# arkworks-rs/algebra

Hardware: AMD Instinct MI355X
Metric: G1 scalar-muls/sec (MSM, 2^24) (higher is better)
Workload: dtype u32

## Files before the change

### algebra_amd/_lib.py

```python
import ctypes as C
import os

_HERE = os.path.dirname(os.path.abspath(__file__))
LIB_PATH = os.environ.get("ARK_HIP_LIB") or os.path.join(_HERE, "libark_hip.so")

u64p = C.POINTER(C.c_uint64)


class ArkHipError(RuntimeError):
    def __init__(self, code, what):
        super().__init__("%s failed with code %d" % (what, code))
        self.code = code


class Radix2DomainStruct(C.Structure):
    _fields_ = [
        ("size", C.c_uint64),
        ("log_size_of_group", C.c_uint32),
        ("_pad", C.c_uint32),
        ("size_as_field_element", C.c_uint64 * 4),
        ("size_inv", C.c_uint64 * 4),
        ("group_gen", C.c_uint64 * 4),
        ("group_gen_inv", C.c_uint64 * 4),
        ("offset", C.c_uint64 * 4),
        ("offset_inv", C.c_uint64 * 4),
        ("offset_pow_size", C.c_uint64 * 4),
    ]


SYMBOLS = {
    "ark_hip_device_count": (C.c_int, []),
    "ark_hip_init": (C.c_int, [C.c_int]),
    "ark_hip_set_device": (C.c_int, [C.c_int]),
    "ark_hip_get_device": (C.c_int, []),
    "ark_hip_host_alloc": (C.c_int, [C.c_size_t, C.POINTER(C.c_void_p)]),
    "ark_hip_host_free": (C.c_int, [C.c_void_p]),
    "ark_hip_msm_sw_device_async": (C.c_int, [C.c_int, C.c_void_p, C.c_void_p, C.c_size_t, C.c_int, C.POINTER(C.c_void_p)]),
    "ark_hip_msm_wait": (C.c_int, [C.c_void_p, C.c_void_p]),
    "ark_hip_msm_bases_prepare": (C.c_int, [C.c_int, C.c_void_p, C.c_size_t, C.POINTER(C.c_void_p)]),
    "ark_hip_msm_bases_prepare_device": (C.c_int, [C.c_int, C.c_void_p, C.c_size_t, C.POINTER(C.c_void_p)]),
    "ark_hip_msm_bases_free": (C.c_int, [C.c_void_p]),
    "ark_hip_msm_bases_info": (C.c_int, [C.c_void_p, C.POINTER(C.c_size_t), C.POINTER(C.c_int), C.POINTER(C.c_int),
                                         C.POINTER(C.c_size_t)]),
    "ark_hip_msm_prepared": (C.c_int, [C.c_void_p, C.c_void_p, C.c_size_t, C.c_int, C.c_void_p]),
    "ark_hip_msm_prepared_device": (C.c_int, [C.c_void_p, C.c_void_p, C.c_size_t, C.c_int, C.c_void_p]),
    "ark_hip_msm_prepared_async": (C.c_int, [C.c_void_p, C.c_void_p, C.c_size_t, C.c_int, C.POINTER(C.c_void_p)]),
    "ark_hip_msm_prepared_device_async": (C.c_int, [C.c_void_p, C.c_void_p, C.c_size_t, C.c_int, C.POINTER(C.c_void_p)]),
    "ark_hip_msm_sw_chunks": (C.c_int, [C.c_int, C.c_void_p, C.c_size_t, C.c_void_p, C.c_size_t, C.c_size_t, C.c_void_p]),
    "ark_hip_msm_sw_multi": (C.c_int, [C.c_int, C.c_int, C.c_void_p, C.c_void_p, C.c_size_t, C.c_int, C.c_void_p]),
    "ark_hip_msm_sw_multi_device": (C.c_int, [C.c_int, C.c_int, C.POINTER(C.c_void_p), C.POINTER(C.c_void_p),
                                              C.POINTER(C.c_size_t), C.c_int, C.c_void_p]),
    "ark_hip_batch_mul_table_new": (C.c_int, [C.c_int, C.c_void_p, C.c_size_t, C.POINTER(C.c_void_p)]),
    "ark_hip_batch_mul_table_free": (C.c_int, [C.c_void_p]),
    "ark_hip_batch_mul": (C.c_int, [C.c_void_p, C.c_void_p, C.c_size_t, C.c_int, C.c_void_p]),
    "ark_hip_batch_mul_device": (C.c_int, [C.c_void_p, C.c_void_p, C.c_size_t, C.c_int, C.c_void_p]),
    "ark_hip_fft_in_place_degree_aware": (C.c_int, [C.c_int, C.POINTER(Radix2DomainStruct), C.c_void_p, C.c_size_t]),
    "ark_hip_fft_in_place_degree_aware_device": (C.c_int, [C.c_int, C.POINTER(Radix2DomainStruct), C.c_void_p, C.c_size_t]),
    "ark_hip_fft_batch_in_place_device": (C.c_int, [C.c_int, C.POINTER(Radix2DomainStruct), C.POINTER(C.c_void_p), C.c_size_t,
                                                    C.c_int]),
    "ark_hip_shutdown": (None, []),
    "ark_hip_synchronize": (C.c_int, []),
    "ark_hip_version": (C.c_char_p, []),
    "ark_hip_host_threads": (C.c_int, [C.POINTER(C.c_int)]),
    "ark_hip_curve_info": (C.c_int, [C.c_int] + [C.POINTER(C.c_int)] * 4),
    "ark_hip_malloc": (C.c_int, [C.c_size_t, C.POINTER(C.c_void_p)]),
    "ark_hip_free": (C.c_int, [C.c_void_p]),
    "ark_hip_memcpy_h2d": (C.c_int, [C.c_void_p, C.c_void_p, C.c_size_t]),
    "ark_hip_memcpy_d2h": (C.c_int, [C.c_void_p, C.c_void_p, C.c_size_t]),
    "ark_hip_curve_generator": (C.c_int, [C.c_int, C.c_void_p]),
    "ark_hip_msm_sw": (C.c_int, [C.c_int, C.c_void_p, C.c_void_p, C.c_size_t, C.c_int, C.c_void_p]),
    "ark_hip_msm_sw_small": (C.c_int, [C.c_int, C.c_void_p, C.c_void_p, C.c_size_t, C.c_int, C.c_int, C.c_void_p]),
    "ark_hip_msm_sw_small_device": (C.c_int, [C.c_int, C.c_void_p, C.c_void_p, C.c_size_t, C.c_int, C.c_int, C.c_void_p]),
    "ark_hip_msm_prepared_small_device": (C.c_int, [C.c_void_p, C.c_void_p, C.c_size_t, C.c_int, C.c_int, C.c_void_p]),
    "ark_hip_msm_bases_pin": (C.c_int, [C.c_int, C.c_void_p, C.c_size_t]),
    "ark_hip_msm_bases_unpin": (C.c_int, [C.c_int, C.c_void_p, C.c_size_t]),
    "ark_hip_msm_cache_config": (C.c_int, [C.c_longlong, C.c_int]),
    "ark_hip_msm_cache_clear": (C.c_int, []),
    "ark_hip_msm_cache_stats": (C.c_int, [C.POINTER(C.c_uint64)]),
    "ark_hip_msm_cache_hash_stats": (C.c_int, [C.POINTER(C.c_uint64)]),
    "ark_hip_msm_sw_device": (C.c_int, [C.c_int, C.c_void_p, C.c_void_p, C.c_size_t, C.c_int, C.c_void_p]),
    "ark_hip_msm_plan": (C.c_int, [C.c_int, C.c_size_t, C.c_int, C.POINTER(C.c_int), C.POINTER(C.c_int)]),
    "ark_hip_msm_plan_widths": (C.c_int, [C.c_int, C.c_size_t, C.c_uint32, C.POINTER(C.c_uint32), C.POINTER(C.c_int),
                                          C.POINTER(C.c_int)]),
    "ark_hip_msm_set_timing": (C.c_int, [C.c_int]),
    "ark_hip_msm_last_timing": (C.c_int, [C.POINTER(C.c_double)]),
    "ark_hip_sw_sum": (C.c_int, [C.c_int, C.c_void_p, C.c_size_t, C.c_void_p]),
    "ark_hip_sw_into_affine": (C.c_int, [C.c_int, C.c_void_p, C.c_size_t, C.c_void_p]),
    "ark_hip_sw_add_affine_device": (C.c_int, [C.c_int, C.c_void_p, C.c_void_p, C.c_size_t, C.c_void_p]),
    "ark_hip_sw_normalize_batch_device": (C.c_int, [C.c_int, C.c_void_p, C.c_void_p, C.c_size_t]),
    "ark_hip_radix2_domain_new": (C.c_int, [C.c_int, C.c_size_t, C.POINTER(Radix2DomainStruct)]),
    "ark_hip_radix2_domain_get_coset": (C.c_int, [C.c_int, C.POINTER(Radix2DomainStruct), C.c_void_p,
                                                  C.POINTER(Radix2DomainStruct)]),
    "ark_hip_fft_in_place": (C.c_int, [C.c_int, C.POINTER(Radix2DomainStruct), C.c_void_p]),
    "ark_hip_ifft_in_place": (C.c_int, [C.c_int, C.POINTER(Radix2DomainStruct), C.c_void_p]),
    "ark_hip_fft_in_place_device": (C.c_int, [C.c_int, C.POINTER(Radix2DomainStruct), C.c_void_p]),
    "ark_hip_ifft_in_place_device": (C.c_int, [C.c_int, C.POINTER(Radix2DomainStruct), C.c_void_p]),
    "ark_hip_fr_mul_device": (C.c_int, [C.c_int, C.c_void_p, C.c_void_p, C.c_void_p, C.c_size_t]),
    "ark_hip_poly_mul": (C.c_int, [C.c_int, C.c_void_p, C.c_size_t, C.c_void_p, C.c_size_t, C.c_void_p, C.POINTER(C.c_size_t)]),
    "ark_hip_sw_normalize_batch": (C.c_int, [C.c_int, C.c_void_p, C.c_size_t, C.c_void_p]),
    "ark_hip_fr_pow": (C.c_int, [C.c_int, C.c_void_p, C.c_uint64, C.c_void_p]),
    "ark_hip_fft_axis_device": (C.c_int, [C.c_int, C.c_void_p, C.c_uint, C.c_size_t, C.c_void_p]),
    "ark_hip_comm_unique_id": (C.c_int, [C.c_void_p]),
    "ark_hip_comm_init": (C.c_int, [C.c_void_p, C.c_int, C.c_int]),
    "ark_hip_comm_info": (C.c_int, [C.POINTER(C.c_int), C.POINTER(C.c_int)]),
    "ark_hip_comm_destroy": (C.c_int, []),
    "ark_hip_msm_sw_device_sharded": (C.c_int, [C.c_int, C.c_void_p, C.c_void_p, C.c_size_t, C.c_int, C.c_void_p]),
    "ark_hip_msm_prepared_device_sharded": (C.c_int, [C.c_void_p, C.c_void_p, C.c_size_t, C.c_int, C.c_void_p]),
    "ark_hip_msm_prepared_multi": (C.c_int, [C.c_int, C.POINTER(C.c_void_p), C.c_void_p, C.c_size_t, C.c_int, C.c_void_p]),
    "ark_hip_fft_sharded_device": (C.c_int, [C.c_int, C.POINTER(Radix2DomainStruct), C.c_void_p, C.c_int]),
    "ark_hip_fft_shard_local_device": (C.c_int, [C.c_int, C.POINTER(Radix2DomainStruct), C.c_int, C.c_int, C.c_void_p, C.c_int]),
    "ark_hip_fft_shard_cross_device": (C.c_int, [C.c_int, C.POINTER(Radix2DomainStruct), C.c_int, C.c_void_p, C.c_void_p, C.c_int]),
    "ark_hip_fr_add_device": (C.c_int, [C.c_int, C.c_void_p, C.c_void_p, C.c_void_p, C.c_size_t]),
    "ark_hip_fr_sub_device": (C.c_int, [C.c_int, C.c_void_p, C.c_void_p, C.c_void_p, C.c_size_t]),
    "ark_hip_fr_neg_device": (C.c_int, [C.c_int, C.c_void_p, C.c_void_p, C.c_size_t]),
    "ark_hip_fft_group_in_place": (C.c_int, [C.c_int, C.c_void_p, C.c_void_p, C.c_int]),
    "ark_hip_fft_group_in_place_device": (C.c_int, [C.c_int, C.c_void_p, C.c_void_p, C.c_int]),
    "ark_hip_fr_div_device": (C.c_int, [C.c_int, C.c_void_p, C.c_void_p, C.c_void_p, C.c_size_t]),
    "ark_hip_fr_inverse_device": (C.c_int, [C.c_int, C.c_void_p, C.c_void_p, C.c_size_t]),
    "ark_hip_fr_scale_device": (C.c_int, [C.c_int, C.c_void_p, C.c_void_p, C.c_void_p, C.c_size_t]),
    "ark_hip_memcpy_d2d": (C.c_int, [C.c_void_p, C.c_void_p, C.c_size_t]),
    "ark_hip_memset_device": (C.c_int, [C.c_void_p, C.c_int, C.c_size_t]),
    "ark_hip_poly_evaluate_device": (C.c_int, [C.c_int, C.c_void_p, C.c_size_t, C.c_void_p, C.c_void_p]),
    "ark_hip_poly_divide_linear_device": (C.c_int, [C.c_int, C.c_void_p, C.c_size_t, C.c_void_p, C.c_void_p, C.c_void_p]),
    "ark_hip_poly_divide_by_vanishing_device": (C.c_int, [C.c_int, C.c_size_t, C.c_void_p, C.c_size_t, C.c_void_p, C.c_void_p]),
    "ark_hip_domain_lagrange_coefficients_device": (C.c_int, [C.c_int, C.POINTER(Radix2DomainStruct), C.c_void_p, C.c_void_p]),
    "ark_hip_fr_inner_product_device": (C.c_int, [C.c_int, C.c_void_p, C.c_void_p, C.c_size_t, C.c_void_p]),
    "ark_hip_poly_scan_plan": (C.c_int, [C.c_size_t, C.POINTER(C.c_int), C.POINTER(C.c_int)]),
    "ark_hip_fft_set_kernel": (C.c_int, [C.c_int]),
    "ark_hip_fft_set_timing": (C.c_int, [C.c_int]),
    "ark_hip_fft_last_timing": (C.c_int, [C.POINTER(C.c_double)]),
}

TEST_SYMBOLS = {
    "ark_hip_test_field_op": (C.c_int, [C.c_int, C.c_int, C.c_void_p, C.c_void_p, C.c_void_p, C.c_size_t]),
    "ark_hip_test_basefield_op": (C.c_int, [C.c_int, C.c_int, C.c_void_p, C.c_void_p, C.c_void_p, C.c_size_t]),
    "ark_hip_test_host_basefield_op": (C.c_int, [C.c_int, C.c_int, C.c_void_p, C.c_void_p, C.c_void_p, C.c_size_t]),
    "ark_hip_test_point_op": (C.c_int, [C.c_int, C.c_int, C.c_void_p, C.c_void_p, C.c_void_p, C.c_size_t]),
    "ark_hip_test_msm_sharded_emulated": (C.c_int, [C.c_int, C.c_int, C.POINTER(C.c_void_p), C.POINTER(C.c_void_p),
                                                    C.POINTER(C.c_size_t), C.c_int, C.c_void_p, C.POINTER(C.c_int)]),
    "ark_hip_test_base_hash": (C.c_int, [C.c_void_p, C.c_size_t, C.POINTER(C.c_uint64)]),
    "ark_hip_test_lazy_raw_op": (C.c_int, [C.c_int, C.c_int, C.c_int, C.c_int, C.c_void_p, C.c_void_p, C.c_size_t]),
    "ark_hip_test_lazy_acc_op": (C.c_int, [C.c_int, C.c_int, C.c_void_p, C.c_void_p, C.c_void_p, C.c_size_t]),
    "ark_hip_test_msm_host_fold": (C.c_int, [C.c_int, C.c_void_p, C.c_int, C.c_int, C.c_int, C.c_void_p, C.c_void_p]),
    "ark_hip_test_msm_host_fold_l0": (C.c_int, [C.c_int, C.c_void_p, C.c_int, C.c_int, C.c_int, C.c_void_p, C.c_void_p]),
}
TEST_LIB_PATH = os.path.join(_HERE, "libark_hip_test.so")

_lib = None
_test_lib = None


def lib():
    global _lib
    if _lib is None:
        if not os.path.exists(LIB_PATH):
            raise ImportError(
                "algebra_amd: %s not found -- the HIP extension is not built and there is no CPU fallback "
                "(run `make -C algebra_amd/csrc -j8` or __graft_entry__.build())" % LIB_PATH)
        try:
            import torch
        except ImportError:
            pass
        l = C.CDLL(LIB_PATH)
        _bind(l, SYMBOLS, not os.environ.get("ARK_HIP_LIB"))
        _lib = l
    return _lib


def _bind(l, table, strict):
    for name, (res, args) in table.items():
        try:
            fn = getattr(l, name)
        except AttributeError:
            if not strict:
                continue
            raise
        fn.restype = res
        fn.argtypes = args


def test_lib():
    global _test_lib
    if _test_lib is None:
        if not os.path.exists(TEST_LIB_PATH):
            raise ImportError("algebra_amd: %s not found (run `make -C algebra_amd/csrc -j8`)" % TEST_LIB_PATH)
        try:
            import torch
        except ImportError:
            pass
        l = C.CDLL(TEST_LIB_PATH)
        _bind(l, SYMBOLS, True)
        _bind(l, TEST_SYMBOLS, True)
        _test_lib = l
    return _test_lib


def check(code, what):
    if code != 0:
        raise ArkHipError(code, what)
```

### algebra_amd/csrc/msm.cuh

```cuda
#pragma once
#include <hip/hip_runtime.h>
#include <stdio.h>
#include <stdlib.h>
#include <vector>
#include <mutex>
#include <atomic>
#include "hostpool.hpp"
#include <math.h>
#include "curves.cuh"
#include "ec28.cuh"
#include "lazyk.cuh"
#include "msm_sort.cuh"

namespace arkhip {

#define ARK_HIP_TRY(expr)                                                                          \
  do {                                                                                             \
    hipError_t _e = (expr);                                                                        \
    if (_e != hipSuccess) {                                                                        \
      fprintf(stderr, "ark_hip: %s failed: %s (%s:%d)\n", #expr, hipGetErrorString(_e), __FILE__, __LINE__); \
      return -(int)_e - 1000;                                                                      \
    }                                                                                              \
  } while (0)

static constexpr u32 KEY_NONE = 0xffffffffu;

__host__ __device__ __forceinline__ int msm_window_width(int w, int c, int W, int narrow) {
  return w >= W - narrow ? c - 1 : c;
}

template <class SP>
__host__ __device__ __forceinline__ u32 msm_scalar_magnitude(const u32* __restrict__ scalars, u32 i, int mont, u32* v ,
                                                             u32* __restrict__ err) {
  typedef Fp<SP> S;
  S s = S::load(scalars + (size_t)i * S::N);
  if (mont) s = S::from_mont(s);
  if constexpr (SP::BITS < 32 * S::N) {
    if ((s.l[S::N - 1] >> (SP::BITS - 32 * (S::N - 1))) != 0) {
#if defined(__HIP_DEVICE_COMPILE__)
      if (err) atomicOr(err, 1u);
#else
      (void)err;
#endif
      s = S::zero();
    }
  }
  {
    u32 u[S::N];
    u32 borrow = 0;
#pragma unroll
    for (int k = 0; k < S::N; k++) {
      u32 bo;
      u[k] = __builtin_subc(s.l[k], (u32)SP::P[k], borrow, &bo);
      borrow = bo;
    }
    if (!borrow) {
#pragma unroll
      for (int k = 0; k < S::N; k++) s.l[k] = u[k];
    }
  }
  u32 t[S::N];
  {
    u32 borrow = 0;
#pragma unroll
    for (int k = 0; k < S::N; k++) {
      u64 x = (u64)SP::P[k] - s.l[k] - borrow;
      t[k] = (u32)x;
      borrow = (u32)(x >> 63);
    }
  }
  bool lt = false;
#pragma unroll
  for (int k = 0; k < S::N; k++) {
    if (t[k] != s.l[k]) lt = t[k] < s.l[k];
  }
#pragma unroll
  for (int k = 0; k < S::N; k++) v[k] = lt ? t[k] : s.l[k];
  v[S::N] = 0;
  return lt ? 0x80000000u : 0u;
}

static constexpr int MSM_WIDTH_CLASSES = 9;
static constexpr int MSM_WIDTH_TOP[MSM_WIDTH_CLASSES] = {0, 1, 8, 16, 32, 64, 128, 192, 256};
struct MsmWidths {
  u32 max_bits;
  u32 count[MSM_WIDTH_CLASSES];
};
template <class SP>
__global__ void __launch_bounds__(1024) msm_scalar_bits_kernel(const u32* __restrict__ scalars, u32 n, u32 stride, int mont,
                                                               u32* __restrict__ out ,
                                                               u32 chunk = 0, u32* __restrict__ nz_counts = nullptr) {
  typedef Fp<SP> S;
  __shared__ u32 blk[1 + MSM_WIDTH_CLASSES];
  if (threadIdx.x <= MSM_WIDTH_CLASSES) blk[threadIdx.x] = 0;
  __syncthreads();
  u32 bits = 0;
  u32 mine[MSM_WIDTH_CLASSES] = {0, 0, 0, 0, 0, 0, 0, 0, 0};
  const u64 step = chunk ? (u64)blockDim.x : (u64)gridDim.x * blockDim.x;
  const u64 first = chunk ? (u64)blockIdx.x * chunk + threadIdx.x : (u64)blockIdx.x * blockDim.x + threadIdx.x;
  const u64 rounds = chunk ? (u64)chunk / blockDim.x
                           : (((u64)n + stride - 1) / stride + step - 1) / step;
  for (u64 it = 0; it < rounds; it++) {
    const u64 t = it * step + first;
    int cls = -1;
    if (t * stride < n) {
      u32 v[S::N + 1];
      (void)msm_scalar_magnitude<SP>(scalars, (u32)(t * stride), mont, v, nullptr);
      u32 b = 0;
#pragma unroll
      for (int k = 0; k < S::N; k++)
        if (v[k]) b = 32u * (u32)k + 32u - (u32)__builtin_clz(v[k]);
      bits = b > bits ? b : bits;
      cls = 0;
#pragma unroll
      for (int k = 1; k < MSM_WIDTH_CLASSES; k++) cls += b > (u32)MSM_WIDTH_TOP[k - 1] ? 1 : 0;
    }
#pragma unroll
    for (int k = 0; k < MSM_WIDTH_CLASSES; k++) mine[k] += (u32)__popcll(__ballot(cls == k));
  }
#pragma unroll
  for (int o = 32; o > 0; o >>= 1) {
    const u32 other = (u32)__shfl_xor((int)bits, o);
    bits = other > bits ? other : bits;
  }
  if ((threadIdx.x & 63) == 0) {
    atomicMax(&blk[0], bits);
#pragma unroll
    for (int k = 0; k < MSM_WIDTH_CLASSES; k++)
      if (mine[k]) atomicAdd(&blk[1 + k], mine[k]);
  }
  __syncthreads();
  if (nz_counts && threadIdx.x == 0) {
    u32 seen = 0;
#pragma unroll
    for (int k = 0; k < MSM_WIDTH_CLASSES; k++) seen += blk[1 + k];
    nz_counts[blockIdx.x] = seen - blk[1];
  }
  if (gridDim.x == 1) {
    if (threadIdx.x <= MSM_WIDTH_CLASSES) out[threadIdx.x] = blk[threadIdx.x];
  } else if (threadIdx.x == 0) {
    if (blk[0] > __atomic_load_n(out, __ATOMIC_RELAXED)) atomicMax(out, blk[0]);
  } else if (threadIdx.x <= MSM_WIDTH_CLASSES && blk[threadIdx.x]) {
    atomicAdd(out + threadIdx.x, blk[threadIdx.x]);
  }
}

template <class SP>
__global__ void __launch_bounds__(1024) msm_compact_scalars_kernel(const u32* __restrict__ scalars, u32 n, int mont, u32 chunk,
                                                                   const u32* __restrict__ chunk_off, u32* __restrict__ err,
                                                                   u32* __restrict__ out_scalars, u32* __restrict__ out_idx, u32 cap) {
  typedef Fp<SP> S;
  __shared__ u32 wave_cnt[16];
  __shared__ u32 run_s;
  if (threadIdx.x == 0) run_s = chunk_off[blockIdx.x];
  __syncthreads();
  const u32 lane = threadIdx.x & 63u, wave = threadIdx.x >> 6;
  const u32 rounds = chunk / blockDim.x;
  for (u32 it = 0; it < rounds; it++) {
    const u64 i = (u64)blockIdx.x * chunk + (u64)it * blockDim.x + threadIdx.x;
    bool keep = false;
    if (i < n) {
      u32 v[S::N + 1];
      (void)msm_scalar_magnitude<SP>(scalars, (u32)i, mont, v, err);
      u32 any = 0;
#pragma unroll
      for (int k = 0; k < S::N; k++) any |= v[k];
      keep = any != 0;
    }
    const unsigned long long m = __ballot(keep);
    if (lane == 0) wave_cnt[wave] = (u32)__popcll(m);
    __syncthreads();
    u32 before = run_s;
    for (u32 w = 0; w < wave; w++) before += wave_cnt[w];
    if (keep) {
      const u32 pos = before + (u32)__popcll(m & ((1ull << lane) - 1ull));
      if (pos < cap) {
        const uint4* src = (const uint4*)(scalars + (size_t)i * S::N);
        uint4* dst = (uint4*)(out_scalars + (size_t)pos * S::N);
        dst[0] = src[0];
        dst[1] = src[1];
        out_idx[pos] = (u32)i;
      } else {
        atomicOr(err, 2u);
      }
    }
    __syncthreads();
    if (threadIdx.x == 0) {
      u32 tot = 0;
      for (u32 w = 0; w < (blockDim.x >> 6); w++) tot += wave_cnt[w];
      run_s += tot;
    }
    __syncthreads();
  }
}
template <class SP>
void msm_sample_widths_host(const void* h_scalars, size_t n, int mont, MsmWidths* out) {
  typedef Fp<SP> S;
  *out = MsmWidths{};
  out->max_bits = (u32)SP::BITS;
  if (n == 0) return;
  const size_t stride = n > 1024 ? n / 1024 : 1;
  size_t seen = 0;
  u32 cnt[MSM_WIDTH_CLASSES] = {0};
  for (size_t i = 0; i < n; i += stride) {
    u32 v[S::N + 1];
    (void)msm_scalar_magnitude<SP>((const u32*)h_scalars, (u32)i, mont, v, nullptr);
    u32 b = 0;
    for (int k = 0; k < S::N; k++)
      if (v[k]) b = 32u * (u32)k + 32u - (u32)__builtin_clz(v[k]);
    int cls = 0;
    for (int k = 1; k < MSM_WIDTH_CLASSES; k++) cls += b > (u32)MSM_WIDTH_TOP[k - 1] ? 1 : 0;
    cnt[cls]++;
    seen++;
  }
  for (int k = 0; k < MSM_WIDTH_CLASSES; k++) out->count[k] = (u32)((double)cnt[k] * (double)n / (double)seen);
}
static inline struct MsmPlan msm_plan_for_widths(size_t n, int field_bits, double mul_cost, bool lazy28, const MsmWidths& w);
static inline bool msm_widths_skewed(const MsmWidths& w) {
  u64 seen = 0, wide = 0;
  for (int k = 0; k < MSM_WIDTH_CLASSES; k++) {
    seen += w.count[k];
    if (MSM_WIDTH_TOP[k] > 128) wide += w.count[k];
  }
  return 2 * wide < seen;
}

template <class SP>
__global__ void __launch_bounds__(256) msm_digits_kernel(const u32* __restrict__ scalars, u32 n, int mont, int c,
                                                         int W, int narrow, u32* __restrict__ keys,
                                                         u32* __restrict__ err) {
  u32 i = blockIdx.x * blockDim.x + threadIdx.x;
  if (i >= n) return;
  typedef Fp<SP> S;
  u32 v[S::N + 1];
  const u32 flip = msm_scalar_magnitude<SP>(scalars, i, mont, v, err);
  u32 carry = 0;
  for (int w = 0; w < W; w++) {
    const int cw = msm_window_width(w, c, W, narrow);
    const u32 mask = (1u << cw) - 1u;
    const u32 half = 1u << (cw - 1);
    u32 raw = (v[0] & mask) + carry;
#pragma unroll
    for (int k = 0; k < S::N; k++) v[k] = (v[k] >> cw) | (v[k + 1] << (32 - cw));
    u32 key = KEY_NONE;
    if (w < W - 1) {
      carry = raw >= half ? 1u : 0u;
    } else {
      carry = 0;
    }
    int d = (int)raw - (int)(carry << cw);
    if (d != 0) {
      u32 mag = d < 0 ? (u32)(-d) : (u32)d;
      if (mag > half) {
        atomicOr(err, 1u);
        mag = half;
      }
      u32 sign = (d < 0 ? 0x80000000u : 0u) ^ flip;
      key = sign | (mag - 1);
    }
    keys[(size_t)w * n + i] = key;
  }
}

template <int BYTES>
__global__ void __launch_bounds__(256) msm_digits_small_kernel(const unsigned char* __restrict__ scalars, u32 n, int c, int W,
                                                               int narrow, u64 vmask, u32* __restrict__ keys) {
  u32 i = blockIdx.x * blockDim.x + threadIdx.x;
  if (i >= n) return;
  u64 v;
  if constexpr (BYTES == 1) v = scalars[i];
  else if constexpr (BYTES == 2) v = ((const unsigned short*)scalars)[i];
  else if constexpr (BYTES == 4) v = ((const u32*)scalars)[i];
  else v = ((const u64*)scalars)[i];
  v &= vmask;
  u32 carry = 0;
  for (int w = 0; w < W; w++) {
    const int cw = msm_window_width(w, c, W, narrow);
    const u32 mask = (1u << cw) - 1u;
    const u32 half = 1u << (cw - 1);
    const u32 raw = ((u32)v & mask) + carry;
    v >>= cw;
    carry = (w < W - 1 && raw >= half) ? 1u : 0u;
    const int d = (int)raw - (int)(carry << cw);
    u32 key = KEY_NONE;
    if (d != 0) {
      u32 mag = d < 0 ? (u32)(-d) : (u32)d;
      if (mag > half) mag = half;
      key = (d < 0 ? 0x80000000u : 0u) | (mag - 1);
    }
    keys[(size_t)w * n + i] = key;
  }
}

static constexpr int SCAN_TILE = 2048;

static __global__ void __launch_bounds__(256) scan_block_sums(const u32* __restrict__ in, size_t m, u32* __restrict__ sums) {
  __shared__ u32 sh[256];
  size_t base = (size_t)blockIdx.x * SCAN_TILE;
  u32 s = 0;
  for (int k = 0; k < 8; k++) {
    size_t j = base + threadIdx.x + (size_t)k * 256;
    if (j < m) s += in[j];
  }
  sh[threadIdx.x] = s;
  __syncthreads();
  for (int o = 128; o > 0; o >>= 1) {
    if ((int)threadIdx.x < o) sh[threadIdx.x] += sh[threadIdx.x + o];
    __syncthreads();
  }
  if (threadIdx.x == 0) sums[blockIdx.x] = sh[0];
}
static __global__ void __launch_bounds__(1024) scan_sums_inplace(u32* sums, u32 nb) {
  __shared__ u32 sh[1024];
  __shared__ u32 carry_s;
  if (threadIdx.x == 0) carry_s = 0;
  __syncthreads();
  for (u32 base = 0; base < nb; base += 1024) {
    u32 j = base + threadIdx.x;
    u32 x = j < nb ? sums[j] : 0;
    sh[threadIdx.x] = x;
    __syncthreads();
    for (int o = 1; o < 1024; o <<= 1) {
      u32 y = (int)threadIdx.x >= o ? sh[threadIdx.x - o] : 0;
      __syncthreads();
      sh[threadIdx.x] += y;
      __syncthreads();
    }
    u32 incl = sh[threadIdx.x];
    u32 cbase = carry_s;
    if (j < nb) sums[j] = cbase + incl - x;
    __syncthreads();
    if (threadIdx.x == 1023) carry_s = cbase + incl;
    __syncthreads();
  }
}
static constexpr u32 SCAN_SMALL_MAX = 16384;
static __global__ void __launch_bounds__(1024) scan_small_kernel(const u32* __restrict__ in, u32 m, u32* __restrict__ offsets) {
  __shared__ u32 sh[1024];
  const u32 per = (m + 1023u) / 1024u;
  const u32 lo = threadIdx.x * per;
  u32 s = 0;
  for (u32 k = 0; k < per; k++)
    if (lo + k < m) s += in[lo + k];
  sh[threadIdx.x] = s;
  __syncthreads();
  for (u32 o = 1; o < 1024; o <<= 1) {
    u32 y = threadIdx.x >= o ? sh[threadIdx.x - o] : 0;
    __syncthreads();
    sh[threadIdx.x] += y;
    __syncthreads();
  }
  u32 run = sh[threadIdx.x] - s;
  for (u32 k = 0; k < per; k++)
    if (lo + k < m) {
      offsets[lo + k] = run;
      run += in[lo + k];
    }
  if (threadIdx.x == 1023) offsets[m] = sh[1023];
}
static inline void scan_exclusive(const u32* in, size_t m, u32* sums, u32* offsets, hipStream_t stream);
static __global__ void __launch_bounds__(256) scan_apply(const u32* __restrict__ in, size_t m, const u32* __restrict__ sums,
                                                  u32* __restrict__ offsets) {
  __shared__ u32 sh[256];
  size_t base = (size_t)blockIdx.x * SCAN_TILE + (size_t)threadIdx.x * 8;
  u32 x[8];
  u32 s = 0;
#pragma unroll
  for (int k = 0; k < 8; k++) {
    size_t j = base + k;
    x[k] = j < m ? in[j] : 0;
    s += x[k];
  }
  sh[threadIdx.x] = s;
  __syncthreads();
  for (int o = 1; o < 256; o <<= 1) {
    u32 y = (int)threadIdx.x >= o ? sh[threadIdx.x - o] : 0;
    __syncthreads();
    sh[threadIdx.x] += y;
    __syncthreads();
  }
  u32 run = sums[blockIdx.x] + sh[threadIdx.x] - s;
#pragma unroll
  for (int k = 0; k < 8; k++) {
    size_t j = base + k;
    if (j < m) offsets[j] = run;
    run += x[k];
    if (j == m - 1) offsets[m] = run;
  }
}

static inline void scan_exclusive(const u32* in, size_t m, u32* sums, u32* offsets, hipStream_t stream) {
  if (m <= SCAN_SMALL_MAX) {
    hipLaunchKernelGGL(scan_small_kernel, dim3(1), dim3(1024), 0, stream, in, (u32)m, offsets);
    return;
  }
  const u32 nblk = (u32)((m + SCAN_TILE - 1) / SCAN_TILE);
  hipLaunchKernelGGL(scan_block_sums, dim3(nblk), dim3(256), 0, stream, in, m, sums);
  hipLaunchKernelGGL(scan_sums_inplace, dim3(1), dim3(1024), 0, stream, sums, nblk);
  hipLaunchKernelGGL(scan_apply, dim3(nblk), dim3(256), 0, stream, in, m, sums, offsets);
}

static constexpr int ORDER_TILE = 2048;
static constexpr int ORDER_BINS = 256;
__device__ __forceinline__ u32 msm_lane_load(const u32* __restrict__ offsets, size_t g, int wsum, size_t wstride) {
  u32 cnt = 0;
  for (int w = 0; w < wsum; w++) cnt += offsets[g + w * wstride + 1] - offsets[g + w * wstride];
  return cnt;
}
static __global__ void __launch_bounds__(256) msm_order_hist_kernel(const u32* __restrict__ offsets, size_t nb, int shift,
                                                                    u32 nblocks, int wsum, size_t wstride,
                                                                    u32* __restrict__ block_hist) {
  __shared__ u32 sh[ORDER_BINS];
  sh[threadIdx.x] = 0;
  __syncthreads();
  size_t base = (size_t)blockIdx.x * ORDER_TILE;
  for (int k = 0; k < ORDER_TILE / 256; k++) {
    size_t g = base + threadIdx.x + (size_t)k * 256;
    if (g < nb) {
      u32 cls = msm_lane_load(offsets, g, wsum, wstride) >> shift;
      if (cls > ORDER_BINS - 1) cls = ORDER_BINS - 1;
      atomicAdd(&sh[ORDER_BINS - 1 - cls], 1u);
    }
  }
  __syncthreads();
  block_hist[(size_t)threadIdx.x * nblocks + blockIdx.x] = sh[threadIdx.x];
}
static __global__ void __launch_bounds__(256) msm_order_scatter_kernel(const u32* __restrict__ offsets, size_t nb, int shift,
                                                                       u32 nblocks, int wsum, size_t wstride,
                                                                       const u32* __restrict__ block_off,
                                                                       u32* __restrict__ order) {
  __shared__ u32 sh[ORDER_BINS];
  sh[threadIdx.x] = block_off[(size_t)threadIdx.x * nblocks + blockIdx.x];
  __syncthreads();
  size_t base = (size_t)blockIdx.x * ORDER_TILE;
  for (int k = 0; k < ORDER_TILE / 256; k++) {
    size_t g = base + threadIdx.x + (size_t)k * 256;
    if (g < nb) {
      u32 cls = msm_lane_load(offsets, g, wsum, wstride) >> shift;
      if (cls > ORDER_BINS - 1) cls = ORDER_BINS - 1;
      u32 pos = atomicAdd(&sh[ORDER_BINS - 1 - cls], 1u);
      order[pos] = (u32)g;
    }
  }
}

template <class C>
__global__ void __launch_bounds__(256, C::ACC_MIN_WAVES) msm_accumulate_kernel(const char* __restrict__ bases,
                                                             const u32* __restrict__ sorted,
                                                             const u32* __restrict__ offsets,
                                                             const u32* __restrict__ order, u32 nbuckets,
                                                             const u32* __restrict__ d_thresh, int HB, int LB,
                                                             int accum, char* __restrict__ buckets) {
  typedef typename C::FA F;
  u32 t = (blockIdx.x * blockDim.x + threadIdx.x) / F::LANES;
  if (t >= nbuckets) return;
  u32 g = order ? order[t] : t;
  u32 j = offsets[g], end = offsets[g + 1];
  if (end - j > *d_thresh) return;
  if (accum && j == end) return;
  char* cell = buckets + (size_t)msm_slot_to_bucket(g, HB, LB) * XYZZ<F>::BYTES;
  XYZZ<F> acc = accum ? XYZZ<F>::load(cell) : XYZZ<F>::zero();
  if (j < end) {
    u32 e = sorted[j];
    u32 e1 = j + 1 < end ? sorted[j + 1] : 0;
    Affine<F> p = Affine<F>::load(bases + (size_t)(e & 0x7fffffffu) * Affine<F>::BYTES);
    for (;;) {
      u32 e2 = 0;
      Affine<F> p_next = p;
      const bool more = j + 1 < end;
      if (more) {
        p_next = Affine<F>::load(bases + (size_t)(e1 & 0x7fffffffu) * Affine<F>::BYTES);
        if (j + 2 < end) e2 = sorted[j + 2];
      }
      if (!p.is_zero()) {
        F y = p.y;
        if constexpr (C::RELAXED_A) y = (e >> 31) != 0 ? F::neg_r(p.y) : p.y;
        else y = F::cond_neg(p.y, (e >> 31) != 0);
        if constexpr (C::RELAXED_A) xyzz_madd_relaxed<F>(acc, p.x, y);
        else xyzz_madd<F>(acc, p.x, y);
      }
      if (!more) break;
      e = e1;
      e1 = e2;
      p = p_next;
      j++;
    }
  }
  if constexpr (C::RELAXED_A) acc = xyzz_canonical<F>(acc);
  acc.store(cell);
}

#ifndef ARK_LAZY_MIN_WAVES
#define ARK_LAZY_MIN_WAVES 2
#endif
template <class C>
__global__ void __launch_bounds__(256, ARK_LAZY_MIN_WAVES) msm_accumulate_lazy_kernel(const char* __restrict__ bases,
                                                                  const u32* __restrict__ sorted,
                                                                  const u32* __restrict__ offsets,
                                                                  const u32* __restrict__ order, u32 nbuckets,
                                                                  const u32* __restrict__ d_thresh, int HB, int LB,
                                                                  int accum, char* __restrict__ buckets) {
  typedef LazyK<C> K;
  typedef typename K::FM F;
  u32 t = (blockIdx.x * blockDim.x + threadIdx.x) / K::LANES;
  if (t >= nbuckets) return;
  u32 g = order ? order[t] : t;
  u32 j = offsets[g], end = offsets[g + 1];
  if (end - j > *d_thresh) return;
  if (accum && j == end) return;
  char* cell = buckets + (size_t)msm_slot_to_bucket(g, HB, LB) * XYZZ<F>::BYTES;
  typename K::Acc acc = K::inf();
  if (accum) acc = K::from_bucket(XYZZ<F>::load(cell));
  if (j < end) {
    u32 e = sorted[j];
    u32 e1 = j + 1 < end ? sorted[j + 1] : 0;
    Affine<F> p = Affine<F>::load(bases + (size_t)(e & 0x7fffffffu) * Affine<F>::BYTES);
    for (;;) {
      u32 e2 = 0;
      Affine<F> p_next = p;
      const bool more = j + 1 < end;
      if (more) {
        p_next = Affine<F>::load(bases + (size_t)(e1 & 0x7fffffffu) * Affine<F>::BYTES);
        if (j + 2 < end) e2 = sorted[j + 2];
      }
      if (!p.is_zero()) {
        if (K::madd(acc, p, (e >> 31) != 0))
          K::mdbl(acc, bases + (size_t)(e & 0x7fffffffu) * Affine<F>::BYTES, (e >> 31) != 0);
      }
      if (!more) break;
      e = e1;
      e1 = e2;
      p = p_next;
      j++;
    }
  }
  K::to_bucket(acc).store(cell);
}
template <class C>
__global__ void __launch_bounds__(256, ARK_LAZY_MIN_WAVES) msm_accumulate_parts_kernel(const char* __restrict__ bases,
                                                                  const u32* __restrict__ sorted,
                                                                  const u32* __restrict__ offsets,
                                                                  const u32* __restrict__ order, u32 nbuckets,
                                                                  const u32* __restrict__ d_thresh, int HB, int LB,
                                                                  u32 nparts, char* __restrict__ parts) {
  typedef LazyK<C> K;
  typedef typename K::FM F;
  const u32 gid = (blockIdx.x * blockDim.x + threadIdx.x) / K::LANES;
  const u32 part = gid / nbuckets, t = gid - part * nbuckets;
  if (part >= nparts) return;
  const u32 g = order ? order[t] : t;
  const u32 start = offsets[g], stop = offsets[g + 1];
  const u32 len = stop - start;
  if (len > *d_thresh) return;
  const u32 per = (len + nparts - 1) / nparts;
  const u32 a = part * per, b = a + per;
  u32 j = start + (a < len ? a : len);
  const u32 end = start + (b < len ? b : len);
  char* cell = parts + ((size_t)part * nbuckets + msm_slot_to_bucket(g, HB, LB)) * XYZZ<F>::BYTES;
  typename K::Acc acc = K::inf();
  if (j < end) {
    u32 e = sorted[j];
    u32 e1 = j + 1 < end ? sorted[j + 1] : 0;
    Affine<F> p = Affine<F>::load(bases + (size_t)(e & 0x7fffffffu) * Affine<F>::BYTES);
    for (;;) {
      u32 e2 = 0;
      Affine<F> p_next = p;
      const bool more = j + 1 < end;
      if (more) {
        p_next = Affine<F>::load(bases + (size_t)(e1 & 0x7fffffffu) * Affine<F>::BYTES);
        if (j + 2 < end) e2 = sorted[j + 2];
      }
      if (!p.is_zero()) {
        if (K::madd(acc, p, (e >> 31) != 0))
          K::mdbl(acc, bases + (size_t)(e & 0x7fffffffu) * Affine<F>::BYTES, (e >> 31) != 0);
      }
      if (!more) break;
      e = e1;
      e1 = e2;
      p = p_next;
      j++;
    }
  }
  K::to_bucket(acc).store(cell);
}
template <class C>
__global__ void __launch_bounds__(256) msm_sum_parts_kernel(const u32* __restrict__ offsets, u32 nbuckets,
                                                            const u32* __restrict__ d_thresh, int HB, int LB, u32 nparts,
                                                            const char* __restrict__ parts, int accum,
                                                            char* __restrict__ buckets) {
  typedef LazyK<C> K;
  typedef typename K::FM F;
  const u32 g = (blockIdx.x * blockDim.x + threadIdx.x) / K::LANES;
  if (g >= nbuckets) return;
  const u32 len = offsets[g + 1] - offsets[g];
  if (len > *d_thresh) return;
  if (accum && len == 0) return;
  const size_t bkt = msm_slot_to_bucket(g, HB, LB);
  char* cell = buckets + bkt * XYZZ<F>::BYTES;
  typename K::Acc acc = K::inf();
  if (accum) acc = K::from_bucket(XYZZ<F>::load(cell));
  for (u32 q = 0; q < nparts; q++) K::add(acc, XYZZ<F>::load(parts + ((size_t)q * nbuckets + bkt) * XYZZ<F>::BYTES));
  K::to_bucket(acc).store(cell);
}


template <class C>
__global__ void __launch_bounds__(256, ARK_LAZY_MIN_WAVES) msm_accumulate_shared_lazy_kernel(
    const char* __restrict__ table, size_t wstride, const u32* __restrict__ sorted, const u32* __restrict__ offsets,
    const u32* __restrict__ order, u32 nbuckets, int W, int B, const u32* __restrict__ d_thresh, int HB, int LB,
    char* __restrict__ buckets) {
  typedef LazyK<C> K;
  typedef typename K::FM F;
  u32 t = (blockIdx.x * blockDim.x + threadIdx.x) / K::LANES;
  if (t >= nbuckets) return;
  const u32 s = order ? order[t] : t;
  const u32 heavy_thresh = *d_thresh;
  typename K::Acc acc = K::inf();
  int w = 0;
  u32 na = offsets[s], nb2 = offsets[s + 1];
  u32 j = 0, end = 0;
  const char* wbase = table;
  auto open_next = [&]() -> bool {
    while (w < W) {
      const u32 a = na, b = nb2;
      const char* wb = table + (size_t)w * wstride * Affine<F>::BYTES;
      w++;
      if (w < W) {
        const u32 g = ((u32)w << B) | s;
        na = offsets[g];
        nb2 = offsets[g + 1];
      }
      if (b - a > heavy_thresh) continue;
      if (b > a) {
        j = a;
        end = b;
        wbase = wb;
        return true;
      }
    }
    return false;
  };
  auto next_entry = [&](u32& eo, const char*& wbo) -> bool {
    if (j >= end && !open_next()) return false;
    eo = sorted[j];
    wbo = wbase;
    j++;
    return true;
  };
  u32 e = 0, e1 = 0;
  const char *wb = table, *wb1 = table;
  if (next_entry(e, wb)) {
    Affine<F> p = Affine<F>::load(wb + (size_t)(e & 0x7fffffffu) * Affine<F>::BYTES);
    bool have1 = next_entry(e1, wb1);
    for (;;) {
      u32 e2 = 0;
      const char* wb2 = table;
      bool have2 = false;
      Affine<F> p_next = p;
      if (have1) {
        p_next = Affine<F>::load(wb1 + (size_t)(e1 & 0x7fffffffu) * Affine<F>::BYTES);
        have2 = next_entry(e2, wb2);
      }
      if (!p.is_zero()) {
        if (K::madd(acc, p, (e >> 31) != 0))
          K::mdbl(acc, wb + (size_t)(e & 0x7fffffffu) * Affine<F>::BYTES, (e >> 31) != 0);
      }
      if (!have1) break;
      e = e1;
      p = p_next;
      e1 = e2;
      wb1 = wb2;
      have1 = have2;
    }
  }
  K::to_bucket(acc).store(buckets + (size_t)msm_slot_to_bucket(s, HB, LB) * XYZZ<F>::BYTES);
}

template <class C>
__global__ void __launch_bounds__(256, C::ACC_MIN_WAVES) msm_accumulate_shared_kernel(
    const char* __restrict__ table, size_t wstride, const u32* __restrict__ sorted, const u32* __restrict__ offsets,
    const u32* __restrict__ order, u32 nbuckets, int W, int B, const u32* __restrict__ d_thresh, int HB, int LB,
    char* __restrict__ buckets) {
  typedef typename C::FA F;
  typedef XYZZ<F> Pt;
  u32 t = (blockIdx.x * blockDim.x + threadIdx.x) / F::LANES;
  if (t >= nbuckets) return;
  const u32 s = order ? order[t] : t;
  const u32 heavy_thresh = *d_thresh;
  Pt acc = Pt::zero();
  int w = 0;
  u32 na = offsets[s], nb2 = offsets[s + 1];
  u32 j = 0, end = 0;
  const char* wbase = table;
  auto open_next = [&]() -> bool {
    while (w < W) {
      const u32 a = na, b = nb2;
      const char* wb = table + (size_t)w * wstride * Affine<F>::BYTES;
      w++;
      if (w < W) {
        const u32 g = ((u32)w << B) | s;
        na = offsets[g];
        nb2 = offsets[g + 1];
      }
      if (b - a > heavy_thresh) continue;
      if (b > a) {
        j = a;
        end = b;
        wbase = wb;
        return true;
      }
    }
    return false;
  };
  auto next_entry = [&](u32& eo, const char*& wbo) -> bool {
    if (j >= end && !open_next()) return false;
    eo = sorted[j];
    wbo = wbase;
    j++;
    return true;
  };
  u32 e = 0, e1 = 0;
  const char *wb = table, *wb1 = table;
  if (next_entry(e, wb)) {
    Affine<F> p = Affine<F>::load(wb + (size_t)(e & 0x7fffffffu) * Affine<F>::BYTES);
    bool have1 = next_entry(e1, wb1);
    for (;;) {
      u32 e2 = 0;
      const char* wb2 = table;
      bool have2 = false;
      Affine<F> p_next = p;
      if (have1) {
        p_next = Affine<F>::load(wb1 + (size_t)(e1 & 0x7fffffffu) * Affine<F>::BYTES);
        have2 = next_entry(e2, wb2);
      }
      if (!p.is_zero()) {
        F y = p.y;
        if constexpr (C::RELAXED_A) y = (e >> 31) != 0 ? F::neg_r(p.y) : p.y;
        else y = F::cond_neg(p.y, (e >> 31) != 0);
        if constexpr (C::RELAXED_A) xyzz_madd_relaxed<F>(acc, p.x, y);
        else xyzz_madd<F>(acc, p.x, y);
      }
      if (!have1) break;
      e = e1;
      p = p_next;
      e1 = e2;
      wb1 = wb2;
      have1 = have2;
    }
  }
  if constexpr (C::RELAXED_A) acc = xyzz_canonical<F>(acc);
  acc.store(buckets + (size_t)msm_slot_to_bucket(s, HB, LB) * Pt::BYTES);
}

template <class C>
__global__ void __launch_bounds__(128) msm_table_step_kernel(const char* __restrict__ in, char* __restrict__ out, size_t n,
                                                             int width) {
  typedef typename C::F F;
  size_t i = (size_t)blockIdx.x * blockDim.x + threadIdx.x;
  if (i >= n) return;
  Affine<F> p = Affine<F>::load(in + i * Affine<F>::BYTES);
  XYZZ<F> acc = XYZZ<F>::zero();
  if (!p.is_zero()) {
    acc = xyzz_mdbl<F>(p.x, p.y);
    for (int k = 1; k < width; k++) acc = xyzz_dbl<F>(acc);
  }
  acc.store(out + i * XYZZ<F>::BYTES);
}

#ifndef ARK_HEAVY_CHUNK
#define ARK_HEAVY_CHUNK 1024
#endif
#ifndef ARK_HEAVY_COMBINE_THREADS
#define ARK_HEAVY_COMBINE_THREADS 128
#endif
static constexpr u32 HEAVY_CHUNK = ARK_HEAVY_CHUNK;
struct HeavyEntry { u32 bucket, first_item, items; };
__host__ __device__ __forceinline__ u32 msm_heavy_chunk(u32 total) {
  return total >= (1u << 23) ? 4u * HEAVY_CHUNK : total >= (1u << 22) ? 2u * HEAVY_CHUNK : HEAVY_CHUNK;
}

__device__ __forceinline__ u32 msm_heavy_threshold(const u32* __restrict__ offsets, u32 nslots, u32 forced) {
  const u32 total = offsets[nslots];
  u32 t = total / 154000u;
  if (t < 64u) t = 64u;
  const u32 mr = 4u * (total / nslots);
  if (t < mr && nslots >= 32768u) t = mr;
  return forced ? forced : t;
}

static __global__ void __launch_bounds__(256) msm_find_heavy_kernel(const u32* __restrict__ offsets, u32 nbuckets,
                                                                    u32 forced, u32* __restrict__ ctr ,
                                                                    HeavyEntry* __restrict__ list,
                                                                    uint2* __restrict__ items) {
  u32 g = blockIdx.x * blockDim.x + threadIdx.x;
  const u32 thresh = msm_heavy_threshold(offsets, nbuckets, forced);
  if (g == 0) ctr[2] = thresh;
  const u32 chunk = msm_heavy_chunk(offsets[nbuckets]);
  u32 k = 0, first = 0;
  if (g < nbuckets) {
    const u32 cnt = offsets[g + 1] - offsets[g];
    if (cnt > thresh) {
      k = (cnt + chunk - 1) / chunk;
      first = atomicAdd(&ctr[0], k);
      const u32 slot = atomicAdd(&ctr[1], 1u);
      list[slot] = HeavyEntry{g, first, k};
    }
  }
  if (k && k <= 16)
    for (u32 q = 0; q < k; q++) items[first + q] = make_uint2(g, q);
  unsigned long long big = __ballot(k > 16);
  while (big) {
    const int src = __ffsll((long long)big) - 1;
    big &= big - 1;
    const u32 kk = (u32)__shfl((int)k, src), ff = (u32)__shfl((int)first, src), gg = (u32)__shfl((int)g, src);
    for (u32 q = threadIdx.x & 63u; q < kk; q += 64u) items[ff + q] = make_uint2(gg, q);
  }
}

#ifndef ARK_REDUCE_LAZY
#define ARK_REDUCE_LAZY 1
#endif
template <class C, bool LAZY = (C::LAZY_A && ARK_REDUCE_LAZY != 0)>
struct AccOps;

template <class C>
struct AccOps<C, false> {
  typedef typename C::FA F;
  typedef XYZZ<F> Pt;
  typedef Pt Acc;
  static constexpr u32 LANES = F::LANES;
  static constexpr size_t ACC_BYTES = Pt::BYTES;
  ARK_DEV static Acc zero() { return Pt::zero(); }
  ARK_DEV static Acc from_pt(const Pt& p) { return p; }
  ARK_DEV static void madd(Acc& acc, const Affine<F>& p, bool neg, const char*) {
    if constexpr (C::RELAXED_A) xyzz_madd_relaxed<F>(acc, p.x, neg ? F::neg_r(p.y) : p.y);
    else xyzz_madd<F>(acc, p.x, F::cond_neg(p.y, neg));
  }
  ARK_DEV static void add(Acc& acc, const Pt& b) {
    if constexpr (C::RELAXED_A) xyzz_add_relaxed<F>(acc, b);
    else xyzz_add<F>(acc, b);
  }
  ARK_DEV static void add_acc(Acc& acc, const Acc& b) { add(acc, b); }
  ARK_DEV static Pt fin(const Acc& a) {
    if constexpr (C::RELAXED_A) return xyzz_canonical<F>(a);
    else return a;
  }
  ARK_DEV static void park(const Acc& a, char* slot) { a.store(slot); }
  ARK_DEV static Acc unpark(const char* slot) { return Pt::load(slot); }
  ARK_DEV static void tree(Acc& acc, char* sh, u32 slot, u32 width) {
    park(acc, sh + (size_t)slot * ACC_BYTES);
    __syncthreads();
    for (u32 o = width / 2; o > 0; o >>= 1) {
      if (slot < o) {
        add_acc(acc, unpark(sh + (size_t)(slot + o) * ACC_BYTES));
        park(acc, sh + (size_t)slot * ACC_BYTES);
      }
      __syncthreads();
    }
  }
};

template <class C>
struct AccOps<C, true> {
  typedef LazyK<C> K;
  typedef typename K::FM F;
  typedef XYZZ<F> Pt;
  typedef typename K::Acc Acc;
  static constexpr u32 LANES = K::LANES;
  static constexpr size_t ACC_BYTES = ((size_t)K::WORDS * 4 + 15) / 16 * 16;
  ARK_DEV static Acc zero() { return K::inf(); }
  ARK_DEV static Acc from_pt(const Pt& p) { return K::from_bucket(p); }
  ARK_DEV static void madd(Acc& acc, const Affine<F>& p, bool neg, const char* src) {
    if (K::madd(acc, p, neg)) K::mdbl(acc, src, neg);
  }
  ARK_DEV static void add(Acc& acc, const Pt& b) { K::add(acc, b); }
  ARK_DEV static void add_acc(Acc& acc, const Acc& b) { K::add_acc(acc, b); }
  ARK_DEV static Pt fin(const Acc& a) { return K::to_bucket(a); }
  ARK_DEV static void park(const Acc& a, char* slot) { K::park(a, slot); }
  ARK_DEV static Acc unpark(const char* slot) { return K::unpark(slot); }
  ARK_DEV static void tree(Acc& acc, char* sh, u32 slot, u32 width) {
    park(acc, sh + (size_t)slot * ACC_BYTES);
    __syncthreads();
    for (u32 o = width / 2; o > 0; o >>= 1) {
      if (slot < o) {
        add_acc(acc, unpark(sh + (size_t)(slot + o) * ACC_BYTES));
        park(acc, sh + (size_t)slot * ACC_BYTES);
      }
      __syncthreads();
    }
  }
};

template <class C>
__global__ void __launch_bounds__(256, (C::LAZY_A && C::FA::LANES == 2) ? 1 : 2) msm_heavy_partial_kernel(const char* __restrict__ bases,
                                                                const u32* __restrict__ sorted,
                                                                const u32* __restrict__ offsets,
                                                                const u32* __restrict__ ctr,
                                                                const uint2* __restrict__ items, size_t wstride, int B,
                                                                u32 nslots, char* __restrict__ partials) {
  typedef AccOps<C> Ops;
  typedef typename Ops::F F;
  typedef typename Ops::Pt Pt;
  constexpr u32 NS = 64 / Ops::LANES;
  extern __shared__ uint4 heavy_lds[];
  const u32 wave = __builtin_amdgcn_readfirstlane(threadIdx.x >> 6), slot = (threadIdx.x & 63) / Ops::LANES, wpb = blockDim.x >> 6;
  char* sh = (char*)heavy_lds + (size_t)wave * NS * Ops::ACC_BYTES;
  const u32 nitems = ctr[0];
  const u32 chunk = msm_heavy_chunk(offsets[nslots]);
  for (u32 first = blockIdx.x * wpb; first < nitems; first += gridDim.x * wpb) {
    const u32 item = first + wave;
    const bool live = item < nitems;
    typename Ops::Acc acc = Ops::zero();
    if (live) {
      uint2 it = items[item];
      u32 lo = offsets[it.x] + it.y * chunk;
      u32 hi = offsets[it.x + 1];
      if (hi > lo + chunk) hi = lo + chunk;
      const char* wb = bases + (size_t)(it.x >> B) * wstride * Affine<F>::BYTES;
      for (u32 j = lo + slot; j < hi; j += NS) {
        u32 e = sorted[j];
        const char* src = wb + (size_t)(e & 0x7fffffffu) * Affine<F>::BYTES;
        Affine<F> p = Affine<F>::load(src);
        if (!p.is_zero()) Ops::madd(acc, p, (e >> 31) != 0, src);
      }
    }
    Ops::tree(acc, sh, slot, NS);
    if (live && slot == 0) Ops::fin(acc).store(partials + (size_t)item * Pt::BYTES);
    __syncthreads();
  }
}

template <class C, bool SHARED>
__global__ void __launch_bounds__(ARK_HEAVY_COMBINE_THREADS) msm_heavy_combine_kernel(const u32* __restrict__ ctr,
                                                               const HeavyEntry* __restrict__ list,
                                                               const char* __restrict__ partials, int HB, int LB,
                                                               const u32* __restrict__ offsets, u32* __restrict__ sorted,
                                                               int accum, char* __restrict__ buckets) {
  typedef AccOps<C> Ops;
  typedef typename Ops::Pt Pt;
  constexpr u32 NS = ARK_HEAVY_COMBINE_THREADS / Ops::LANES;
  extern __shared__ uint4 heavy_lds[];
  char* sh = (char*)heavy_lds;
  const u32 slot = threadIdx.x / Ops::LANES;
  const u32 nheavy = ctr[1];
  for (u32 hslot = blockIdx.x; hslot < nheavy; hslot += gridDim.x) {
    HeavyEntry h = list[hslot];
    typename Ops::Acc acc = Ops::zero();
    for (u32 q = slot; q < h.items; q += NS) {
      Pt x = Pt::load(partials + (size_t)(h.first_item + q) * Pt::BYTES);
      Ops::add(acc, x);
    }
    Ops::tree(acc, sh, slot, NS);
    if (slot == 0) {
      if constexpr (SHARED) {
        Ops::fin(acc).store(buckets + (size_t)hslot * Pt::BYTES);
        if (threadIdx.x == 0) sorted[offsets[h.bucket]] = hslot;
      } else {
        char* cell = buckets + (size_t)msm_slot_to_bucket(h.bucket, HB, LB) * Pt::BYTES;
        if (accum) {
          Pt prev = Pt::load(cell);
          Ops::add(acc, prev);
        }
        Ops::fin(acc).store(cell);
      }
    }
    __syncthreads();
  }
}

template <class C>
__global__ void __launch_bounds__(64) msm_apply_heavy_kernel(const u32* __restrict__ ctr, const HeavyEntry* __restrict__ list,
                                                             const u32* __restrict__ offsets,
                                                             const u32* __restrict__ sorted,
                                                             const char* __restrict__ hfinal, int W, int B,
                                                             int HB, int LB, char* __restrict__ buckets) {
  typedef AccOps<C> Ops;
  typedef typename Ops::Pt Pt;
  const u32 nheavy = ctr[1], heavy_thresh = ctr[2];
  const u32 stride = gridDim.x * blockDim.x / Ops::LANES;
  for (u32 h = (blockIdx.x * blockDim.x + threadIdx.x) / Ops::LANES; h < nheavy; h += stride) {
    const u32 g = list[h].bucket;
    const u32 w0 = g >> B, s = g & ((1u << B) - 1u);
    bool owner = true;
    for (u32 w = 0; w < w0; w++) {
      const u32 gg = (w << B) | s;
      if (offsets[gg + 1] - offsets[gg] > heavy_thresh) owner = false;
    }
    if (!owner) continue;
    char* cell = buckets + (size_t)msm_slot_to_bucket(s, HB, LB) * Pt::BYTES;
    typename Ops::Acc acc = Ops::from_pt(Pt::load(cell));
    for (u32 w = w0; w < (u32)W; w++) {
      const u32 gg = (w << B) | s;
      const u32 a2 = offsets[gg];
      if (offsets[gg + 1] - a2 > heavy_thresh) {
        Pt x = Pt::load(hfinal + (size_t)sorted[a2] * Pt::BYTES);
        Ops::add(acc, x);
      }
    }
    Ops::fin(acc).store(cell);
  }
}

struct MsmLevelGeom {
  u32 L;
  u32 mwin;
  u32 m;
  u32 mn;
  u32 nfull;
  u32 total;
};
ARK_DEV void msm_level_chunk(const MsmLevelGeom& g, u32 t, u32& w, u32& tt, u32& len) {
  const u32 nf = g.nfull * g.m;
  u32 nbw;
  if (t < nf) {
    w = t / g.m;
    tt = t - w * g.m;
    nbw = g.mwin;
  } else {
    const u32 u = t - nf, wn = u / g.mn;
    w = g.nfull + wn;
    tt = u - wn * g.mn;
    nbw = g.mwin >> 1;
  }
  const u32 first = tt * g.L;
  len = nbw - first < g.L ? nbw - first : g.L;
}
template <class C>
__global__ void __launch_bounds__(128, (C::LAZY_A && C::FA::LANES == 2) ? 1 : 2) msm_reduce_level_kernel(const char* __restrict__ in, MsmLevelGeom g,
                                                               char* __restrict__ outS, char* __restrict__ outA) {
  typedef AccOps<C> Ops;
  typedef typename Ops::Pt Pt;
  const u32 t = (blockIdx.x * blockDim.x + threadIdx.x) / Ops::LANES;
  if (t >= g.total) return;
  u32 w, tt, len;
  msm_level_chunk(g, t, w, tt, len);
  const size_t base = (size_t)w * g.mwin + (size_t)tt * g.L;
  const size_t o = (size_t)w * g.m + tt;
  __shared__ uint4 park_lds[(128 / Ops::LANES) * Ops::ACC_BYTES / 16];
  char* slot = (char*)park_lds + (size_t)(threadIdx.x / Ops::LANES) * Ops::ACC_BYTES;
  typename Ops::Acc running = Ops::zero();
  Ops::park(running, slot);
  for (u32 r = len; r-- > 0;) {
    Pt x = Pt::load(in + (base + r) * Pt::BYTES);
    Ops::add(running, x);
    typename Ops::Acc acc = Ops::unpark(slot);
    Ops::add_acc(acc, running);
    Ops::park(acc, slot);
  }
  Ops::fin(running).store(outS + o * Pt::BYTES);
  Ops::fin(Ops::unpark(slot)).store(outA + o * Pt::BYTES);
}

template <class C>
__global__ void __launch_bounds__(128, (C::LAZY_A && C::FA::LANES == 2) ? 1 : 2) msm_reduce_level_split_kernel(
    const char* __restrict__ in, MsmLevelGeom g, char* __restrict__ outS, char* __restrict__ outA) {
  typedef AccOps<C> Ops;
  typedef typename Ops::Pt Pt;
  constexpr u32 PTS = 64 / Ops::LANES;
  __shared__ uint4 hand_lds[2 * PTS * Ops::ACC_BYTES / 16];
  const u32 role = threadIdx.x >> 6;
  const u32 pslot = (threadIdx.x & 63u) / Ops::LANES;
  const u32 t = blockIdx.x * PTS + pslot;
  const bool live = t < g.total;
  u32 w = 0, tt = 0, len = 0;
  if (live) msm_level_chunk(g, t, w, tt, len);
  const size_t base = (size_t)w * g.mwin + (size_t)tt * g.L;
  char* slot0 = (char*)hand_lds + (size_t)pslot * Ops::ACC_BYTES;
  char* slot1 = slot0 + (size_t)PTS * Ops::ACC_BYTES;
  typename Ops::Acc a = Ops::zero();
  for (u32 step = 0; step <= g.L; step++) {
    if (role == 0) {
      if (step < len) {
        Pt x = Pt::load(in + (base + (len - 1 - step)) * Pt::BYTES);
        Ops::add(a, x);
        Ops::park(a, (step & 1u) ? slot1 : slot0);
      }
    } else if (step > 0 && step <= len) {
      Ops::add_acc(a, Ops::unpark(((step - 1) & 1u) ? slot1 : slot0));
    }
    __syncthreads();
  }
  if (live) Ops::fin(a).store((role == 0 ? outS : outA) + ((size_t)w * g.m + tt) * Pt::BYTES);
}

template <class C>
__global__ void __launch_bounds__(256) msm_reduce_bits_kernel(const char* __restrict__ S, const char* __restrict__ A,
                                                              u32 m, u32 mn, u32 nfull, int nbits, u32 chunk,
                                                              char* __restrict__ partial) {
  typedef AccOps<C> Ops;
  typedef typename Ops::Pt Pt;
  extern __shared__ uint4 reduce_lds[];
  char* sh = (char*)reduce_lds;
  const u32 q = blockIdx.y, w = blockIdx.z, ch = blockIdx.x;
  const u32 slot = threadIdx.x / Ops::LANES, nslots = blockDim.x / Ops::LANES;
  const u32 mw = w < nfull ? m : mn;
  const bool plain = (int)q == nbits;
  const char* src = plain ? A : S;
  typename Ops::Acc acc = Ops::zero();
  for (u32 e = slot; e < chunk; e += nslots) {
    u32 j = ch * chunk + e;
    if (j < mw && (plain || ((j >> q) & 1u))) {
      Pt x = Pt::load(src + ((size_t)w * m + j) * Pt::BYTES);
      Ops::add(acc, x);
    }
  }
  Ops::tree(acc, sh, slot, nslots);
  if (slot == 0) Ops::fin(acc).store(partial + (((size_t)w * gridDim.y + q) * gridDim.x + ch) * Pt::BYTES);
}

template <class C>
__global__ void __launch_bounds__(64) msm_reduce_rowcol_kernel(const char* __restrict__ S, const char* __restrict__ A, u32 m,
                                                               u32 mn, u32 nfull, u32 d, u32 rows, u32 lps,
                                                               char* __restrict__ out) {
  typedef AccOps<C> Ops;
  typedef typename Ops::Pt Pt;
  constexpr u32 NS = 64 / Ops::LANES;
  __shared__ uint4 rowcol_lds[NS * Ops::ACC_BYTES / 16];
  const u32 w = blockIdx.y, slot = threadIdx.x / Ops::LANES;
  const u32 mw = w < nfull ? m : mn;
  const u32 D = 1u << d, nsum = 2 * rows + D;
  const u32 grp = slot / lps, k0 = slot - grp * lps;
  const u32 s = blockIdx.x * (NS / lps) + grp;
  typename Ops::Acc acc = Ops::zero();
  if (s < nsum) {
    const char* src = S;
    u32 first, step, len;
    if (s < 2 * rows) {
      const u32 h = s < rows ? s : s - rows;
      if (s >= rows) src = A;
      first = h * D;
      step = 1;
      len = first >= mw ? 0 : (mw - first < D ? mw - first : D);
    } else {
      first = s - 2 * rows;
      step = D;
      len = first >= mw ? 0 : (mw - first + D - 1) >> d;
    }
    src += (size_t)w * m * Pt::BYTES;
    for (u32 k = k0; k < len; k += lps) {
      Pt x = Pt::load(src + (size_t)(first + k * step) * Pt::BYTES);
      Ops::add(acc, x);
    }
  }
  Ops::tree(acc, (char*)rowcol_lds + (size_t)grp * lps * Ops::ACC_BYTES, k0, lps);
  if (s < nsum && k0 == 0) Ops::fin(acc).store(out + ((size_t)w * nsum + s) * Pt::BYTES);
}
template <class C>
__global__ void __launch_bounds__(256) msm_reduce_bits2_kernel(const char* __restrict__ rc, u32 d, u32 rows, int nbits,
                                                               char* __restrict__ out) {
  typedef AccOps<C> Ops;
  typedef typename Ops::Pt Pt;
  extern __shared__ uint4 reduce_lds[];
  char* sh = (char*)reduce_lds;
  const u32 q = blockIdx.x, w = blockIdx.y;
  const u32 slot = threadIdx.x / Ops::LANES, nslots = blockDim.x / Ops::LANES;
  const u32 D = 1u << d, nsum = 2 * rows + D;
  const bool plain = (int)q == nbits;
  const u32 first = plain ? rows : (q < d ? 2 * rows : 0);
  const u32 len = q < d ? D : rows;
  const u32 bit = q < d ? q : q - d;
  const char* src = rc + ((size_t)w * nsum + first) * Pt::BYTES;
  typename Ops::Acc acc = Ops::zero();
  for (u32 e = slot; e < len; e += nslots)
    if (plain || ((e >> bit) & 1u)) {
      Pt x = Pt::load(src + (size_t)e * Pt::BYTES);
      Ops::add(acc, x);
    }
  u32 width = 1;
  while (width < len && width < nslots) width <<= 1;
  Ops::tree(acc, sh, slot, width);
  if (slot == 0) Ops::fin(acc).store(out + ((size_t)w * gridDim.x + q) * Pt::BYTES);
}

template <class C>
__global__ void __launch_bounds__(64) msm_sum_chunks_kernel(const char* __restrict__ partial, u32 npairs, u32 nchunks,
                                                            char* __restrict__ out) {
  typedef AccOps<C> Ops;
  typedef typename Ops::Pt Pt;
  constexpr u32 NS = 64 / Ops::LANES;
  extern __shared__ uint4 chunk_lds[];
  char* sh = (char*)chunk_lds;
  const u32 t = blockIdx.x, slot = threadIdx.x / Ops::LANES;
  if (t >= npairs) return;
  typename Ops::Acc acc = Ops::zero();
  for (u32 k = slot; k < nchunks; k += NS) {
    Pt x = Pt::load(partial + ((size_t)t * nchunks + k) * Pt::BYTES);
    Ops::add(acc, x);
  }
  u32 width = 1;
  while (width < nchunks && width < NS) width <<= 1;
  Ops::tree(acc, sh, slot, width);
  if (slot == 0) Ops::fin(acc).store(out + (size_t)t * Pt::BYTES);
}

struct MsmPlan {
  int c;
  int W;
  int narrow;
  size_t nb;
  bool shared;
  unsigned parts = 0;
  size_t nbuckets() const { return shared ? ((size_t)1 << (c - 1)) : nb; }
  int red_windows() const { return shared ? 1 : W; }
};

static inline double msm_mul_cost(int curve_id) { return curve_id == 0 ? 0.5 : (curve_id >= 3 ? 2.7 : 1.0); }
static inline bool msm_lazy28(int curve_id) { return curve_id <= 2; }
static inline bool msm_lazy_enabled() {
  static const bool on = [] {
    const char* e = getenv("ARK_HIP_MSM_LAZY");
    return !(e && e[0] == '0');
  }();
  return on;
}
static inline int msm_scalar_bits(int curve_id) {
  switch (curve_id) {
    case 0: return BN254_FR::BITS;
    case 1: case 4: return BLS12_381_FR::BITS;
    default: return BLS12_377_FR::BITS;
  }
}

static inline void msm_window_layout(int c, int bits, int* W, int* narrow) {
  int w = (bits + c - 1) / c;
  int deficit = w * c - bits;
  if (deficit > w || c < 3) {
    *W = (bits + 1 + c - 1) / c;
    *narrow = 0;
    return;
  }
  *W = w;
  *narrow = deficit;
}
static inline int msm_window_offset(int w, int c, int W, int narrow) {
  int off = 0;
  for (int k = 0; k < w; k++) off += msm_window_width(k, c, W, narrow);
  return off;
}

static inline MsmPlan msm_make_plan(size_t n, int bits, double mul_cost, bool shared, bool lazy28 = false,
                                    const MsmWidths* widths = nullptr, bool split_runs = false) {
  const double plain_k = lazy28 ? 0.79 : 1.0;
  int best_c = 3;
  double best = 1e300;
  const char* env = getenv(shared ? "ARK_HIP_MSM_C_PREPARED" : "ARK_HIP_MSM_C");
  if (env && atoi(env) >= 3 && atoi(env) <= 26) {
    best_c = atoi(env);
  } else {
    const int c_max = shared ? 25 : 23;
    for (int c = 3; c <= (bits < c_max ? (bits < 3 ? 3 : bits) : c_max); c++) {
      int W, narrow;
      msm_window_layout(c, bits, &W, &narrow);
      double nbk = (double)(W - narrow) * (double)(1u << (c - 1)) + (double)narrow * (double)(1u << (c - 2));
      if (shared) nbk = (double)(1u << (c - 1));
      double entries = (double)n * W;
      if (widths) {
        entries = 0.0;
        for (int k = 1; k < MSM_WIDTH_CLASSES; k++) {
          int need = (MSM_WIDTH_TOP[k] + 1 + c - 1) / c;
          if (need > W) need = W;
          entries += (double)widths->count[k] * need;
        }
        if (entries < 1.0) entries = 1.0;
      }
      const double madd = 1.0 / 5.5e9 * mul_cost, fadd = 1.4 / 5.5e9 * mul_cost;
      const bool fp2 = mul_cost > 2.0;
      double acc = entries * madd;
      if (shared) {
        const double lanes = 131072.0 / (fp2 ? 2.0 : 1.0);
        const double load = entries / nbk, lmax = load + 3.0 * sqrt(load) + 2.0;
        const double per_add = fp2 ? 30e-6 : (nbk <= lanes / 2 ? 14e-6 : 24e-6) * mul_cost;
        const double walk = lmax * per_add + W * 5e-6;
        if (nbk <= lanes || walk > acc) acc = walk;
      } else if (fp2) {
        acc = entries * 0.40e-9 * (1.0 + ldexp(1.0, 13 - c));
        const double load = entries / nbk;
        const double chain = (load + 3.0 * sqrt(load) + 2.0) * 38e-6;
        if (chain > acc) acc = chain;
      } else {
        const double load = entries / nbk;
        const double rounds = nbk / 131072.0;
        const double credit = nbk <= 1e6 ? 1.0 : (nbk >= 4e6 ? 0.0 : (4e6 - nbk) / 3e6);
        acc = (entries - credit * nbk * (1.0 - exp(-load))) * madd * plain_k * (rounds >= 1.0 ? 1.0 + 0.3 / (rounds * rounds) : 1.0);
        const double lmax = load + 3.0 * sqrt(load) + 2.0;
        const double chain = lmax * (lazy28 ? (mul_cost < 1.0 ? 13.5e-6 : 19e-6) : 32e-6 * mul_cost);
        if (chain > acc) acc = chain;
        if (!widths && (narrow > 0 || W * c == bits)) {
          const double frac = bits == 253 ? 0.583 : (bits == 254 ? 0.756 : (bits == 255 ? 0.906 : 1.0));
          const int wt = narrow > 0 ? c - 1 : c;
          const double load_top = (double)n / (frac * ldexp(1.0, wt - 1));
          const double chain_top = (load_top + 3.0 * sqrt(load_top) + 2.0) * 11e-6 * (mul_cost < 1.0 ? 0.7 : 1.0);
          if (chain_top > acc) acc = chain_top;
        }
      }
      double red0 = nbk * 2.0 * fadd * (fp2 && shared ? 2.5 : 1.0);
      const double red0_lat = (fp2 && shared) ? 0.6e-3 : 2.0 * 8.0 * 21e-6 * mul_cost;
      if (red0_lat > red0) red0 = red0_lat;
      double bits_stage = 0.5e-3 * mul_cost;
      if (!shared && fp2) {
        red0 = 0.45e-3 + (nbk < 1.2e6 ? nbk : 1.2e6) * 2.6e-9 + (nbk > 1.2e6 ? nbk - 1.2e6 : 0.0) * 1.7e-9;
        bits_stage = 0.0;
      }
      if (!shared && !fp2) {
        const double nred = 0.5 * (nbk + (double)W * ldexp(1.0, c - 1));
        red0 = (nred * 0.47e-9 + (nred < 1e6 ? nred : 1e6) * 0.10e-9) * mul_cost;
        bits_stage = 0.40e-3 * mul_cost;
      }
      const double per_bucket = (shared && n >= ((size_t)1 << 23) && c <= 22) ? 1.5e-11 : 1.0e-10;
      const double sort = (double)n * W * 2.0e-11 + (double)W * (double)(1u << (c - 1)) * per_bucket;
      double cost = acc + red0 + bits_stage + sort;
      if (narrow == W) continue;
      if (narrow == 0) {
        const int tb = (bits - 1) - (W - 1) * c;
        if (tb >= (shared ? 0 : 1) && tb <= 5) cost *= shared ? 2.0 : 1.4;
        else if (!shared && !fp2 && bits <= 129 && tb > 5 && tb < c - 3) cost *= 1.4;
      }
      if ((size_t)n * (size_t)W >= (1ull << 32)) continue;
      static const bool dbg = getenv("ARK_HIP_PLAN_DEBUG") != nullptr;
      if (dbg)
        fprintf(stderr, "plan n=%zu c=%d W=%d narrow=%d: accumulate %.3f reduce %.3f + %.3f sort %.3f -> %.3f ms\n", n, c, W, narrow,
                acc * 1e3, red0 * 1e3, bits_stage * 1e3, sort * 1e3, cost * 1e3);
      if (cost < best) { best = cost; best_c = c; }
    }
  }
  unsigned parts = 0;
  if (split_runs && !shared && !widths && bits > 128 && !(env && atoi(env) >= 3 && atoi(env) <= 26)) {
    static const bool on = [] { const char* e = getenv("ARK_HIP_MSM_SMALL_SPLIT"); return !(e && e[0] == '0'); }();
    const bool fp2 = mul_cost > 2.0;
    int logn = 0;
    while (((size_t)1 << logn) < n) logn++;
    if (on && n >= 256 && n <= (fp2 ? (size_t)24576 : bits == 253 ? (size_t)20480 : (size_t)73728)) {
      const int cap = fp2 ? 11 : 12;
      best_c = logn - 2 < cap ? logn - 2 : cap;
      parts = (!fp2 && (n >> (best_c - 1)) >= 32) ? 8u : 4u;
    }
  }
  MsmPlan p;
  p.c = best_c;
  p.shared = shared;
  p.parts = parts;
  msm_window_layout(best_c, bits, &p.W, &p.narrow);
  if (!shared && getenv("ARK_HIP_MSM_UNIFORM")) {
    p.W = (bits + 1 + best_c - 1) / best_c;
    p.narrow = 0;
  }
  p.nb = (size_t)p.W << (best_c - 1);
  return p;
}

static inline MsmPlan msm_plan_for_widths(size_t n, int field_bits, double mul_cost, bool lazy28, const MsmWidths& w) {
  const int slack = 8;
  int bits = field_bits;
  if ((int)w.max_bits + 1 + slack <= field_bits) bits = (w.max_bits ? (int)w.max_bits : 1) + 1;
  return msm_make_plan(n, bits, mul_cost, false, lazy28, &w);
}

struct DevBuf {
  void* p = nullptr;
  size_t cap = 0;
  int ensure(size_t bytes) {
    if (bytes <= cap) return 0;
    if (p) (void)hipFree(p);
    p = nullptr;
    cap = 0;
    size_t want = bytes + bytes / 8 + 256;
    hipError_t e = hipMalloc(&p, want);
    if (e != hipSuccess) {
      fprintf(stderr, "ark_hip: hipMalloc(%zu) failed: %s\n", want, hipGetErrorString(e));
      (void)hipGetLastError();
      return -1;
    }
    cap = want;
    return 0;
  }
  void release() {
    if (p) (void)hipFree(p);
    p = nullptr;
    cap = 0;
  }
};

struct MsmTimings {
  float digits = 0, scan = 0, scatter = 0, accumulate = 0, reduce = 0, total = 0;
  int c = 0, W = 0;
};

struct MsmJob {
  void* pinned = nullptr;
  size_t pinned_cap = 0;
  hipEvent_t done = nullptr;
  hipEvent_t acc_done = nullptr;
  bool busy = false;
  bool empty = false;
  bool no_result = false;
  MsmPlan pl{};
  int nbits = 0;
  u32 L0 = 1;
  u32 Q = 0;
  size_t npairs = 0;
  const char* d_sums = nullptr;
  bool short_job = false;
  bool timing = false;
  hipEvent_t ev[6] = {nullptr, nullptr, nullptr, nullptr, nullptr, nullptr};
};
static constexpr int MSM_JOBS = 4;

struct MsmWorkspace {
  DevBuf hctr, hlist, hitems, hpart, hfinal, keys, part, thist, toff, sorted, offsets, sums, buckets, lvlS[2], lvlA[2],
      order, ohist, ooff, probe, big, parts;
  MsmJob jobs[MSM_JOBS];
  std::mutex mu;
  bool attr_set = false;
  hipStream_t side = nullptr;
  hipEvent_t grp_ev[2] = {nullptr, nullptr};
  u32* probe_host = nullptr;
  DevBuf nzcnt, cscal, cidx;
  bool probe_allowed = true;
  void release() {
    if (probe_host) (void)hipHostFree(probe_host);
    probe_host = nullptr;
    hctr.release(); hlist.release(); hitems.release(); hpart.release(); hfinal.release();
    nzcnt.release(); cscal.release(); cidx.release();
    keys.release(); part.release(); thist.release(); toff.release(); sorted.release();
    offsets.release(); sums.release();
    order.release(); ohist.release(); ooff.release(); probe.release(); big.release(); parts.release();
    buckets.release();
    if (side) { (void)hipStreamSynchronize(side); (void)hipStreamDestroy(side); side = nullptr; }
    for (auto& e : grp_ev) { if (e) (void)hipEventDestroy(e); e = nullptr; }
    for (int i = 0; i < 2; i++) { lvlS[i].release(); lvlA[i].release(); }
    for (auto& j : jobs) {
      if (j.pinned) (void)hipHostFree(j.pinned);
      j.pinned = nullptr;
      j.pinned_cap = 0;
      if (j.done) (void)hipEventDestroy(j.done);
      if (j.acc_done) (void)hipEventDestroy(j.acc_done);
      j.done = nullptr;
      for (auto& e : j.ev) { if (e) (void)hipEventDestroy(e); e = nullptr; }
      j.busy = false;
    }
  }
};

static inline int msm_job_pinned(MsmJob& j, size_t bytes) {
  if (j.pinned_cap >= bytes) return 0;
  if (j.pinned) (void)hipHostFree(j.pinned);
  j.pinned = nullptr;
  j.pinned_cap = 0;
  ARK_HIP_TRY(hipHostMalloc(&j.pinned, bytes + 256));
  j.pinned_cap = bytes + 256;
  return 0;
}

struct MsmPiece {
  const MsmPlan* plan;
  void* buckets;
  bool first, last;
  hipEvent_t after_prev;
  hipEvent_t after_this;
};

template <class C>
int msm_enqueue(MsmWorkspace& ws, const void* d_points, size_t wstride, const MsmPlan* prepared, const void* d_scalars,
                size_t n, int scalars_mont, hipStream_t stream, bool timing, int sbytes = 0, int sbits = 0,
                const MsmPiece* piece = nullptr) {
  typedef typename C::F F;
  typedef XYZZ<F> Pt;
  std::lock_guard<std::mutex> lock(ws.mu);
  int slot = -1;
  for (int i = 0; i < MSM_JOBS; i++)
    if (!ws.jobs[i].busy) { slot = i; break; }
  if (slot < 0) return -6;
  MsmJob& job = ws.jobs[slot];
  job.empty = (n == 0);
  job.timing = false;
  job.no_result = false;
  if (piece && (prepared || n == 0)) return -1;
  if (n == 0) {
    job.busy = true;
    return slot;
  }
  if (n >= (1ull << 31)) return -2;
  if (sbytes && (prepared || (sbytes != 1 && sbytes != 2 && sbytes != 4 && sbytes != 8) || sbits < 1 || sbits > 8 * sbytes))
    return -1;
  int plan_bits = sbytes ? sbits + 1 : C::S::BITS;
  MsmWidths widths{};
  bool have_widths = false;
  u32 nz_chunk = 0, nz_blocks = 0;
  bool measured_exact = false;
  if (!sbytes && !piece && n >= ((size_t)1 << 19)) {
    static const bool probe_on = [] {
      const char* e = getenv("ARK_HIP_MSM_PROBE");
      return !(e && atoi(e) == 0);
    }();
    bool idle = true;
    for (int i = 0; i < MSM_JOBS; i++) idle = idle && !ws.jobs[i].busy;
    if (probe_on && idle && ws.probe_allowed) {
      constexpr size_t PW = (1 + MSM_WIDTH_CLASSES) * 4;
      if (ws.probe.ensure(PW)) return -3;
      if (!ws.probe_host) ARK_HIP_TRY(hipHostMalloc((void**)&ws.probe_host, 64, hipHostMallocDefault));
      auto measure = [&](u32 stride, MsmWidths* w) -> int {
        const u32 cnt = (u32)((n + stride - 1) / stride);
        u32 blocks = cnt <= 8192 ? 1u : (cnt + 1023) / 1024;
        if (blocks > 1024) blocks = 1024;
        if (blocks > 1) ARK_HIP_TRY(hipMemsetAsync(ws.probe.p, 0, PW, stream));
        if (stride == 1 && blocks > 1) {
          nz_chunk = (u32)(((n + blocks - 1) / blocks + 1023) / 1024 * 1024);
          nz_blocks = (u32)((n + nz_chunk - 1) / nz_chunk);
          if (ws.nzcnt.ensure((size_t)(2 * nz_blocks + 2) * 4)) return -3;
          hipLaunchKernelGGL((msm_scalar_bits_kernel<typename C::S>), dim3(nz_blocks), dim3(1024), 0, stream,
                             (const u32*)d_scalars, (u32)n, stride, scalars_mont, (u32*)ws.probe.p, nz_chunk, (u32*)ws.nzcnt.p);
        } else
        hipLaunchKernelGGL((msm_scalar_bits_kernel<typename C::S>), dim3(blocks), dim3(1024), 0, stream,
                           (const u32*)d_scalars, (u32)n, stride, scalars_mont, (u32*)ws.probe.p);
        ARK_HIP_TRY(hipMemcpyAsync(ws.probe_host, ws.probe.p, PW, hipMemcpyDeviceToHost, stream));
        ARK_HIP_TRY(hipStreamSynchronize(stream));
        w->max_bits = ws.probe_host[0];
        for (int k = 0; k < MSM_WIDTH_CLASSES; k++) w->count[k] = ws.probe_host[1 + k];
        return 0;
      };
      MsmWidths sample{};
      if (int rc = measure((u32)(n / 4096), &sample)) return rc;
      if (msm_widths_skewed(sample)) {
        if (int rc = measure(1u, &widths)) return rc;
        measured_exact = nz_blocks > 1;
        if (!prepared) {
          have_widths = true;
        } else if (widths.max_bits <= 48) {
          prepared = nullptr;
          wstride = 0;
          have_widths = true;
        }
      }
    }
  }
  const MsmPlan pl = prepared ? *prepared
                     : piece  ? *piece->plan
                     : have_widths ? msm_plan_for_widths(n, C::S::BITS, msm_mul_cost(C::ID), C::LAZY_A, widths)
                                   : msm_make_plan(n, plan_bits, msm_mul_cost(C::ID), false, C::LAZY_A, nullptr,
                                                   C::LAZY_A && msm_lazy_enabled());
  const size_t n_all = n;
  const void* const d_scalars_all = d_scalars;
  bool compacted = false;
  if (measured_exact && !sbytes && !piece) {
    static const bool compact_env = [] { const char* e = getenv("ARK_HIP_MSM_COMPACT"); return !(e && e[0] == '0'); }();
    const size_t zeros = widths.count[0];
    if (compact_env && zeros * 4 >= n && zeros < n && zeros * (size_t)pl.W >= 3 * n) {
      const size_t nz = n - zeros;
      if (ws.cscal.ensure(nz * 32) || ws.cidx.ensure(nz * 4)) return -3;
      compacted = true;
      n = nz;
      d_scalars = ws.cscal.p;
    }
  }
  const int c = pl.c, W = pl.W;
  const size_t nb = pl.nb;
  const size_t nbk = pl.nbuckets();
  const int Wr = pl.red_windows();
  if ((size_t)n * (size_t)W >= (1ull << 32)) return -2;
  if (prepared && (wstride < n || (size_t)W * wstride >= (1ull << 31))) return -2;
  const size_t mwin = (size_t)1 << (c - 1);

  const int Bbits = c - 1;
  int HB, LB;
  msm_part_split(n, Bbits, &HB, &LB);
  const u32 nsuper = (u32)W << HB;
  const u32 ptile = msm_part_tile(HB);
  const u32 ntiles = (u32)((n + ptile - 1) / ptile);
  const size_t nthist = (size_t)nsuper * ntiles;
  if (ws.keys.ensure((size_t)W * n * 4)) return -3;
  if (ws.sorted.ensure((size_t)W * n * 4)) return -3;
  if (ws.part.ensure((size_t)W * n * 8)) return -3;
  if (ws.thist.ensure(nthist * 4) || ws.toff.ensure((nthist + 2) * 4)) return -3;
  if (ws.offsets.ensure((nb + 2) * 4)) return -3;
  const u32 ntscan = (u32)((nthist + SCAN_TILE - 1) / SCAN_TILE);
  const u32 noblk = (u32)((nbk + ORDER_TILE - 1) / ORDER_TILE);
  const size_t nohist = (size_t)noblk * ORDER_BINS;
  const u32 noscan = (u32)((nohist + SCAN_TILE - 1) / SCAN_TILE);
  const size_t nsums = (size_t)(ntscan > noscan ? ntscan : noscan) + 2;
  if (ws.sums.ensure(2 * nsums * 4)) return -3;
  if (ws.order.ensure(nbk * 4) || ws.ohist.ensure((nohist + ORDER_BINS) * 4) || ws.ooff.ensure((nohist + ORDER_BINS + 2) * 4)) return -3;
  if (!piece && ws.buckets.ensure(nbk * Pt::BYTES)) return -3;
  char* const d_buckets = piece ? (char*)piece->buckets : (char*)ws.buckets.p;
  const int accum = (piece && !piece->first) ? 1 : 0;

  const u32 red_narrow = (!pl.shared && mwin >= 2) ? (u32)pl.narrow : 0u;
  const u32 red_full = (u32)Wr - red_narrow;
  u32 L0 = 32;
  {
    size_t want = (mwin * (size_t)Wr) >> 17;
    u32 p2 = 1;
    while (p2 < want) p2 <<= 1;
    const size_t nbr = mwin * (size_t)Wr;
    const u32 l0_min = nbr <= ((size_t)1 << 15) ? 2 : (nbr <= ((size_t)1 << 17) ? 4 : 8);
    if (p2 < l0_min) p2 = l0_min;
    if (p2 < L0) L0 = p2;
    if (Wr == 1 && nbr > ((size_t)1 << 18)) L0 = nbr <= ((size_t)1 << 21) ? 16 : 32;
    if (Wr > 1 && C::FA::LANES == 1 && nbr > ((size_t)1 << 19) && nbr <= ((size_t)1 << 20)) L0 = 16;
    if (Wr > 1 && C::FA::LANES == 2 && nbr > ((size_t)1 << 18)) {
      const u32 cap = C::S::BITS == 253 ? 64u : 32u;
      u32 g = 8;
      while (g < cap && (size_t)g * 32768 < nbr) g <<= 1;
      L0 = g;
    }
    static const bool fill_env = [] { const char* e = getenv("ARK_HIP_MSM_L0_FILL"); return !(e && e[0] == '0'); }();
    if (fill_env && Wr > 1 && C::FA::LANES == 1 && L0 == 32 && nbr > ((size_t)1 << 21)) {
      static const size_t resident = [] {
        int dev = 0, cus = 0, blocks = 0;
        if (hipGetDevice(&dev) != hipSuccess || hipDeviceGetAttribute(&cus, hipDeviceAttributeMultiprocessorCount, dev) != hipSuccess ||
            hipOccupancyMaxActiveBlocksPerMultiprocessor(&blocks, msm_reduce_level_kernel<C>, 128, 0) != hipSuccess) {
          (void)hipGetLastError();
          return (size_t)0;
        }
        return (size_t)blocks * (size_t)cus * 128;
      }();
      auto chunks = [&](u32 L) { return red_full * ((mwin + L - 1) / L) + red_narrow * ((mwin / 2 + L - 1) / L); };
      if (resident) {
        const size_t rounds = (chunks(32) + resident - 1) / resident;
        while (L0 > 8 && chunks(L0 - 1) <= rounds * resident) L0--;
      }
    }
    if (const char* e0 = getenv("ARK_HIP_MSM_L0")) {
      int v = atoi(e0);
      if (v >= 1 && v <= 128) L0 = (u32)v;
    }
    if (L0 > mwin) L0 = (u32)mwin;
  }
  const size_t m = (mwin + L0 - 1) / L0;
  const size_t mn = red_narrow ? (mwin / 2 + L0 - 1) / L0 : m;
  int nbits = 0;
  while (((size_t)1 << nbits) < m) nbits++;
  const u32 Q = (u32)nbits + 1;
  bool two_digit = m >= (C::FA::LANES == 2 ? 1024u : 2048u);
  if (const char* e2 = getenv("ARK_HIP_MSM_STAGE2")) {
    if (e2[0] == '0') two_digit = false;
    if (e2[0] == '1') two_digit = true;
  }
  const u32 d2 = (u32)nbits / 2;
  const u32 rows2 = (u32)((m + ((size_t)1 << d2) - 1) >> d2);
  const size_t nsum2 = 2 * (size_t)rows2 + ((size_t)1 << d2);
  u32 chunk = (size_t)Wr * Q * ((m + 4095) / 4096) < 512 ? 1024 : 4096;
  if (Wr == 1) chunk = m <= 16384 ? 1024 : (m <= 65536 ? 2048 : 4096);
  if (const char* ec = getenv("ARK_HIP_MSM_CHUNK")) {
    int v = atoi(ec);
    if (v == 256 || v == 512 || v == 1024 || v == 2048 || v == 4096 || v == 8192 || v == 16384) chunk = (u32)v;
  }
  if (chunk > m || two_digit) chunk = (u32)m;
  const u32 nchunks = (u32)((m + chunk - 1) / chunk);
  const size_t npart = (size_t)Wr * Q * nchunks;
  const size_t npairs = (size_t)Wr * Q;
  if (ws.lvlS[0].ensure(m * Wr * Pt::BYTES) || ws.lvlA[0].ensure(m * Wr * Pt::BYTES)) return -3;
  if (ws.lvlS[1].ensure(npart * Pt::BYTES)) return -3;
  if (nchunks > 1 && ws.lvlA[1].ensure(npairs * Pt::BYTES)) return -3;
  if (two_digit && ws.lvlA[1].ensure((size_t)Wr * nsum2 * Pt::BYTES)) return -3;
  {
    int rc = msm_job_pinned(job, npairs * Pt::BYTES + 64);
    if (rc) return rc;
  }
  if (!job.done) ARK_HIP_TRY(hipEventCreateWithFlags(&job.done, hipEventDisableTiming));
  if (!job.acc_done) ARK_HIP_TRY(hipEventCreateWithFlags(&job.acc_done, hipEventDisableTiming));
  if (timing) {
    for (auto& e : job.ev)
      if (!e) ARK_HIP_TRY(hipEventCreate(&e));
    ARK_HIP_TRY(hipEventRecord(job.ev[0], stream));
  }

  u32* keys = (u32*)ws.keys.p;
  u32* sorted = (u32*)ws.sorted.p;
  u32* offsets = (u32*)ws.offsets.p;
  u32* thist = (u32*)ws.thist.p;
  u32* toff = (u32*)ws.toff.p;
  uint2* part = (uint2*)ws.part.p;
  u32* order = (u32*)ws.order.p;
  u32* sums = (u32*)ws.sums.p;

  const size_t total_entries = (size_t)n * W;
  size_t mean_load = total_entries / nbk;
  u32 forced_thresh = 0;
  if (const char* hv = getenv("ARK_HIP_MSM_HEAVY")) {
    if (atoi(hv) >= 64) forced_thresh = (u32)atoi(hv);
  }
  const size_t max_heavy = total_entries / 64 + 1;
  const size_t max_items = total_entries / HEAVY_CHUNK + max_heavy + 1;
  if (ws.hctr.ensure(64) || ws.hlist.ensure((max_heavy + 1) * sizeof(HeavyEntry)) || ws.hitems.ensure((max_items + 1) * 8) ||
      ws.hpart.ensure((max_items + 1) * Pt::BYTES))
    return -3;
  if (pl.shared && ws.hfinal.ensure(max_heavy * Pt::BYTES)) return -3;
  ARK_HIP_TRY(hipMemsetAsync(ws.hctr.p, 0, 64, stream));
  if (compacted) {
    u32* const cnt = (u32*)ws.nzcnt.p;
    u32* const off = cnt + nz_blocks + 1;
    scan_exclusive(cnt, nz_blocks, nullptr, off, stream);
    hipLaunchKernelGGL((msm_compact_scalars_kernel<typename C::S>), dim3(nz_blocks), dim3(1024), 0, stream,
                       (const u32*)d_scalars_all, (u32)n_all, scalars_mont, nz_chunk, (const u32*)off, (u32*)ws.hctr.p + 3,
                       (u32*)ws.cscal.p, (u32*)ws.cidx.p, (u32)n);
  }
  const u32 nblk = (u32)((n + 255) / 256);
  if (sbytes) {
    const u64 vmask = sbits >= 64 ? ~0ull : ((1ull << sbits) - 1ull);
    const unsigned char* sp = (const unsigned char*)d_scalars;
    switch (sbytes) {
      case 1: hipLaunchKernelGGL((msm_digits_small_kernel<1>), dim3(nblk), dim3(256), 0, stream, sp, (u32)n, c, W, pl.narrow, vmask, keys); break;
      case 2: hipLaunchKernelGGL((msm_digits_small_kernel<2>), dim3(nblk), dim3(256), 0, stream, sp, (u32)n, c, W, pl.narrow, vmask, keys); break;
      case 4: hipLaunchKernelGGL((msm_digits_small_kernel<4>), dim3(nblk), dim3(256), 0, stream, sp, (u32)n, c, W, pl.narrow, vmask, keys); break;
      default: hipLaunchKernelGGL((msm_digits_small_kernel<8>), dim3(nblk), dim3(256), 0, stream, sp, (u32)n, c, W, pl.narrow, vmask, keys); break;
    }
  } else {
    hipLaunchKernelGGL((msm_digits_kernel<typename C::S>), dim3(nblk), dim3(256), 0, stream, (const u32*)d_scalars,
                       (u32)n, scalars_mont, c, W, pl.narrow, keys, (u32*)ws.hctr.p + 3);
  }
  if (timing) ARK_HIP_TRY(hipEventRecord(job.ev[1], stream));

  int ngroups = 1;
  if (!pl.shared && !piece && W >= 6 && n >= ((size_t)1 << 19)) {
    static const int groups_env = [] {
      const char* e = getenv("ARK_HIP_MSM_GROUPS");
      return e ? atoi(e) : 0;
    }();
    if (groups_env == 2 || (groups_env != 1 && n >= ((size_t)1 << 25))) ngroups = 2;
  }
  static const bool heavy_side_env = [] {
    const char* e = getenv("ARK_HIP_MSM_HEAVY_SIDE");
    return !(e && atoi(e) == 0);
  }();
  static const int heavy_side_min_log = [] {
    const char* e = getenv("ARK_HIP_MSM_HEAVY_SIDE_MIN_LOG");
    return e ? atoi(e) : 20;
  }();
  const bool heavy_side = heavy_side_env && ngroups == 1 && !piece && n >= ((size_t)1 << heavy_side_min_log);
  if (ngroups == 2 || heavy_side) {
    if (!ws.side) ARK_HIP_TRY(hipStreamCreateWithFlags(&ws.side, hipStreamNonBlocking));
    for (auto& e : ws.grp_ev)
      if (!e) ARK_HIP_TRY(hipEventCreateWithFlags(&e, hipEventDisableTiming));
  }
  const size_t lds_a = ((size_t)8 << HB) + (size_t)ptile * 8;
  if (lds_a > PART_SCATTER_LDS_MAX) return -2;
  const u32 stage_cap = msm_part_stage_cap(LB);
  const size_t lds_b = ((size_t)(1 << LB) + 1024 + stage_cap) * 4;
  if (!ws.attr_set) {
    ARK_HIP_TRY(hipFuncSetAttribute((const void*)msm_part_scatter_kernel, hipFuncAttributeMaxDynamicSharedMemorySize,
                                    (int)PART_SCATTER_LDS_MAX));
    ARK_HIP_TRY(hipFuncSetAttribute((const void*)msm_part_finish_kernel, hipFuncAttributeMaxDynamicSharedMemorySize,
                                    160 * 1024 - 64));
    ws.attr_set = true;
  }
  static const bool big_env = [] {
    const char* e = getenv("ARK_HIP_MSM_BIG_SLICES");
    return !(e && atoi(e) == 0);
  }();
  const bool big_on = big_env && n > (size_t)2 * PART_BIG;
  const size_t big_region = (size_t)nsuper + 2 * nb;
  if (big_on && ws.big.ensure(2 * big_region * 4)) return -3;
  bool lazy = false;
  if constexpr (C::LAZY_A) lazy = msm_lazy_enabled();
  u32 run_parts = 1;
  size_t parts_region = 0;
  if (lazy && !pl.shared && !piece) {
    static const size_t lanes_target = [] {
      const char* e = getenv("ARK_HIP_MSM_PARTS_LANES");
      return e ? (size_t)atol(e) : (size_t)262144;
    }();
    double expect = (double)n * W;
    if (have_widths) {
      expect = 0.0;
      for (int k = 1; k < MSM_WIDTH_CLASSES; k++) {
        int need = (MSM_WIDTH_TOP[k] + 1 + c - 1) / c;
        expect += (double)widths.count[k] * (need > W ? W : need);
      }
    }
    const double mean_run = expect / (double)nb;
    while (run_parts < 8 && nb * (size_t)(2 * run_parts) <= lanes_target && mean_run >= 32.0 * (2 * run_parts)) run_parts *= 2;
    if (pl.parts) run_parts = pl.parts;
    if (const char* e = getenv("ARK_HIP_MSM_RUN_PARTS")) {
      const int v = atoi(e);
      if (v == 1 || v == 2 || v == 4 || v == 8) run_parts = (u32)v;
    }
    if (run_parts > 1) {
      parts_region = (size_t)run_parts * nb * Pt::BYTES;
      if (ws.parts.ensure(2 * parts_region)) return -3;
    }
  }
  const int W0 = ngroups == 2 ? (W + 1) / 2 : W;
  struct Group {
    int w0, Wg;
    size_t slot0, nslots, nbk_g;
    u32 *keys, *sorted, *offsets, *thist, *toff, *order, *sums, *ohist, *ooff, *hctr;
    u32* big;
    u32* big_count;
    uint2* part;
    HeavyEntry* hlist;
    uint2* hitems;
    char *hpart, *buckets;
    size_t max_heavy;
  } grp[2];
  for (int g = 0; g < ngroups; g++) {
    Group& G = grp[g];
    G.w0 = g == 0 ? 0 : W0;
    G.Wg = g == 0 ? W0 : W - W0;
    G.slot0 = (size_t)G.w0 << Bbits;
    G.nslots = (size_t)G.Wg << Bbits;
    G.nbk_g = pl.shared ? nbk : G.nslots;
    G.keys = keys + (size_t)G.w0 * n;
    G.sorted = sorted + (size_t)G.w0 * n;
    G.part = part + (size_t)G.w0 * n;
    G.offsets = offsets + G.slot0 + (size_t)g;
    G.thist = thist + ((size_t)G.w0 << HB) * ntiles;
    G.toff = toff + ((size_t)G.w0 << HB) * ntiles + (size_t)g;
    G.order = order + G.slot0;
    G.sums = sums + (size_t)g * nsums;
    const size_t noblk0 = ((size_t)(pl.shared ? nbk : ((size_t)W0 << Bbits)) + ORDER_TILE - 1) / ORDER_TILE;
    G.ohist = (u32*)ws.ohist.p + (size_t)g * noblk0 * ORDER_BINS;
    G.ooff = (u32*)ws.ooff.p + (size_t)g * (noblk0 * ORDER_BINS + 1);
    G.hctr = (u32*)ws.hctr.p + 4 * g;
    G.big = big_on ? (u32*)ws.big.p + (size_t)g * big_region : nullptr;
    G.big_count = (u32*)ws.hctr.p + 8 + g;
    const size_t ent0 = (size_t)n * W0;
    const size_t mh0 = ent0 / 64 + 1, mi0 = ent0 / HEAVY_CHUNK + mh0 + 1;
    G.max_heavy = g == 0 ? (ngroups == 2 ? mh0 : max_heavy) : max_heavy - mh0;
    G.hlist = (HeavyEntry*)ws.hlist.p + (g == 0 ? 0 : mh0);
    G.hitems = (uint2*)ws.hitems.p + (g == 0 ? 0 : mi0);
    G.hpart = (char*)ws.hpart.p + (g == 0 ? 0 : mi0) * Pt::BYTES;
    G.buckets = d_buckets + (pl.shared ? 0 : G.slot0 * Pt::BYTES);
  }
  auto sort_group = [&](const Group& G, hipStream_t st, bool mark) -> int {
    const u32 nsuper_g = (u32)G.Wg << HB;
    const size_t nthist_g = (size_t)nsuper_g * ntiles;
    hipLaunchKernelGGL(msm_part_hist_kernel, dim3(ntiles, G.Wg), dim3(256), (size_t)4 << HB, st, G.keys, (u32)n, HB, LB,
                       ntiles, ptile, G.thist);
    scan_exclusive(G.thist, nthist_g, G.sums, G.toff, st);
    if (mark && timing) ARK_HIP_TRY(hipEventRecord(job.ev[2], st));
    hipLaunchKernelGGL(msm_part_scatter_kernel, dim3(ntiles, G.Wg), dim3(1024), lds_a, st, G.keys, (u32)n, HB, LB, ntiles,
                       ptile, G.toff, G.part, compacted ? (const u32*)ws.cidx.p : (const u32*)nullptr);
    hipLaunchKernelGGL(msm_part_finish_kernel, dim3(nsuper_g), dim3(1024), lds_b, st, G.part, G.toff, ntiles, LB, nsuper_g,
                       stage_cap, big_on ? PART_BIG : 0u, G.big_count, G.big, G.offsets, G.sorted);
    if (big_on) {
      u32* const bigcnt = G.big + nsuper_g;
      u32* const cursor = bigcnt + G.nslots;
      hipLaunchKernelGGL(msm_part_big_hist_kernel, dim3(PART_BIG_SLICES, PART_BIG_GRID_Y), dim3(1024), (size_t)4 << LB, st,
                         G.part, G.toff, ntiles, LB, G.big_count, G.big, bigcnt);
      hipLaunchKernelGGL(msm_part_big_place_kernel, dim3(PART_BIG_SLICES, PART_BIG_GRID_Y), dim3(1024),
                         ((size_t)8 << LB) + 4096, st, G.part, G.toff, ntiles, LB, G.big_count, G.big, bigcnt, cursor, G.offsets,
                         G.sorted);
    }
    int shift = 0;
    while ((mean_load >> shift) >= 64) shift++;
    const u32 noblk_g = (u32)((G.nbk_g + ORDER_TILE - 1) / ORDER_TILE);
    const int wsum = pl.shared ? W : 1;
    hipLaunchKernelGGL(msm_order_hist_kernel, dim3(noblk_g), dim3(256), 0, st, G.offsets, G.nbk_g, shift, noblk_g, wsum, mwin,
                       G.ohist);
    scan_exclusive(G.ohist, (size_t)noblk_g * ORDER_BINS, G.sums, G.ooff, st);
    hipLaunchKernelGGL(msm_order_scatter_kernel, dim3(noblk_g), dim3(256), 0, st, G.offsets, G.nbk_g, shift, noblk_g, wsum, mwin,
                       G.ooff, G.order);
    return 0;
  };
  auto accumulate_group = [&](const Group& G, hipStream_t st) -> int {
    hipLaunchKernelGGL(msm_find_heavy_kernel, dim3((u32)((G.nslots + 255) / 256)), dim3(256), 0, st, G.offsets, (u32)G.nslots,
                       forced_thresh, G.hctr, G.hlist, G.hitems);
    constexpr u32 LN = C::FA::LANES;
    constexpr size_t ACCB = AccOps<C>::ACC_BYTES;
    const u32 hthreads = ACCB * (256 / LN) > 49152 ? 128 : 256;
    hipStream_t const acc_st = st;
    if (heavy_side) {
      ARK_HIP_TRY(hipEventRecord(ws.grp_ev[0], st));
      ARK_HIP_TRY(hipStreamWaitEvent(ws.side, ws.grp_ev[0], 0));
      st = ws.side;
    }
    hipLaunchKernelGGL((msm_heavy_partial_kernel<C>), dim3(1024), dim3(hthreads), (hthreads / LN) * ACCB, st,
                       (const char*)d_points, G.sorted, G.offsets, G.hctr, (const uint2*)G.hitems, wstride, Bbits, (u32)G.nslots, G.hpart);
    const u32 combine_grid = G.max_heavy < 16384 ? (u32)G.max_heavy : 16384u;
    if (pl.shared)
      hipLaunchKernelGGL((msm_heavy_combine_kernel<C, true>), dim3(combine_grid), dim3(ARK_HEAVY_COMBINE_THREADS), (ARK_HEAVY_COMBINE_THREADS / LN) * ACCB, st, G.hctr,
                         (const HeavyEntry*)G.hlist, (const char*)G.hpart, HB, LB, G.offsets, G.sorted, 0, (char*)ws.hfinal.p);
    else
      hipLaunchKernelGGL((msm_heavy_combine_kernel<C, false>), dim3(combine_grid), dim3(ARK_HEAVY_COMBINE_THREADS), (ARK_HEAVY_COMBINE_THREADS / LN) * ACCB, st, G.hctr,
                         (const HeavyEntry*)G.hlist, (const char*)G.hpart, HB, LB, G.offsets, G.sorted, accum, G.buckets);
    if (heavy_side) {
      ARK_HIP_TRY(hipEventRecord(ws.grp_ev[1], ws.side));
      st = acc_st;
    }
    if (pl.shared) {
      if constexpr (C::LAZY_A) {
        if (lazy)
          hipLaunchKernelGGL((msm_accumulate_shared_lazy_kernel<C>), dim3((u32)((nbk * C::FA::LANES + 255) / 256)), dim3(256), 0, st,
                             (const char*)d_points, wstride, G.sorted, G.offsets, G.order, (u32)nbk, W, Bbits,
                             (const u32*)G.hctr + 2, HB, LB, G.buckets);
      }
      if (!lazy)
        hipLaunchKernelGGL((msm_accumulate_shared_kernel<C>), dim3((u32)((nbk * C::FA::LANES + 255) / 256)), dim3(256), 0, st,
                           (const char*)d_points, wstride, G.sorted, G.offsets, G.order, (u32)nbk, W, Bbits,
                           (const u32*)G.hctr + 2, HB, LB, G.buckets);
      if (heavy_side) ARK_HIP_TRY(hipStreamWaitEvent(st, ws.grp_ev[1], 0));
      hipLaunchKernelGGL((msm_apply_heavy_kernel<C>), dim3(1024), dim3(64), 0, st, (const u32*)G.hctr,
                         (const HeavyEntry*)G.hlist, G.offsets, G.sorted, (const char*)ws.hfinal.p, W, Bbits, HB, LB, G.buckets);
    } else {
      if constexpr (C::LAZY_A) {
        if (lazy && run_parts > 1) {
          char* const pbuf = (char*)ws.parts.p + (size_t)(&G - grp) * parts_region;
          hipLaunchKernelGGL((msm_accumulate_parts_kernel<C>), dim3((u32)((G.nslots * run_parts * C::FA::LANES + 255) / 256)),
                             dim3(256), 0, st, (const char*)d_points, G.sorted, G.offsets, G.order, (u32)G.nslots,
                             (const u32*)G.hctr + 2, HB, LB, run_parts, pbuf);
          hipLaunchKernelGGL((msm_sum_parts_kernel<C>), dim3((u32)((G.nslots * C::FA::LANES + 255) / 256)), dim3(256), 0, st,
                             G.offsets, (u32)G.nslots, (const u32*)G.hctr + 2, HB, LB, run_parts, (const char*)pbuf, accum,
                             G.buckets);
        } else if (lazy) {
          hipLaunchKernelGGL((msm_accumulate_lazy_kernel<C>), dim3((u32)((G.nslots * C::FA::LANES + 255) / 256)), dim3(256), 0, st,
                             (const char*)d_points, G.sorted, G.offsets, G.order, (u32)G.nslots, (const u32*)G.hctr + 2, HB, LB,
                             accum, G.buckets);
        }
      }
      if (!lazy)
        hipLaunchKernelGGL((msm_accumulate_kernel<C>), dim3((u32)((G.nslots * C::FA::LANES + 255) / 256)), dim3(256), 0, st,
                           (const char*)d_points, G.sorted, G.offsets, G.order, (u32)G.nslots, (const u32*)G.hctr + 2, HB, LB,
                           accum, G.buckets);
      if (heavy_side) ARK_HIP_TRY(hipStreamWaitEvent(st, ws.grp_ev[1], 0));
    }
    return 0;
  };
  if (int rc = sort_group(grp[0], stream, true)) return rc;
  if (timing) ARK_HIP_TRY(hipEventRecord(job.ev[3], stream));
  if (ngroups == 2) {
    ARK_HIP_TRY(hipEventRecord(ws.grp_ev[0], stream));
    ARK_HIP_TRY(hipStreamWaitEvent(ws.side, ws.grp_ev[0], 0));
    if (int rc = sort_group(grp[1], ws.side, false)) return rc;
    ARK_HIP_TRY(hipEventRecord(ws.grp_ev[1], ws.side));
  }
  if (piece && piece->after_prev) ARK_HIP_TRY(hipStreamWaitEvent(stream, piece->after_prev, 0));
  constexpr u32 LNr = C::FA::LANES;
  const bool two_level = nchunks > 1;
  auto reduce_windows = [&](size_t w0, size_t wg, hipStream_t st) {
    const size_t bo = w0 * m * Pt::BYTES;
    const size_t po = w0 * (size_t)Q * nchunks * Pt::BYTES;
    static const int split_env = [] { const char* e = getenv("ARK_HIP_MSM_SPLIT_LEVEL"); return e ? atoi(e) : -1; }();
    const u32 nfull_g = w0 >= red_full ? 0u : (u32)std::min<size_t>(wg, red_full - w0);
    const MsmLevelGeom geom{L0, (u32)mwin, (u32)m, (u32)mn, nfull_g, (u32)(nfull_g * m + (wg - nfull_g) * mn)};
    const size_t split_lanes = m * wg * 2;
    const bool split_level = split_env >= 0 ? split_env != 0
                                            : (LNr == 1 && L0 >= 2 && (split_lanes <= 131072 || (L0 >= 16 && split_lanes <= 262144)));
    if (split_level)
      hipLaunchKernelGGL((msm_reduce_level_split_kernel<C>), dim3((u32)(((size_t)geom.total * LNr + 63) / 64)), dim3(128), 0, st,
                         (const char*)d_buckets + w0 * mwin * Pt::BYTES, geom, (char*)ws.lvlS[0].p + bo,
                         (char*)ws.lvlA[0].p + bo);
    else
    hipLaunchKernelGGL((msm_reduce_level_kernel<C>), dim3((u32)(((size_t)geom.total * LNr + 127) / 128)), dim3(128), 0, st,
                       (const char*)d_buckets + w0 * mwin * Pt::BYTES, geom, (char*)ws.lvlS[0].p + bo,
                       (char*)ws.lvlA[0].p + bo);
    constexpr size_t ACCBr = AccOps<C>::ACC_BYTES;
    const u32 rthreads = ACCBr * (256 / LNr) > 49152 ? 128 : 256;
    if (two_digit) {
      constexpr u32 NSr = 64 / LNr;
      const u32 longest = std::max<u32>(rows2, 1u << d2);
      u32 lps = 1;
      while (lps < NSr && lps * 8 < longest) lps <<= 1;
      char* const rc = (char*)ws.lvlA[1].p + w0 * nsum2 * Pt::BYTES;
      hipLaunchKernelGGL((msm_reduce_rowcol_kernel<C>), dim3((u32)((nsum2 + NSr / lps - 1) / (NSr / lps)), (u32)wg), dim3(64), 0, st,
                         (const char*)ws.lvlS[0].p + bo, (const char*)ws.lvlA[0].p + bo, (u32)m, (u32)mn, nfull_g, d2, rows2, lps, rc);
      hipLaunchKernelGGL((msm_reduce_bits2_kernel<C>), dim3(Q, (u32)wg), dim3(rthreads), (rthreads / LNr) * ACCBr, st,
                         (const char*)rc, d2, rows2, nbits, (char*)ws.lvlS[1].p + po);
      return;
    }
    hipLaunchKernelGGL((msm_reduce_bits_kernel<C>), dim3(nchunks, Q, (u32)wg), dim3(rthreads), (rthreads / LNr) * ACCBr, st,
                       (const char*)ws.lvlS[0].p + bo, (const char*)ws.lvlA[0].p + bo, (u32)m, (u32)mn, nfull_g, nbits, chunk,
                       (char*)ws.lvlS[1].p + po);
    if (two_level)
      hipLaunchKernelGGL((msm_sum_chunks_kernel<C>), dim3((u32)(wg * Q)), dim3(64), (64 / LNr) * AccOps<C>::ACC_BYTES, st,
                         (const char*)ws.lvlS[1].p + po, (u32)(wg * Q), nchunks, (char*)ws.lvlA[1].p + w0 * Q * Pt::BYTES);
  };
  const bool whole_job = !piece || piece->last;
  static const bool split_env = getenv("ARK_HIP_MSM_SPLIT_REDUCE") && getenv("ARK_HIP_MSM_SPLIT_REDUCE")[0] == '1';
  const bool split_reduce = split_env && ngroups == 2 && whole_job && Wr == W;
  if (int rc = accumulate_group(grp[0], stream)) return rc;
  if (ngroups == 2) {
    if (split_reduce) {
      ARK_HIP_TRY(hipEventRecord(ws.grp_ev[0], stream));
      ARK_HIP_TRY(hipStreamWaitEvent(ws.side, ws.grp_ev[0], 0));
    }
    ARK_HIP_TRY(hipStreamWaitEvent(stream, ws.grp_ev[1], 0));
    if (split_reduce) {
      reduce_windows(0, (size_t)grp[0].Wg, ws.side);
      ARK_HIP_TRY(hipEventRecord(ws.grp_ev[1], ws.side));
    }
    if (int rc = accumulate_group(grp[1], stream)) return rc;
  }
  if (timing) ARK_HIP_TRY(hipEventRecord(job.ev[4], stream));
  if (piece) ARK_HIP_TRY(hipEventRecord(piece->after_this, stream));
  if (piece && !piece->last) {
    ARK_HIP_TRY(hipGetLastError());
    ARK_HIP_TRY(hipMemcpyAsync((char*)job.pinned + npairs * Pt::BYTES, (const u32*)ws.hctr.p + 3, 4, hipMemcpyDeviceToHost, stream));
    if (timing) ARK_HIP_TRY(hipEventRecord(job.ev[5], stream));
    ARK_HIP_TRY(hipEventRecord(job.done, stream));
    job.pl = pl;
    job.npairs = npairs;
    job.timing = timing;
    job.no_result = true;
    job.busy = true;
    return slot;
  }

  ARK_HIP_TRY(hipEventRecord(job.acc_done, stream));
  if (split_reduce) {
    reduce_windows((size_t)grp[1].w0, (size_t)grp[1].Wg, stream);
    ARK_HIP_TRY(hipStreamWaitEvent(stream, ws.grp_ev[1], 0));
  } else {
    reduce_windows(0, (size_t)Wr, stream);
  }
  const char* d_sums = two_level ? (const char*)ws.lvlA[1].p : (const char*)ws.lvlS[1].p;
  ARK_HIP_TRY(hipGetLastError());
  ARK_HIP_TRY(hipMemcpyAsync(job.pinned, d_sums, npairs * Pt::BYTES, hipMemcpyDeviceToHost, stream));
  ARK_HIP_TRY(hipMemcpyAsync((char*)job.pinned + npairs * Pt::BYTES, (const u32*)ws.hctr.p + 3, 4, hipMemcpyDeviceToHost, stream));
  if (timing) ARK_HIP_TRY(hipEventRecord(job.ev[5], stream));
  ARK_HIP_TRY(hipEventRecord(job.done, stream));
  job.pl = pl;
  job.nbits = nbits;
  job.L0 = L0;
  job.short_job = (double)n * (double)W <= 6.0e6;
  job.Q = Q;
  job.npairs = npairs;
  job.d_sums = d_sums;
  job.timing = timing;
  job.busy = true;
  return slot;
}

static inline hipError_t msm_wait_event(hipEvent_t ev) {
  static const bool block = [] {
    const char* e = getenv("ARK_HIP_WAIT");
    return e && e[0] == 'b';
  }();
  if (block) return hipEventSynchronize(ev);
  bool polled = false;
  for (;;) {
    const hipError_t e = hipEventQuery(ev);
    if (e != hipErrorNotReady) {
      if (polled) (void)hipGetLastError();
      return e;
    }
    polled = true;
#if defined(__x86_64__)
    __builtin_ia32_pause();
#endif
  }
}

template <class F>
XYZZ<F> msm_host_mul_small(const XYZZ<F>& h, u32 k) {
  int top = 31;
  while (!((k >> top) & 1u)) top--;
  XYZZ<F> r = h;
  for (int b = top - 1; b >= 0; b--) {
    r = xyzz_dbl<F>(r);
    if ((k >> b) & 1u) xyzz_add<F>(r, h);
  }
  return r;
}
template <class C>
XYZZ<typename C::F> msm_host_window_sum(const char* parts, u32 Q, int nbits, u32 L0, int w) {
  typedef typename C::F F;
  typedef XYZZ<F> Pt;
  auto part_at = [&](u32 q) { return Pt::load(parts + ((size_t)w * Q + q) * Pt::BYTES); };
  Pt h = Pt::zero();
  for (int b = nbits - 1; b >= 0; b--) {
    h = xyzz_dbl<F>(h);
    Pt ub = part_at((u32)b);
    xyzz_add<F>(h, ub);
  }
  h = msm_host_mul_small<F>(h, L0);
  Pt asum = part_at((u32)nbits);
  xyzz_add<F>(h, asum);
  return h;
}
template <class C>
struct MsmWindowSums {
  const char* parts;
  u32 Q;
  int nbits;
  u32 L0;
  XYZZ<typename C::F>* T;
  static void task(void* ctx, int w) {
    const MsmWindowSums& s = *(const MsmWindowSums*)ctx;
    s.T[(size_t)w] = msm_host_window_sum<C>(s.parts, s.Q, s.nbits, s.L0, w);
  }
};
template <class C>
XYZZ<typename C::F> msm_host_combine_windows(const XYZZ<typename C::F>* T, int Wr, const int* off) {
  typedef typename C::F F;
  XYZZ<F> total = T[(size_t)Wr - 1];
  for (int w = Wr - 2; w >= 0; w--) {
    for (int i = off[w]; i < off[w + 1]; i++) total = xyzz_dbl<F>(total);
    xyzz_add<F>(total, T[(size_t)w]);
  }
  return total;
}
template <class C>
XYZZ<typename C::F> msm_host_fold(const char* parts, u32 Q, int Wr, int nbits, u32 L0, const int* off) {
  typedef typename C::F F;
  typedef XYZZ<F> Pt;
  auto part_at = [&](int w, u32 q) { return Pt::load(parts + ((size_t)w * Q + q) * Pt::BYTES); };
  if (C::FA::LANES == 2 && Wr >= 4 && HostPool::instance().helpers() > 0) {
    std::vector<Pt> T((size_t)Wr);
    MsmWindowSums<C> ws{parts, Q, nbits, L0, T.data()};
    HostPool::instance().run_all(&MsmWindowSums<C>::task, &ws, Wr);
    return msm_host_combine_windows<C>(T.data(), Wr, off);
  }
  if (L0 & (L0 - 1)) {
    std::vector<Pt> T((size_t)Wr);
    for (int w = 0; w < Wr; w++) T[(size_t)w] = msm_host_window_sum<C>(parts, Q, nbits, L0, w);
    return msm_host_combine_windows<C>(T.data(), Wr, off);
  }
  int log2L0 = 0;
  while ((1u << log2L0) < L0) log2L0++;
  int top = 0;
  for (int w = 0; w < Wr; w++) top = std::max(top, off[w] + log2L0 + nbits - 1);
  Pt total = Pt::zero();
  for (int pos = top; pos >= 0; pos--) {
    total = xyzz_dbl<F>(total);
    for (int w = Wr - 1; w >= 0; w--) {
      const int rel = pos - off[w];
      if (rel < 0) continue;
      if (rel == 0) {
        Pt asum = part_at(w, (u32)nbits);
        xyzz_add<F>(total, asum);
      }
      const int b2 = rel - log2L0;
      if (b2 >= 0 && b2 < nbits) {
        Pt ub = part_at(w, (u32)b2);
        xyzz_add<F>(total, ub);
      }
    }
  }
  return total;
}

template <class C>
int msm_finish(MsmWorkspace& ws, int slot, uint64_t* out_xyz, MsmTimings* tm) {
  typedef typename C::F F;
  typedef XYZZ<F> Pt;
  if (slot < 0 || slot >= MSM_JOBS) return -1;
  MsmJob& job = ws.jobs[slot];
  if (!job.busy) return -1;
  struct Release {
    MsmWorkspace& ws;
    MsmJob& j;
    ~Release() {
      std::lock_guard<std::mutex> lock(ws.mu);
      j.busy = false;
    }
  } release{ws, job};
  if (job.empty) {
    if (out_xyz) Jac<F>::zero().store(out_xyz);
    return 0;
  }
  const MsmPlan& pl = job.pl;
  const int c = pl.c, W = pl.W, Wr = pl.red_windows(), nbits = job.nbits;
  const u32 Q = job.Q;
  std::vector<Pt> early_T;
  MsmWindowSums<C> early_ws{(const char*)job.pinned, Q, nbits, job.L0, nullptr};
  HostPool::Handle early;
  struct EarlyGuard {
    HostPool::Handle& h;
    ~EarlyGuard() {
      if (h) HostPool::instance().cancel(h);
    }
  } early_guard{early};
  static const bool tail_all = [] { const char* e = getenv("ARK_HIP_HOST_TAIL_ALL"); return !(e && e[0] == '0'); }();
  if (out_xyz && !job.no_result && (job.short_job || tail_all) && Wr >= 8 && HostPool::instance().helpers() > 0 &&
      hipEventQuery(job.done) == hipErrorNotReady) {
    (void)hipGetLastError();
    if (!job.short_job && job.acc_done) ARK_HIP_TRY(msm_wait_event(job.acc_done));
    try {
      early_T.resize((size_t)Wr);
      early_ws.T = early_T.data();
      early = HostPool::instance().open(&MsmWindowSums<C>::task, &early_ws, Wr);
    } catch (...) {
      early.reset();
    }
  }
  ARK_HIP_TRY(msm_wait_event(job.done));
  const u32 h_err = *(const u32*)((const char*)job.pinned + job.npairs * Pt::BYTES);
  if (h_err) return -4;
  if (job.no_result) {
    if (tm && job.timing) {
      (void)hipEventElapsedTime(&tm->total, job.ev[0], job.ev[5]);
      tm->c = c;
      tm->W = W;
    }
    return 0;
  }

  if (out_xyz) {
    std::vector<int> off((size_t)Wr + 1);
    off[0] = 0;
    for (int w = 0; w < Wr; w++) off[w + 1] = off[w] + msm_window_width(w, c, W, pl.narrow);
    Pt total;
    if (early) {
      HostPool::instance().run(early);
      early.reset();
      total = msm_host_combine_windows<C>(early_T.data(), Wr, off.data());
    } else {
      total = msm_host_fold<C>((const char*)job.pinned, Q, Wr, nbits, job.L0, off.data());
    }
    xyzz_to_jac<F>(total).store(out_xyz);
  }

  if (tm && job.timing) {
    (void)hipEventElapsedTime(&tm->digits, job.ev[0], job.ev[1]);
    (void)hipEventElapsedTime(&tm->scan, job.ev[1], job.ev[2]);
    (void)hipEventElapsedTime(&tm->scatter, job.ev[2], job.ev[3]);
    (void)hipEventElapsedTime(&tm->accumulate, job.ev[3], job.ev[4]);
    (void)hipEventElapsedTime(&tm->reduce, job.ev[4], job.ev[5]);
    (void)hipEventElapsedTime(&tm->total, job.ev[0], job.ev[5]);
    tm->c = c;
    tm->W = W;
  }
  return 0;
}

struct MsmSumsHeader {
  int c, W, narrow, shared, nbits;
  u32 L0;
  u32 Q, npairs;
  u32 err;
  u32 pad[7];
};
static_assert(sizeof(MsmSumsHeader) == 64, "header layout");
struct MsmSumsInfo {
  MsmSumsHeader h;
  const char* d_sums;
};
template <class C>
__global__ void __launch_bounds__(128) msm_sum_ranks_kernel(const char* __restrict__ blocks, int world, size_t block_bytes,
                                                            u32 npairs, char* __restrict__ out) {
  typedef AccOps<C> Ops;
  typedef typename Ops::Pt Pt;
  const u32 t = (blockIdx.x * blockDim.x + threadIdx.x) / Ops::LANES;
  if (t >= npairs) return;
  typename Ops::Acc acc = Ops::zero();
  for (int r = 0; r < world; r++) {
    const Pt x = Pt::load(blocks + (size_t)r * block_bytes + sizeof(MsmSumsHeader) + (size_t)t * Pt::BYTES);
    Ops::add(acc, x);
  }
  Ops::fin(acc).store(out + (size_t)t * Pt::BYTES);
}
template <class C>
int msm_sum_ranks(const void* d_blocks, int world, size_t block_bytes, u32 npairs, void* d_out, hipStream_t stream) {
  if (npairs == 0) return 0;
  constexpr u32 LN = C::FA::LANES;
  hipLaunchKernelGGL((msm_sum_ranks_kernel<C>), dim3((npairs * LN + 127) / 128), dim3(128), 0, stream, (const char*)d_blocks,
                     world, block_bytes, npairs, (char*)d_out);
  ARK_HIP_TRY(hipGetLastError());
  return 0;
}
template <class C>
int msm_fold_sums(const MsmSumsHeader& h, const void* h_sums, uint64_t* out_xyz) {
  typedef typename C::F F;
  MsmPlan pl{};
  pl.c = h.c;
  pl.W = h.W;
  pl.narrow = h.narrow;
  pl.shared = h.shared != 0;
  const int Wr = pl.red_windows();
  std::vector<int> off((size_t)Wr + 1);
  off[0] = 0;
  for (int w = 0; w < Wr; w++) off[w + 1] = off[w] + msm_window_width(w, h.c, h.W, h.narrow);
  const XYZZ<F> total = msm_host_fold<C>((const char*)h_sums, h.Q, Wr, h.nbits, h.L0, off.data());
  xyzz_to_jac<F>(total).store(out_xyz);
  return 0;
}
static inline int msm_job_sums(MsmWorkspace& ws, int slot, MsmSumsInfo* out) {
  if (slot < 0 || slot >= MSM_JOBS) return -1;
  const MsmJob& job = ws.jobs[slot];
  if (!job.busy || job.no_result) return -1;
  *out = MsmSumsInfo{};
  if (job.empty) return 1;
  out->h.c = job.pl.c;
  out->h.W = job.pl.W;
  out->h.narrow = job.pl.narrow;
  out->h.shared = job.pl.shared ? 1 : 0;
  out->h.nbits = job.nbits;
  out->h.L0 = job.L0;
  out->h.Q = job.Q;
  out->h.npairs = (u32)job.npairs;
  out->d_sums = job.d_sums;
  return 0;
}

template <class C>
int msm_prepare_table(const void* d_bases, size_t n, const MsmPlan& pl, void* d_table, void* d_tmp, hipStream_t stream) {
  typedef typename C::F F;
  const size_t row = n * Affine<F>::BYTES;
  if (n == 0) return 0;
  ARK_HIP_TRY(hipMemcpyAsync(d_table, d_bases, row, hipMemcpyDeviceToDevice, stream));
  for (int w = 0; w + 1 < pl.W; w++) {
    const int width = msm_window_width(w, pl.c, pl.W, pl.narrow);
    hipLaunchKernelGGL((msm_table_step_kernel<C>), dim3((u32)((n + 127) / 128)), dim3(128), 0, stream,
                       (const char*)d_table + (size_t)w * row, (char*)d_tmp, n, width);
    xyzz_to_affine_batched_launch<F>(d_tmp, (char*)d_table + (size_t)(w + 1) * row, n, stream);
  }
  ARK_HIP_TRY(hipGetLastError());
  return 0;
}

}
```

### algebra_amd/csrc/msm_sort.cuh

```cuda
#pragma once
#include <hip/hip_runtime.h>
#include <stdlib.h>
#include "fp.cuh"

namespace arkhip {

static constexpr int PART_LO_BITS = 10;
static constexpr int PART_LO_BITS_MAX = 12;
static constexpr u32 PART_LDS_WORDS = (160 * 1024 - 64) / 4;

static inline void msm_part_split(size_t n, int B, int* HB, int* LB) {
  int hb = 0;
  if (B > PART_LO_BITS) {
    hb = B - PART_LO_BITS;
    if (hb > 9) {
      hb = B - PART_LO_BITS_MAX;
      if (hb < 9) hb = 9;
    }
    int lg = 0;
    while (((size_t)1 << lg) < n) lg++;
    if (hb < lg - 15) hb = lg - 15;
    if (hb > B) hb = B;
    if (const char* e = getenv("ARK_HIP_MSM_HB")) {
      const int v = atoi(e);
      if (v >= 0 && v <= B && B - v <= PART_LO_BITS_MAX) hb = v;
    }
  } else {
    int lg = 0;
    while (((size_t)1 << lg) < n) lg++;
    hb = lg - 15;
    if (hb < 0) hb = 0;
    if (hb > B) hb = B;
  }
  *HB = hb;
  *LB = B - hb;
}
static inline u32 msm_part_stage_cap(int LB) { return PART_LDS_WORDS - 1024u - (1u << LB) - 16u; }
static constexpr int PART_TILE = 8192;
static constexpr int PART_TILE_BIG = 16384;
static constexpr size_t PART_SCATTER_LDS_MAX = 160 * 1024 - 4096 - 64;
static inline u32 msm_part_tile(int HB) {
  if (const char* e = getenv("ARK_HIP_MSM_TILE")) {
    const int v = atoi(e);
    if (v == PART_TILE || (v == PART_TILE_BIG && ((size_t)8 << HB) + (size_t)PART_TILE_BIG * 8 <= PART_SCATTER_LDS_MAX)) return (u32)v;
  }
  const bool fits = ((size_t)8 << HB) + (size_t)PART_TILE_BIG * 8 <= PART_SCATTER_LDS_MAX;
  return (HB >= 11 && fits) ? (u32)PART_TILE_BIG : (u32)PART_TILE;
}
static constexpr u32 PART_KEY_NONE = 0xffffffffu;
static constexpr int PART_MLP = 8;
static constexpr int PART_OUT_MLP = 4;
static constexpr int PART_SCATTER_KEYS = PART_TILE_BIG / 1024;

__host__ __device__ __forceinline__ u32 msm_slot_to_bucket(u32 slot, int HB, int LB) {
  const u32 B = (u32)(HB + LB);
  const u32 w = slot >> B;
  const u32 in = slot & ((1u << B) - 1u);
  const u32 low = in >> LB;
  const u32 high = in & ((1u << LB) - 1u);
  return (w << B) | (high << HB) | low;
}

static __device__ __forceinline__ u32 part_tile_of_block(u32 b, u32 ntiles) {
  const u32 per = ntiles >> 3;
  return b < (per << 3) ? (b & 7u) * per + (b >> 3) : b;
}

static __global__ void __launch_bounds__(256) msm_part_hist_kernel(const u32* __restrict__ keys, u32 n, int HB, int LB,
                                                                   u32 ntiles, u32 tile, u32* __restrict__ tile_hist) {
  extern __shared__ u32 part_lds[];
  const u32 nbins = 1u << HB;
  const u32 hmask = nbins - 1u;
  for (u32 b = threadIdx.x; b < nbins; b += blockDim.x) part_lds[b] = 0;
  __syncthreads();
  const u32 w = blockIdx.y;
  const size_t base = (size_t)w * n;
  const u32 tile_id = part_tile_of_block(blockIdx.x, ntiles);
  const u32 lo = tile_id * tile;
  const u32 hi = lo + tile < n ? lo + tile : n;
  for (u32 c0 = lo; c0 < hi; c0 += blockDim.x * PART_MLP) {
    u32 k[PART_MLP];
#pragma unroll
    for (int b = 0; b < PART_MLP; b++) {
      const u32 i = c0 + (u32)b * blockDim.x + threadIdx.x;
      k[b] = i < hi ? keys[base + i] : PART_KEY_NONE;
    }
#pragma unroll
    for (int b = 0; b < PART_MLP; b++)
      if (k[b] != PART_KEY_NONE) atomicAdd(&part_lds[k[b] & hmask], 1u);
  }
  __syncthreads();
  for (u32 b = threadIdx.x; b < nbins; b += blockDim.x)
    tile_hist[((size_t)((w << HB) | b)) * ntiles + tile_id] = part_lds[b];
}

static __global__ void __launch_bounds__(1024, 8) msm_part_scatter_kernel(const u32* __restrict__ keys, u32 n, int HB,
                                                                       int LB, u32 ntiles, u32 tile,
                                                                       const u32* __restrict__ tile_off,
                                                                       uint2* __restrict__ part,
                                                                       const u32* __restrict__ point_idx = nullptr) {
  extern __shared__ u32 part_lds[];
  const u32 nbins = 1u << HB;
  u32* cnt = part_lds;
  u32* lstart = part_lds + nbins;
  uint2* stage = (uint2*)(part_lds + 2 * nbins);
  __shared__ u32 wsum[1024];
  const u32 w = blockIdx.y;
  const size_t base = (size_t)w * n;
  const u32 tile_id = part_tile_of_block(blockIdx.x, ntiles);
  const u32 lo = tile_id * tile;
  const u32 hi = lo + tile < n ? lo + tile : n;
  const u32 hmask = nbins - 1u;
  for (u32 b = threadIdx.x; b < nbins; b += blockDim.x) cnt[b] = 0;
  u32 key[PART_SCATTER_KEYS], pidx[PART_SCATTER_KEYS];
#pragma unroll
  for (int b = 0; b < PART_SCATTER_KEYS; b++) {
    const u32 i = lo + (u32)b * blockDim.x + threadIdx.x;
    key[b] = i < hi ? keys[base + i] : PART_KEY_NONE;
    pidx[b] = (point_idx && i < hi) ? point_idx[i] : i;
  }
  __syncthreads();
#pragma unroll
  for (int b = 0; b < PART_SCATTER_KEYS; b++)
    if (key[b] != PART_KEY_NONE) atomicAdd(&cnt[key[b] & hmask], 1u);
  __syncthreads();
  const u32 per = (nbins + blockDim.x - 1) / blockDim.x;
  u32 s = 0;
  for (u32 q = 0; q < per; q++) {
    u32 b = threadIdx.x * per + q;
    if (b < nbins) s += cnt[b];
  }
  wsum[threadIdx.x] = s;
  __syncthreads();
  for (u32 o = 1; o < blockDim.x; o <<= 1) {
    u32 y = threadIdx.x >= o ? wsum[threadIdx.x - o] : 0;
    __syncthreads();
    wsum[threadIdx.x] += y;
    __syncthreads();
  }
  u32 run = wsum[threadIdx.x] - s;
  for (u32 q = 0; q < per; q++) {
    u32 b = threadIdx.x * per + q;
    if (b < nbins) {
      u32 v = cnt[b];
      lstart[b] = run;
      cnt[b] = run;
      run += v;
    }
  }
  __syncthreads();
  const u32 total = wsum[blockDim.x - 1];
#pragma unroll
  for (int b = 0; b < PART_SCATTER_KEYS; b++) {
    if (key[b] != PART_KEY_NONE) {
      const u32 pos = atomicAdd(&cnt[key[b] & hmask], 1u);
      stage[pos] = make_uint2(key[b], pidx[b]);
    }
  }
  __syncthreads();
  for (u32 j0 = 0; j0 < total; j0 += blockDim.x * PART_OUT_MLP) {
    uint2 e[PART_OUT_MLP];
    u32 dst[PART_OUT_MLP];
#pragma unroll
    for (int b = 0; b < PART_OUT_MLP; b++) {
      const u32 j = j0 + (u32)b * blockDim.x + threadIdx.x;
      if (j < total) {
        e[b] = stage[j];
        const u32 bin = e[b].x & hmask;
        dst[b] = tile_off[((size_t)((w << HB) | bin)) * ntiles + tile_id] + (j - lstart[bin]);
      }
    }
#pragma unroll
    for (int b = 0; b < PART_OUT_MLP; b++) {
      const u32 j = j0 + (u32)b * blockDim.x + threadIdx.x;
      if (j < total) {
        const u32 bkt = e[b].x & 0x7fffffffu;
        part[dst[b]] = make_uint2((bkt >> HB) | (e[b].x & 0x80000000u), e[b].y);
      }
    }
  }
}

__device__ __forceinline__ u32 lds_inc_leading(u32* cnt, u32 key) {
  const u32 k0 = __builtin_amdgcn_readfirstlane(key);
  const unsigned long long same = __ballot(key == k0);
  u32 pos;
  if (key == k0) {
    const u32 rank = __builtin_amdgcn_mbcnt_hi((u32)(same >> 32), __builtin_amdgcn_mbcnt_lo((u32)same, 0u));
    u32 base = 0;
    if (rank == 0) base = atomicAdd(&cnt[k0], (u32)__popcll(same));
    pos = __builtin_amdgcn_readfirstlane(base) + rank;
  } else {
    pos = atomicAdd(&cnt[key], 1u);
  }
  return pos;
}

static __global__ void __launch_bounds__(1024) msm_part_finish_kernel(const uint2* __restrict__ part,
                                                                      const u32* __restrict__ tile_off, u32 ntiles,
                                                                      int LB, u32 nsuper, u32 stage_cap, u32 big_thresh,
                                                                      u32* __restrict__ big_count, u32* __restrict__ big,
                                                                      u32* __restrict__ offsets,
                                                                      u32* __restrict__ sorted) {
  extern __shared__ u32 part_lds[];
  const u32 nlow = 1u << LB;
  u32* cnt = part_lds;
  u32* wsum = part_lds + nlow;
  u32* stage = wsum + 1024;
  const u32 sb = blockIdx.x;
  const u32 start = tile_off[(size_t)sb * ntiles];
  const u32 end = tile_off[(size_t)(sb + 1) * ntiles];
  if (sb == nsuper - 1 && threadIdx.x == 0) offsets[(size_t)nsuper << LB] = end;
  if (big_thresh && end - start > big_thresh) {
    if (threadIdx.x == 0) big[atomicAdd(big_count, 1u)] = sb;
    u32* const bigcnt = big + nsuper + ((size_t)sb << LB);
    u32* const cursor = bigcnt + ((size_t)nsuper << LB);
    for (u32 b = threadIdx.x; b < nlow; b += blockDim.x) {
      bigcnt[b] = 0;
      cursor[b] = 0;
    }
    return;
  }
  for (u32 b = threadIdx.x; b < nlow; b += blockDim.x) cnt[b] = 0;
  __syncthreads();
  const u32 lmask = nlow - 1u;
  for (u32 c0 = start; c0 < end; c0 += blockDim.x * PART_MLP) {
    u32 kx[PART_MLP];
#pragma unroll
    for (int b = 0; b < PART_MLP; b++) {
      const u32 j = c0 + (u32)b * blockDim.x + threadIdx.x;
      kx[b] = j < end ? part[j].x : PART_KEY_NONE;
    }
#pragma unroll
    for (int b = 0; b < PART_MLP; b++)
      if (kx[b] != PART_KEY_NONE) lds_inc_leading(cnt, kx[b] & lmask);
  }
  __syncthreads();
  const u32 per = nlow > blockDim.x ? nlow / blockDim.x : 1u;
  const u32 b0 = threadIdx.x * per;
  u32 v = 0;
  if (b0 < nlow)
    for (u32 k = 0; k < per; k++) v += cnt[b0 + k];
  wsum[threadIdx.x] = v;
  __syncthreads();
  for (u32 o = 1; o < blockDim.x; o <<= 1) {
    u32 y = threadIdx.x >= o ? wsum[threadIdx.x - o] : 0;
    __syncthreads();
    wsum[threadIdx.x] += y;
    __syncthreads();
  }
  if (b0 < nlow) {
    u32 run = wsum[threadIdx.x] - v;
    for (u32 k = 0; k < per; k++) {
      const u32 c = cnt[b0 + k];
      cnt[b0 + k] = run;
      offsets[((size_t)sb << LB) + b0 + k] = start + run;
      run += c;
    }
  }
  __syncthreads();
  const u32 total = end - start;
  if (total <= stage_cap) {
    for (u32 c0 = start; c0 < end; c0 += blockDim.x * PART_MLP) {
      uint2 e[PART_MLP];
#pragma unroll
      for (int b = 0; b < PART_MLP; b++) {
        const u32 j = c0 + (u32)b * blockDim.x + threadIdx.x;
        e[b] = j < end ? part[j] : make_uint2(PART_KEY_NONE, 0u);
      }
#pragma unroll
      for (int b = 0; b < PART_MLP; b++) {
        if (e[b].x != PART_KEY_NONE) {
          const u32 pos = lds_inc_leading(cnt, e[b].x & lmask);
          stage[pos] = e[b].y | (e[b].x & 0x80000000u);
        }
      }
    }
    __syncthreads();
    for (u32 j = threadIdx.x; j < total; j += blockDim.x) sorted[start + j] = stage[j];
  } else {
    for (u32 j = start + threadIdx.x; j < end; j += blockDim.x) {
      uint2 e = part[j];
      u32 pos = lds_inc_leading(cnt, e.x & lmask);
      sorted[start + pos] = e.y | (e.x & 0x80000000u);
    }
  }
}

static constexpr u32 PART_BIG = 1u << 17;
static constexpr u32 PART_BIG_SLICES = 16;
static constexpr u32 PART_BIG_GRID_Y = 32;

__device__ __forceinline__ void msm_part_big_slice(u32 start, u32 end, u32* lo, u32* hi) {
  const u32 total = end - start;
  const u32 per = (total + PART_BIG_SLICES - 1) / PART_BIG_SLICES;
  const u32 a = blockIdx.x * per, b = a + per;
  *lo = start + (a < total ? a : total);
  *hi = start + (b < total ? b : total);
}

static __global__ void __launch_bounds__(1024) msm_part_big_hist_kernel(const uint2* __restrict__ part,
                                                                        const u32* __restrict__ tile_off, u32 ntiles, int LB,
                                                                        const u32* __restrict__ big_count,
                                                                        const u32* __restrict__ big,
                                                                        u32* __restrict__ bigcnt) {
  extern __shared__ u32 part_lds[];
  const u32 nbig = big_count[0];
  const u32 nlow = 1u << LB, lmask = nlow - 1u;
  for (u32 k = blockIdx.y; k < nbig; k += gridDim.y) {
    const u32 sb = big[k];
    u32 lo, hi;
    msm_part_big_slice(tile_off[(size_t)sb * ntiles], tile_off[(size_t)(sb + 1) * ntiles], &lo, &hi);
    for (u32 b = threadIdx.x; b < nlow; b += blockDim.x) part_lds[b] = 0;
    __syncthreads();
    for (u32 c0 = lo; c0 < hi; c0 += blockDim.x * PART_MLP) {
      u32 kx[PART_MLP];
#pragma unroll
      for (int b = 0; b < PART_MLP; b++) {
        const u32 j = c0 + (u32)b * blockDim.x + threadIdx.x;
        kx[b] = j < hi ? part[j].x : PART_KEY_NONE;
      }
#pragma unroll
      for (int b = 0; b < PART_MLP; b++)
        if (kx[b] != PART_KEY_NONE) lds_inc_leading(part_lds, kx[b] & lmask);
    }
    __syncthreads();
    for (u32 b = threadIdx.x; b < nlow; b += blockDim.x)
      if (part_lds[b]) atomicAdd(&bigcnt[((size_t)sb << LB) + b], part_lds[b]);
    __syncthreads();
  }
}

static __global__ void __launch_bounds__(1024) msm_part_big_place_kernel(const uint2* __restrict__ part,
                                                                         const u32* __restrict__ tile_off, u32 ntiles, int LB,
                                                                         const u32* __restrict__ big_count,
                                                                         const u32* __restrict__ big,
                                                                         const u32* __restrict__ bigcnt,
                                                                         u32* __restrict__ cursor, u32* __restrict__ offsets,
                                                                         u32* __restrict__ sorted) {
  extern __shared__ u32 part_lds[];
  const u32 nbig = big_count[0];
  const u32 nlow = 1u << LB, lmask = nlow - 1u;
  u32* cnt = part_lds;
  u32* wsum = part_lds + nlow;
  u32* mine = wsum + 1024;
  for (u32 k = blockIdx.y; k < nbig; k += gridDim.y) {
    const u32 sb = big[k];
    const u32 start = tile_off[(size_t)sb * ntiles];
    u32 lo, hi;
    msm_part_big_slice(start, tile_off[(size_t)(sb + 1) * ntiles], &lo, &hi);
    for (u32 b = threadIdx.x; b < nlow; b += blockDim.x) {
      cnt[b] = bigcnt[((size_t)sb << LB) + b];
      mine[b] = 0;
    }
    __syncthreads();
    const u32 per = nlow > blockDim.x ? nlow / blockDim.x : 1u;
    const u32 b0 = threadIdx.x * per;
    u32 v = 0;
    if (b0 < nlow)
      for (u32 q = 0; q < per; q++) v += cnt[b0 + q];
    wsum[threadIdx.x] = v;
    __syncthreads();
    for (u32 o = 1; o < blockDim.x; o <<= 1) {
      u32 y = threadIdx.x >= o ? wsum[threadIdx.x - o] : 0;
      __syncthreads();
      wsum[threadIdx.x] += y;
      __syncthreads();
    }
    if (b0 < nlow) {
      u32 run = wsum[threadIdx.x] - v;
      for (u32 q = 0; q < per; q++) {
        const u32 c = cnt[b0 + q];
        cnt[b0 + q] = run;
        if (blockIdx.x == 0) offsets[((size_t)sb << LB) + b0 + q] = start + run;
        run += c;
      }
    }
    __syncthreads();
    for (u32 c0 = lo; c0 < hi; c0 += blockDim.x * PART_MLP) {
      u32 kx[PART_MLP];
#pragma unroll
      for (int b = 0; b < PART_MLP; b++) {
        const u32 j = c0 + (u32)b * blockDim.x + threadIdx.x;
        kx[b] = j < hi ? part[j].x : PART_KEY_NONE;
      }
#pragma unroll
      for (int b = 0; b < PART_MLP; b++)
        if (kx[b] != PART_KEY_NONE) lds_inc_leading(mine, kx[b] & lmask);
    }
    __syncthreads();
    for (u32 b = threadIdx.x; b < nlow; b += blockDim.x) {
      const u32 m = mine[b];
      if (m) mine[b] = cnt[b] + atomicAdd(&cursor[((size_t)sb << LB) + b], m);
    }
    __syncthreads();
    for (u32 c0 = lo; c0 < hi; c0 += blockDim.x * PART_MLP) {
      uint2 e[PART_MLP];
#pragma unroll
      for (int b = 0; b < PART_MLP; b++) {
        const u32 j = c0 + (u32)b * blockDim.x + threadIdx.x;
        e[b] = j < hi ? part[j] : make_uint2(PART_KEY_NONE, 0u);
      }
#pragma unroll
      for (int b = 0; b < PART_MLP; b++) {
        if (e[b].x != PART_KEY_NONE) {
          const u32 pos = lds_inc_leading(mine, e[b].x & lmask);
          sorted[start + pos] = e[b].y | (e[b].x & 0x80000000u);
        }
      }
    }
    __syncthreads();
  }
}


}
```

### algebra_amd/csrc/testops_field.hip

```cpp
#define ARK_LAZYTEST_FFT 1
#include "lazytest.cuh"
#ifndef ARK_TEST_FIELD
#error "compile with -DARK_TEST_FIELD=BLS12_381_FR (or another scalar field of params.hpp)"
#endif
#define ARK_CAT2(a, b) a##b
#define ARK_CAT(a, b) ARK_CAT2(a, b)
namespace arkhip {
int ARK_CAT(test_lazy_raw_op_, ARK_TEST_FIELD)(int op, int k, int h, const void* in, void* out, size_t n, hipStream_t s) {
  return lazytest::lazy_raw_op_launch<ARK_TEST_FIELD, true, void>(op, k, h, in, out, n, s);
}
}
```

### include/ark_hip.h

```cpp
#ifndef ARK_HIP_H
#define ARK_HIP_H
#include <stddef.h>
#include <stdint.h>
#ifdef __cplusplus
extern "C" {
#endif
#if defined(__GNUC__) || defined(__clang__)
#pragma GCC visibility push(default)
#endif

enum { ARK_HIP_BN254_FQ = 0, ARK_HIP_BN254_FR = 1, ARK_HIP_BLS12_381_FQ = 2, ARK_HIP_BLS12_381_FR = 3,
       ARK_HIP_BLS12_377_FQ = 4, ARK_HIP_BLS12_377_FR = 5 };
enum { ARK_HIP_BN254_G1 = 0, ARK_HIP_BLS12_381_G1 = 1, ARK_HIP_BLS12_377_G1 = 2, ARK_HIP_BLS12_377_G2 = 3,
       ARK_HIP_BLS12_381_G2 = 4 };
enum { ARK_HIP_OK = 0, ARK_HIP_ERR_ARG = -1, ARK_HIP_ERR_SIZE = -2, ARK_HIP_ERR_NOMEM = -3,
       ARK_HIP_ERR_SCALAR_RANGE = -4, ARK_HIP_ERR_NO_DEVICE = -5, ARK_HIP_ERR_BUSY = -6,
       ARK_HIP_ERR_COMM = -7   };

int ark_hip_device_count(void);
int ark_hip_init(int device);
int ark_hip_set_device(int device);
int ark_hip_get_device(void);
void ark_hip_shutdown(void);
int ark_hip_synchronize(void);
const char* ark_hip_version(void);
int ark_hip_host_threads(int out[2]);
int ark_hip_curve_info(int curve, int* fe_words, int* scalar_field, int* base_field, int* ext_degree);

int ark_hip_malloc(size_t bytes, void** out_dptr);
int ark_hip_free(void* dptr);
int ark_hip_memcpy_h2d(void* dst_dptr, const void* src_host, size_t bytes);
int ark_hip_memcpy_d2h(void* dst_host, const void* src_dptr, size_t bytes);
int ark_hip_memcpy_d2d(void* dst_dptr, const void* src_dptr, size_t bytes);
int ark_hip_memset_device(void* dptr, int value, size_t bytes);
int ark_hip_host_alloc(size_t bytes, void** out_ptr);
int ark_hip_host_free(void* ptr);

int ark_hip_curve_generator(int curve, uint64_t* out_xy);

int ark_hip_msm_sw(int curve, const uint64_t* bases, const uint64_t* scalars, size_t n, int scalars_are_montgomery,
                   uint64_t* out_xyz);
int ark_hip_msm_bases_pin(int curve, const uint64_t* bases, size_t n);
int ark_hip_msm_bases_unpin(int curve, const uint64_t* bases, size_t n);
int ark_hip_msm_cache_config(long long budget_bytes, int auto_prepare_after);
int ark_hip_msm_cache_clear(void);
int ark_hip_msm_cache_stats(uint64_t out[8]);
int ark_hip_msm_cache_hash_stats(uint64_t out[4]);
int ark_hip_msm_sw_small(int curve, const uint64_t* bases, const void* scalars, size_t n, int scalar_bytes, int max_bits,
                         uint64_t* out_xyz);
int ark_hip_msm_sw_small_device(int curve, const void* d_bases, const void* d_scalars, size_t n, int scalar_bytes,
                                int max_bits, uint64_t* out_xyz);
int ark_hip_msm_sw_device(int curve, const void* d_bases, const void* d_scalars, size_t n, int scalars_are_montgomery,
                          uint64_t* out_xyz);
typedef struct ark_hip_msm_job ark_hip_msm_job;
int ark_hip_msm_sw_device_async(int curve, const void* d_bases, const void* d_scalars, size_t n,
                                int scalars_are_montgomery, ark_hip_msm_job** out_job);
int ark_hip_msm_wait(ark_hip_msm_job* job, uint64_t* out_xyz);

typedef struct ark_hip_msm_bases ark_hip_msm_bases;
int ark_hip_msm_bases_prepare(int curve, const uint64_t* bases, size_t n, ark_hip_msm_bases** out);
int ark_hip_msm_bases_prepare_device(int curve, const void* d_bases, size_t n, ark_hip_msm_bases** out);
int ark_hip_msm_bases_free(ark_hip_msm_bases* bases);
int ark_hip_msm_bases_info(const ark_hip_msm_bases* bases, size_t* n, int* window_bits, int* windows, size_t* table_bytes);
int ark_hip_msm_prepared(const ark_hip_msm_bases* bases, const uint64_t* scalars, size_t n, int scalars_are_montgomery,
                         uint64_t* out_xyz);
int ark_hip_msm_prepared_device(const ark_hip_msm_bases* bases, const void* d_scalars, size_t n,
                                int scalars_are_montgomery, uint64_t* out_xyz);
int ark_hip_msm_prepared_small_device(const ark_hip_msm_bases* bases, const void* d_scalars, size_t n, int scalar_bytes,
                                      int max_bits, uint64_t* out_xyz);
int ark_hip_msm_prepared_async(const ark_hip_msm_bases* bases, const uint64_t* scalars, size_t n,
                               int scalars_are_montgomery, ark_hip_msm_job** out_job);
int ark_hip_msm_prepared_device_async(const ark_hip_msm_bases* bases, const void* d_scalars, size_t n,
                                      int scalars_are_montgomery, ark_hip_msm_job** out_job);

int ark_hip_msm_sw_chunks(int curve, const uint64_t* bases, size_t n_bases, const uint64_t* scalars, size_t n_scalars,
                          size_t step, uint64_t* out_xyz);

int ark_hip_msm_sw_multi(int curve, int n_gpus, const uint64_t* bases, const uint64_t* scalars, size_t n,
                         int scalars_are_montgomery, uint64_t* out_xyz);
int ark_hip_msm_sw_multi_device(int curve, int n_gpus, const void* const* d_bases, const void* const* d_scalars,
                                const size_t* n_per_gpu, int scalars_are_montgomery, uint64_t* out_xyz);
int ark_hip_msm_prepared_multi(int n_gpus, const ark_hip_msm_bases* const* shards, const uint64_t* scalars, size_t n,
                               int scalars_are_montgomery, uint64_t* out_xyz);

int ark_hip_msm_plan(int curve, size_t n, int prepared, int* window_bits, int* windows);
int ark_hip_msm_plan_widths(int curve, size_t n, uint32_t max_bits, const uint32_t counts[9], int* window_bits, int* windows);
int ark_hip_msm_set_timing(int enable);
int ark_hip_msm_last_timing(double out[8]);

typedef struct ark_hip_batch_mul_table ark_hip_batch_mul_table;
int ark_hip_batch_mul_table_new(int curve, const uint64_t* base_xyz, size_t num_scalars, ark_hip_batch_mul_table** out);
int ark_hip_batch_mul_table_free(ark_hip_batch_mul_table* table);
int ark_hip_batch_mul(const ark_hip_batch_mul_table* table, const uint64_t* scalars, size_t n, int scalars_are_montgomery,
                      uint64_t* out_xy);
int ark_hip_batch_mul_device(const ark_hip_batch_mul_table* table, const void* d_scalars, size_t n,
                             int scalars_are_montgomery, void* d_out_xy);

int ark_hip_sw_sum(int curve, const uint64_t* jac_points, size_t n, uint64_t* out_xyz);
int ark_hip_sw_into_affine(int curve, const uint64_t* jac_points, size_t n, uint64_t* out_xy);

int ark_hip_sw_add_affine_device(int curve, const void* d_in, void* d_out, size_t n, const uint64_t* delta_xy);

int ark_hip_sw_normalize_batch_device(int curve, const void* d_jac, void* d_out_xy, size_t n);
int ark_hip_sw_normalize_batch(int curve, const uint64_t* jac_points, size_t n, uint64_t* out_xy);

typedef struct {
  uint64_t size;
  uint32_t log_size_of_group;
  uint32_t _pad;
  uint64_t size_as_field_element[4];
  uint64_t size_inv[4];
  uint64_t group_gen[4];
  uint64_t group_gen_inv[4];
  uint64_t offset[4];
  uint64_t offset_inv[4];
  uint64_t offset_pow_size[4];
} ark_hip_radix2_domain;

int ark_hip_radix2_domain_new(int field, size_t num_coeffs, ark_hip_radix2_domain* out);
int ark_hip_radix2_domain_get_coset(int field, const ark_hip_radix2_domain* dom, const uint64_t* offset,
                                    ark_hip_radix2_domain* out);
int ark_hip_fft_in_place(int field, const ark_hip_radix2_domain* dom, uint64_t* data);
int ark_hip_ifft_in_place(int field, const ark_hip_radix2_domain* dom, uint64_t* data);
int ark_hip_fft_in_place_device(int field, const ark_hip_radix2_domain* dom, void* d_data);
int ark_hip_ifft_in_place_device(int field, const ark_hip_radix2_domain* dom, void* d_data);
int ark_hip_fft_in_place_degree_aware(int field, const ark_hip_radix2_domain* dom, uint64_t* data, size_t num_coeffs);
int ark_hip_fft_in_place_degree_aware_device(int field, const ark_hip_radix2_domain* dom, void* d_data, size_t num_coeffs);
int ark_hip_fft_batch_in_place_device(int field, const ark_hip_radix2_domain* dom, void* const* d_data, size_t count,
                                      int inverse);
int ark_hip_fr_mul_device(int field, const void* d_a, const void* d_b, void* d_r, size_t n);
int ark_hip_fft_group_in_place(int curve, const ark_hip_radix2_domain* dom, uint64_t* jac_points, int inverse);
int ark_hip_fft_group_in_place_device(int curve, const ark_hip_radix2_domain* dom, void* d_jac_points, int inverse);
int ark_hip_fr_add_device(int field, const void* d_a, const void* d_b, void* d_r, size_t n);
int ark_hip_fr_sub_device(int field, const void* d_a, const void* d_b, void* d_r, size_t n);
int ark_hip_fr_neg_device(int field, const void* d_a, void* d_r, size_t n);
int ark_hip_fr_scale_device(int field, const void* d_a, const uint64_t* k, void* d_r, size_t n);
int ark_hip_fr_div_device(int field, const void* d_a, const void* d_b, void* d_r, size_t n);
int ark_hip_fr_inverse_device(int field, const void* d_a, void* d_r, size_t n);
int ark_hip_poly_mul(int field, const uint64_t* a, size_t na, const uint64_t* b, size_t nb, uint64_t* out, size_t* out_len);
int ark_hip_fr_pow(int field, const uint64_t* base, uint64_t exp, uint64_t* out);
int ark_hip_fft_axis_device(int field, void* d_data, unsigned G, size_t cols, const uint64_t* root);

int ark_hip_poly_evaluate_device(int field, const void* d_coeffs, size_t n, const uint64_t* point, uint64_t* out);
int ark_hip_poly_divide_linear_device(int field, const void* d_coeffs, size_t n, const uint64_t* z, void* d_quot,
                                      uint64_t* out_rem);
int ark_hip_poly_divide_by_vanishing_device(int field, size_t domain_size, const void* d_coeffs, size_t n, void* d_quot,
                                            void* d_rem);
int ark_hip_domain_lagrange_coefficients_device(int field, const ark_hip_radix2_domain* dom, const uint64_t* tau, void* d_out);
int ark_hip_fr_inner_product_device(int field, const void* d_a, const void* d_b, size_t n, uint64_t* out);
int ark_hip_poly_scan_plan(size_t n, int* tile, int* levels);

#define ARK_HIP_COMM_ID_BYTES 128
int ark_hip_comm_unique_id(void* out_id);
int ark_hip_comm_init(const void* id, int rank, int world);
int ark_hip_comm_info(int* rank, int* world);
int ark_hip_comm_destroy(void);
int ark_hip_msm_sw_device_sharded(int curve, const void* d_bases, const void* d_scalars, size_t n_local,
                                  int scalars_are_montgomery, uint64_t* out_xyz);
int ark_hip_msm_prepared_device_sharded(const ark_hip_msm_bases* bases, const void* d_scalars, size_t n_local,
                                        int scalars_are_montgomery, uint64_t* out_xyz);
int ark_hip_fft_sharded_device(int field, const ark_hip_radix2_domain* dom, void* d_local, int inverse);
int ark_hip_fft_shard_local_device(int field, const ark_hip_radix2_domain* dom, int rank, int world, void* d_local,
                                   int inverse);
int ark_hip_fft_shard_cross_device(int field, const ark_hip_radix2_domain* dom, int world, const void* d_src, void* d_dst,
                                   int inverse);
int ark_hip_fft_set_kernel(int variant);
int ark_hip_fft_set_timing(int enable);
int ark_hip_fft_last_timing(double out[10]);

#ifdef ARK_HIP_TEST_HOOKS
int ark_hip_test_field_op(int field, int op, const uint64_t* a, const uint64_t* b, uint64_t* r, size_t n);
int ark_hip_test_basefield_op(int curve, int op, const uint64_t* a, const uint64_t* b, uint64_t* r, size_t n);
int ark_hip_test_host_basefield_op(int curve, int op, const uint64_t* a, const uint64_t* b, uint64_t* r, size_t n);
int ark_hip_test_point_op(int curve, int kind, const uint64_t* acc, const uint64_t* other, uint64_t* out, size_t n);
int ark_hip_test_msm_sharded_emulated(int curve, int world, const void* const* d_bases, const void* const* d_scalars,
                                      const size_t* n_local, int scalars_are_montgomery, uint64_t* out_xyz, int* path);
int ark_hip_test_base_hash(const uint64_t* p, size_t words, uint64_t out[2]);
int ark_hip_test_msm_host_fold(int curve, const uint64_t* parts, int windows, int nbits, int log2_l0, const int* widths,
                               uint64_t* out_xyz);
int ark_hip_test_msm_host_fold_l0(int curve, const uint64_t* parts, int windows, int nbits, int l0, const int* widths,
                                  uint64_t* out_xyz);
int ark_hip_test_lazy_raw_op(int field, int op, int k, int h, const uint32_t* in, uint32_t* out, size_t n);
int ark_hip_test_lazy_acc_op(int curve, int kind, const void* acc, const void* other, void* out, size_t n);

#endif

#if defined(__GNUC__) || defined(__clang__)
#pragma GCC visibility pop
#endif
#ifdef __cplusplus
}
#endif
#endif
```

Baseline: 471.6 million.

## Fuse tile histogram into MSM digit kernel and add compact 4-byte partition entries

```diff
diff --git a/algebra_amd/_lib.py b/algebra_amd/_lib.py
--- a/algebra_amd/_lib.py
+++ b/algebra_amd/_lib.py
@@ -143,6 +143,8 @@
     "ark_hip_test_lazy_acc_op": (C.c_int, [C.c_int, C.c_int, C.c_void_p, C.c_void_p, C.c_void_p, C.c_size_t]),
     "ark_hip_test_msm_host_fold": (C.c_int, [C.c_int, C.c_void_p, C.c_int, C.c_int, C.c_int, C.c_void_p, C.c_void_p]),
     "ark_hip_test_msm_host_fold_l0": (C.c_int, [C.c_int, C.c_void_p, C.c_int, C.c_int, C.c_int, C.c_void_p, C.c_void_p]),
+    "ark_hip_test_msm_sort": (C.c_int, [C.c_int, C.c_void_p, C.c_size_t, C.c_int, C.c_int, C.c_int, C.c_void_p, C.c_void_p,
+                                        C.POINTER(C.c_int)]),
 }
 TEST_LIB_PATH = os.path.join(_HERE, "libark_hip_test.so")
 
diff --git a/algebra_amd/csrc/msm.cuh b/algebra_amd/csrc/msm.cuh
--- a/algebra_amd/csrc/msm.cuh
+++ b/algebra_amd/csrc/msm.cuh
@@ -225,71 +225,101 @@
   return 2 * wide < seen;
 }
 
+static constexpr int DIGITS_THREADS = 1024;
+static constexpr size_t DIGITS_LDS_MAX = 64 * 1024;
+static constexpr size_t DIGITS_HIST_MIN_N = (size_t)1 << 22;
+__device__ __forceinline__ void msm_digits_hist_clear(u32* hist, u32 ncnt) {
+  for (u32 b = threadIdx.x; b < ncnt; b += blockDim.x) hist[b] = 0;
+  __syncthreads();
+}
+__device__ __forceinline__ void msm_digits_hist_store(const u32* hist, int W, int HB, u32 ntiles, u32 tile_id, u32* __restrict__ tile_hist) {
+  __syncthreads();
+  for (u32 b = threadIdx.x; b < ((u32)W << HB); b += blockDim.x) tile_hist[(size_t)b * ntiles + tile_id] = hist[b];
+}
+
 template <class SP>
-__global__ void __launch_bounds__(256) msm_digits_kernel(const u32* __restrict__ scalars, u32 n, int mont, int c,
+__global__ void __launch_bounds__(DIGITS_THREADS) msm_digits_kernel(const u32* __restrict__ scalars, u32 n, int mont, int c,
                                                          int W, int narrow, u32* __restrict__ keys,
-                                                         u32* __restrict__ err) {
-  u32 i = blockIdx.x * blockDim.x + threadIdx.x;
-  if (i >= n) return;
+                                                         u32* __restrict__ err, int HB, u32 ntiles, u32 tile,
+                                                         u32* __restrict__ tile_hist) {
+  extern __shared__ u32 digits_lds[];
   typedef Fp<SP> S;
-  u32 v[S::N + 1];
-  const u32 flip = msm_scalar_magnitude<SP>(scalars, i, mont, v, err);
-  u32 carry = 0;
-  for (int w = 0; w < W; w++) {
-    const int cw = msm_window_width(w, c, W, narrow);
-    const u32 mask = (1u << cw) - 1u;
-    const u32 half = 1u << (cw - 1);
-    u32 raw = (v[0] & mask) + carry;
+  const u32 hmask = (1u << HB) - 1u;
+  if (tile_hist) msm_digits_hist_clear(digits_lds, (u32)W << HB);
+  const u32 tile_id = part_tile_of_block(blockIdx.x, ntiles);
+  const u32 lo = tile_id * tile;
+  const u32 hi = lo + tile < n ? lo + tile : n;
+  for (u32 i = lo + threadIdx.x; i < hi; i += blockDim.x) {
+    u32 v[S::N + 1];
+    const u32 flip = msm_scalar_magnitude<SP>(scalars, i, mont, v, err);
+    u32 carry = 0;
+    for (int w = 0; w < W; w++) {
+      const int cw = msm_window_width(w, c, W, narrow);
+      const u32 mask = (1u << cw) - 1u;
+      const u32 half = 1u << (cw - 1);
+      u32 raw = (v[0] & mask) + carry;
 #pragma unroll
-    for (int k = 0; k < S::N; k++) v[k] = (v[k] >> cw) | (v[k + 1] << (32 - cw));
-    u32 key = KEY_NONE;
-    if (w < W - 1) {
-      carry = raw >= half ? 1u : 0u;
-    } else {
-      carry = 0;
-    }
-    int d = (int)raw - (int)(carry << cw);
-    if (d != 0) {
-      u32 mag = d < 0 ? (u32)(-d) : (u32)d;
-      if (mag > half) {
-        atomicOr(err, 1u);
-        mag = half;
-      }
-      u32 sign = (d < 0 ? 0x80000000u : 0u) ^ flip;
-      key = sign | (mag - 1);
-    }
-    keys[(size_t)w * n + i] = key;
-  }
+      for (int k = 0; k < S::N; k++) v[k] = (v[k] >> cw) | (v[k + 1] << (32 - cw));
+      u32 key = KEY_NONE;
+      if (w < W - 1) {
+        carry = raw >= half ? 1u : 0u;
+      } else {
+        carry = 0;
+      }
+      int d = (int)raw - (int)(carry << cw);
+      if (d != 0) {
+        u32 mag = d < 0 ? (u32)(-d) : (u32)d;
+        if (mag > half) {
+          atomicOr(err, 1u);
+          mag = half;
+        }
+        u32 sign = (d < 0 ? 0x80000000u : 0u) ^ flip;
+        key = sign | (mag - 1);
+        if (tile_hist) atomicAdd(&digits_lds[((u32)w << HB) | ((mag - 1) & hmask)], 1u);
+      }
+      keys[(size_t)w * n + i] = key;
+    }
+  }
+  if (tile_hist) msm_digits_hist_store(digits_lds, W, HB, ntiles, tile_id, tile_hist);
 }
 
 template <int BYTES>
-__global__ void __launch_bounds__(256) msm_digits_small_kernel(const unsigned char* __restrict__ scalars, u32 n, int c, int W,
-                                                               int narrow, u64 vmask, u32* __restrict__ keys) {
-  u32 i = blockIdx.x * blockDim.x + threadIdx.x;
-  if (i >= n) return;
-  u64 v;
-  if constexpr (BYTES == 1) v = scalars[i];
-  else if constexpr (BYTES == 2) v = ((const unsigned short*)scalars)[i];
-  else if constexpr (BYTES == 4) v = ((const u32*)scalars)[i];
-  else v = ((const u64*)scalars)[i];
-  v &= vmask;
-  u32 carry = 0;
-  for (int w = 0; w < W; w++) {
-    const int cw = msm_window_width(w, c, W, narrow);
-    const u32 mask = (1u << cw) - 1u;
-    const u32 half = 1u << (cw - 1);
-    const u32 raw = ((u32)v & mask) + carry;
-    v >>= cw;
-    carry = (w < W - 1 && raw >= half) ? 1u : 0u;
-    const int d = (int)raw - (int)(carry << cw);
-    u32 key = KEY_NONE;
-    if (d != 0) {
-      u32 mag = d < 0 ? (u32)(-d) : (u32)d;
-      if (mag > half) mag = half;
-      key = (d < 0 ? 0x80000000u : 0u) | (mag - 1);
-    }
-    keys[(size_t)w * n + i] = key;
-  }
+__global__ void __launch_bounds__(DIGITS_THREADS) msm_digits_small_kernel(const unsigned char* __restrict__ scalars, u32 n, int c, int W,
+                                                               int narrow, u64 vmask, u32* __restrict__ keys, int HB,
+                                                               u32 ntiles, u32 tile, u32* __restrict__ tile_hist) {
+  extern __shared__ u32 digits_lds[];
+  const u32 hmask = (1u << HB) - 1u;
+  if (tile_hist) msm_digits_hist_clear(digits_lds, (u32)W << HB);
+  const u32 tile_id = part_tile_of_block(blockIdx.x, ntiles);
+  const u32 lo = tile_id * tile;
+  const u32 hi = lo + tile < n ? lo + tile : n;
+  for (u32 i = lo + threadIdx.x; i < hi; i += blockDim.x) {
+    u64 v;
+    if constexpr (BYTES == 1) v = scalars[i];
+    else if constexpr (BYTES == 2) v = ((const unsigned short*)scalars)[i];
+    else if constexpr (BYTES == 4) v = ((const u32*)scalars)[i];
+    else v = ((const u64*)scalars)[i];
+    v &= vmask;
+    u32 carry = 0;
+    for (int w = 0; w < W; w++) {
+      const int cw = msm_window_width(w, c, W, narrow);
+      const u32 mask = (1u << cw) - 1u;
+      const u32 half = 1u << (cw - 1);
+      const u32 raw = ((u32)v & mask) + carry;
+      v >>= cw;
+      carry = (w < W - 1 && raw >= half) ? 1u : 0u;
+      const int d = (int)raw - (int)(carry << cw);
+      u32 key = KEY_NONE;
+      if (d != 0) {
+        u32 mag = d < 0 ? (u32)(-d) : (u32)d;
+        if (mag > half) mag = half;
+        key = (d < 0 ? 0x80000000u : 0u) | (mag - 1);
+        if (tile_hist) atomicAdd(&digits_lds[((u32)w << HB) | ((mag - 1) & hmask)], 1u);
+      }
+      keys[(size_t)w * n + i] = key;
+    }
+  }
+  if (tile_hist) msm_digits_hist_store(digits_lds, W, HB, ntiles, tile_id, tile_hist);
 }
 
 static constexpr int SCAN_TILE = 2048;
@@ -1191,6 +1221,171 @@
   while (width < nchunks && width < NS) width <<= 1;
   Ops::tree(acc, sh, slot, width);
   if (slot == 0) Ops::fin(acc).store(out + (size_t)t * Pt::BYTES);
+}
+
+struct MsmSortGeom {
+  size_t n;
+  int W, HB, LB;
+  int entry;
+  u32 ptile, ntiles;
+  bool digits_hist;
+  u32 stage_cap;
+  size_t lds_a, lds_b, lds_big, lds_digits;
+  bool big_on;
+};
+static inline int msm_sort_geom(size_t n, int W, int Bbits, bool compacted, MsmSortGeom* out, int forced_entry = msm_part_entry_env()) {
+  MsmSortGeom g{};
+  g.n = n;
+  g.W = W;
+  msm_part_split(n, Bbits, &g.HB, &g.LB);
+  g.entry = 8;
+  g.ptile = msm_part_tile(g.HB, 8);
+  g.ntiles = (u32)((n + g.ptile - 1) / g.ptile);
+  if (forced_entry == 4 && !compacted) {
+    const u32 t4 = msm_part_tile(g.HB, 4);
+    const u32 nt4 = (u32)((n + t4 - 1) / t4);
+    if (nt4 + 1 <= PART_RUNS_MAX) {
+      g.entry = 4;
+      g.ptile = t4;
+      g.ntiles = nt4;
+    }
+  }
+  const u32 runs = g.entry == 4 ? g.ntiles + 1 : 0u;
+  g.lds_a = msm_part_scatter_lds(g.HB, g.ptile, g.entry);
+  if (g.lds_a > PART_SCATTER_LDS_MAX) return -2;
+  g.stage_cap = msm_part_stage_cap(g.LB) - runs;
+  g.lds_b = ((size_t)(1 << g.LB) + 1024 + msm_part_stage_cap(g.LB)) * 4;
+  g.lds_big = ((size_t)8 << g.LB) + 4096 + (size_t)runs * 4;
+  g.lds_digits = ((size_t)W << g.HB) * 4;
+  g.digits_hist = g.lds_digits <= DIGITS_LDS_MAX && n >= DIGITS_HIST_MIN_N;
+  if (const char* e = getenv("ARK_HIP_MSM_DIGITS_HIST")) {
+    if (e[0] == '1') g.digits_hist = g.lds_digits <= DIGITS_LDS_MAX;
+    if (e[0] == '0') g.digits_hist = false;
+  }
+  if (!g.digits_hist) g.lds_digits = 0;
+  static const bool big_env = [] {
+    const char* e = getenv("ARK_HIP_MSM_BIG_SLICES");
+    return !(e && atoi(e) == 0);
+  }();
+  g.big_on = big_env && n > (size_t)2 * PART_BIG;
+  *out = g;
+  return 0;
+}
+static inline int msm_sort_set_attrs() {
+  ARK_HIP_TRY(hipFuncSetAttribute((const void*)msm_part_scatter_kernel<u32>, hipFuncAttributeMaxDynamicSharedMemorySize, (int)PART_SCATTER_LDS_MAX));
+  ARK_HIP_TRY(hipFuncSetAttribute((const void*)msm_part_scatter_kernel<uint2>, hipFuncAttributeMaxDynamicSharedMemorySize, (int)PART_SCATTER_LDS_MAX));
+  ARK_HIP_TRY(hipFuncSetAttribute((const void*)msm_part_finish_kernel<u32>, hipFuncAttributeMaxDynamicSharedMemorySize, 160 * 1024 - 64));
+  ARK_HIP_TRY(hipFuncSetAttribute((const void*)msm_part_finish_kernel<uint2>, hipFuncAttributeMaxDynamicSharedMemorySize, 160 * 1024 - 64));
+  return 0;
+}
+template <class SP>
+static inline void msm_launch_digits(const MsmSortGeom& g, const void* d_scalars, int mont, int c, int narrow, int sbytes, int sbits,
+                                     u32* keys, u32* err, u32* thist, hipStream_t stream) {
+  u32* const th = g.digits_hist ? thist : nullptr;
+  const u32 dtile = g.digits_hist ? g.ptile : 256u, dtiles = g.digits_hist ? g.ntiles : (u32)((g.n + 255) / 256);
+  const dim3 grid(dtiles), block(g.digits_hist ? DIGITS_THREADS : 256);
+  if (sbytes) {
+    const u64 vmask = sbits >= 64 ? ~0ull : ((1ull << sbits) - 1ull);
+    const unsigned char* sp = (const unsigned char*)d_scalars;
+    switch (sbytes) {
+      case 1: hipLaunchKernelGGL((msm_digits_small_kernel<1>), grid, block, g.lds_digits, stream, sp, (u32)g.n, c, g.W, narrow, vmask, keys, g.HB, dtiles, dtile, th); break;
+      case 2: hipLaunchKernelGGL((msm_digits_small_kernel<2>), grid, block, g.lds_digits, stream, sp, (u32)g.n, c, g.W, narrow, vmask, keys, g.HB, dtiles, dtile, th); break;
+      case 4: hipLaunchKernelGGL((msm_digits_small_kernel<4>), grid, block, g.lds_digits, stream, sp, (u32)g.n, c, g.W, narrow, vmask, keys, g.HB, dtiles, dtile, th); break;
+      default: hipLaunchKernelGGL((msm_digits_small_kernel<8>), grid, block, g.lds_digits, stream, sp, (u32)g.n, c, g.W, narrow, vmask, keys, g.HB, dtiles, dtile, th); break;
+    }
+  } else {
+    hipLaunchKernelGGL((msm_digits_kernel<SP>), grid, block, g.lds_digits, stream, (const u32*)d_scalars, (u32)g.n, mont, c, g.W, narrow,
+                       keys, err, g.HB, dtiles, dtile, th);
+  }
+}
+struct MsmSortBufs {
+  int Wg;
+  const u32* keys;
+  u32 *thist, *toff, *sums;
+  void* part;
+  const u32* point_idx;
+  u32 *big_count, *big;
+  u32 *offsets, *sorted;
+};
+template <class E>
+static inline int msm_sort_launch_as(const MsmSortGeom& g, const MsmSortBufs& b, hipStream_t st, hipEvent_t scanned) {
+  const u32 n = (u32)g.n, ntiles = g.ntiles;
+  const int HB = g.HB, LB = g.LB;
+  const u32 nsuper_g = (u32)b.Wg << HB;
+  const size_t nslots = (size_t)nsuper_g << LB;
+  if (!g.digits_hist)
+    hipLaunchKernelGGL(msm_part_hist_kernel, dim3(ntiles, b.Wg), dim3(256), (size_t)4 << HB, st, b.keys, n, HB, LB, ntiles, g.ptile, b.thist);
+  scan_exclusive(b.thist, (size_t)nsuper_g * ntiles, b.sums, b.toff, st);
+  if (scanned) ARK_HIP_TRY(hipEventRecord(scanned, st));
+  E* const part = (E*)b.part;
+  hipLaunchKernelGGL((msm_part_scatter_kernel<E>), dim3(ntiles, b.Wg), dim3(1024), g.lds_a, st, b.keys, n, HB, LB, ntiles, g.ptile,
+                     (const u32*)b.toff, part, b.point_idx);
+  hipLaunchKernelGGL((msm_part_finish_kernel<E>), dim3(nsuper_g), dim3(1024), g.lds_b, st, (const E*)part, (const u32*)b.toff, ntiles,
+                     g.ptile, LB, nsuper_g, g.stage_cap, g.big_on ? PART_BIG : 0u, b.big_count, b.big, b.offsets, b.sorted);
+  if (g.big_on) {
+    u32* const bigcnt = b.big + nsuper_g;
+    u32* const cursor = bigcnt + nslots;
+    hipLaunchKernelGGL((msm_part_big_hist_kernel<E>), dim3(PART_BIG_SLICES, PART_BIG_GRID_Y), dim3(1024), (size_t)4 << LB, st,
+                       (const E*)part, (const u32*)b.toff, ntiles, LB, (const u32*)b.big_count, (const u32*)b.big, bigcnt);
+    hipLaunchKernelGGL((msm_part_big_place_kernel<E>), dim3(PART_BIG_SLICES, PART_BIG_GRID_Y), dim3(1024), g.lds_big, st,
+                       (const E*)part, (const u32*)b.toff, ntiles, g.ptile, LB, (const u32*)b.big_count, (const u32*)b.big,
+                       (const u32*)bigcnt, cursor, b.offsets, b.sorted);
+  }
+  return 0;
+}
+static inline int msm_sort_launch(const MsmSortGeom& g, const MsmSortBufs& b, hipStream_t st, hipEvent_t scanned) {
+  if (g.entry == 4 && b.point_idx) return -1;
+  return g.entry == 4 ? msm_sort_launch_as<u32>(g, b, st, scanned) : msm_sort_launch_as<uint2>(g, b, st, scanned);
+}
+
+static inline void msm_window_layout(int c, int bits, int* W, int* narrow);
+template <class SP>
+int msm_test_sort(const void* d_scalars, size_t n, int mont, int c, int entry, u32* h_offsets, u32* h_sorted, int info[8]) {
+  if (!d_scalars || !h_offsets || !h_sorted || !info || n == 0 || n >= (1ull << 28) || c < 3 || c > 23) return -1;
+  int W, narrow;
+  msm_window_layout(c, SP::BITS, &W, &narrow);
+  const int Bbits = c - 1;
+  MsmSortGeom g;
+  if (int rc = msm_sort_geom(n, W, Bbits, false, &g, entry)) return rc;
+  if ((size_t)n * (size_t)W >= (1ull << 32)) return -2;
+  if (int rc = msm_sort_set_attrs()) return rc;
+  const size_t nb = (size_t)W << Bbits, nsuper = (size_t)W << g.HB, nthist = nsuper * g.ntiles;
+  const size_t nsums = (nthist + SCAN_TILE - 1) / SCAN_TILE + 2;
+  const size_t words[] = {(size_t)W * n, (size_t)W * n, (size_t)W * n * (size_t)(g.entry / 4), nthist, nthist + 2, nsums, nb + 2,
+                          nsuper + 2 * nb, 16};
+  u32* buf[9] = {};
+  int rc = 0;
+  for (int k = 0; k < 9 && !rc; k++)
+    if (hipMalloc((void**)&buf[k], words[k] * 4) != hipSuccess) rc = -3;
+  u32 *keys = buf[0], *sorted = buf[1], *part = buf[2], *thist = buf[3], *toff = buf[4], *sums = buf[5], *offsets = buf[6],
+      *big = buf[7], *hctr = buf[8];
+  hipStream_t st = nullptr;
+  u32 err = 0;
+  if (!rc && hipMemsetAsync(hctr, 0, 64, st) != hipSuccess) rc = -4;
+  if (!rc) {
+    msm_launch_digits<SP>(g, d_scalars, mont, c, narrow, 0, 0, keys, hctr + 3, thist, st);
+    MsmSortBufs b{};
+    b.Wg = W;
+    b.keys = keys;
+    b.thist = thist;
+    b.toff = toff;
+    b.sums = sums;
+    b.part = part;
+    b.big_count = hctr + 8;
+    b.big = big;
+    b.offsets = offsets;
+    b.sorted = sorted;
+    rc = msm_sort_launch(g, b, st, nullptr);
+  }
+  if (!rc && (hipMemcpyAsync(h_offsets, offsets, (nb + 1) * 4, hipMemcpyDeviceToHost, st) != hipSuccess ||
+              hipMemcpyAsync(h_sorted, sorted, (size_t)W * n * 4, hipMemcpyDeviceToHost, st) != hipSuccess ||
+              hipMemcpyAsync(&err, hctr + 3, 4, hipMemcpyDeviceToHost, st) != hipSuccess || hipStreamSynchronize(st) != hipSuccess))
+    rc = -4;
+  for (auto p : buf)
+    if (p) (void)hipFree(p);
+  const int out[8] = {W, narrow, g.HB, g.LB, g.entry, (int)g.ptile, (int)err, g.digits_hist ? 1 : 0};
+  for (int k = 0; k < 8; k++) info[k] = out[k];
+  return rc;
 }
 
 struct MsmPlan {
@@ -1561,15 +1756,15 @@
   const size_t mwin = (size_t)1 << (c - 1);
 
   const int Bbits = c - 1;
-  int HB, LB;
-  msm_part_split(n, Bbits, &HB, &LB);
+  MsmSortGeom sg;
+  if (int rc = msm_sort_geom(n, W, Bbits, compacted, &sg)) return rc;
+  const int HB = sg.HB, LB = sg.LB;
   const u32 nsuper = (u32)W << HB;
-  const u32 ptile = msm_part_tile(HB);
-  const u32 ntiles = (u32)((n + ptile - 1) / ptile);
+  const u32 ntiles = sg.ntiles;
   const size_t nthist = (size_t)nsuper * ntiles;
   if (ws.keys.ensure((size_t)W * n * 4)) return -3;
   if (ws.sorted.ensure((size_t)W * n * 4)) return -3;
-  if (ws.part.ensure((size_t)W * n * 8)) return -3;
+  if (ws.part.ensure((size_t)W * n * (size_t)sg.entry)) return -3;
   if (ws.thist.ensure(nthist * 4) || ws.toff.ensure((nthist + 2) * 4)) return -3;
   if (ws.offsets.ensure((nb + 2) * 4)) return -3;
   const u32 ntscan = (u32)((nthist + SCAN_TILE - 1) / SCAN_TILE);
@@ -1669,7 +1864,7 @@
   u32* offsets = (u32*)ws.offsets.p;
   u32* thist = (u32*)ws.thist.p;
   u32* toff = (u32*)ws.toff.p;
-  uint2* part = (uint2*)ws.part.p;
+  char* part = (char*)ws.part.p;
   u32* order = (u32*)ws.order.p;
   u32* sums = (u32*)ws.sums.p;
 
@@ -1694,20 +1889,11 @@
                        (const u32*)d_scalars_all, (u32)n_all, scalars_mont, nz_chunk, (const u32*)off, (u32*)ws.hctr.p + 3,
                        (u32*)ws.cscal.p, (u32*)ws.cidx.p, (u32)n);
   }
-  const u32 nblk = (u32)((n + 255) / 256);
-  if (sbytes) {
-    const u64 vmask = sbits >= 64 ? ~0ull : ((1ull << sbits) - 1ull);
-    const unsigned char* sp = (const unsigned char*)d_scalars;
-    switch (sbytes) {
-      case 1: hipLaunchKernelGGL((msm_digits_small_kernel<1>), dim3(nblk), dim3(256), 0, stream, sp, (u32)n, c, W, pl.narrow, vmask, keys); break;
-      case 2: hipLaunchKernelGGL((msm_digits_small_kernel<2>), dim3(nblk), dim3(256), 0, stream, sp, (u32)n, c, W, pl.narrow, vmask, keys); break;
-      case 4: hipLaunchKernelGGL((msm_digits_small_kernel<4>), dim3(nblk), dim3(256), 0, stream, sp, (u32)n, c, W, pl.narrow, vmask, keys); break;
-      default: hipLaunchKernelGGL((msm_digits_small_kernel<8>), dim3(nblk), dim3(256), 0, stream, sp, (u32)n, c, W, pl.narrow, vmask, keys); break;
-    }
-  } else {
-    hipLaunchKernelGGL((msm_digits_kernel<typename C::S>), dim3(nblk), dim3(256), 0, stream, (const u32*)d_scalars,
-                       (u32)n, scalars_mont, c, W, pl.narrow, keys, (u32*)ws.hctr.p + 3);
-  }
+  if (!ws.attr_set) {
+    if (int rc = msm_sort_set_attrs()) return rc;
+    ws.attr_set = true;
+  }
+  msm_launch_digits<typename C::S>(sg, d_scalars, scalars_mont, c, pl.narrow, sbytes, sbits, keys, (u32*)ws.hctr.p + 3, thist, stream);
   if (timing) ARK_HIP_TRY(hipEventRecord(job.ev[1], stream));
 
   int ngroups = 1;
@@ -1732,22 +1918,7 @@
     for (auto& e : ws.grp_ev)
       if (!e) ARK_HIP_TRY(hipEventCreateWithFlags(&e, hipEventDisableTiming));
   }
-  const size_t lds_a = ((size_t)8 << HB) + (size_t)ptile * 8;
-  if (lds_a > PART_SCATTER_LDS_MAX) return -2;
-  const u32 stage_cap = msm_part_stage_cap(LB);
-  const size_t lds_b = ((size_t)(1 << LB) + 1024 + stage_cap) * 4;
-  if (!ws.attr_set) {
-    ARK_HIP_TRY(hipFuncSetAttribute((const void*)msm_part_scatter_kernel, hipFuncAttributeMaxDynamicSharedMemorySize,
-                                    (int)PART_SCATTER_LDS_MAX));
-    ARK_HIP_TRY(hipFuncSetAttribute((const void*)msm_part_finish_kernel, hipFuncAttributeMaxDynamicSharedMemorySize,
-                                    160 * 1024 - 64));
-    ws.attr_set = true;
-  }
-  static const bool big_env = [] {
-    const char* e = getenv("ARK_HIP_MSM_BIG_SLICES");
-    return !(e && atoi(e) == 0);
-  }();
-  const bool big_on = big_env && n > (size_t)2 * PART_BIG;
+  const bool big_on = sg.big_on;
   const size_t big_region = (size_t)nsuper + 2 * nb;
   if (big_on && ws.big.ensure(2 * big_region * 4)) return -3;
   bool lazy = false;
@@ -1786,7 +1957,7 @@
     u32 *keys, *sorted, *offsets, *thist, *toff, *order, *sums, *ohist, *ooff, *hctr;
     u32* big;
     u32* big_count;
-    uint2* part;
+    char* part;
     HeavyEntry* hlist;
     uint2* hitems;
     char *hpart, *buckets;
@@ -1801,7 +1972,7 @@
     G.nbk_g = pl.shared ? nbk : G.nslots;
     G.keys = keys + (size_t)G.w0 * n;
     G.sorted = sorted + (size_t)G.w0 * n;
-    G.part = part + (size_t)G.w0 * n;
+    G.part = part + (size_t)G.w0 * n * (size_t)sg.entry;
     G.offsets = offsets + G.slot0 + (size_t)g;
     G.thist = thist + ((size_t)G.w0 << HB) * ntiles;
     G.toff = toff + ((size_t)G.w0 << HB) * ntiles + (size_t)g;
@@ -1822,25 +1993,19 @@
     G.buckets = d_buckets + (pl.shared ? 0 : G.slot0 * Pt::BYTES);
   }
   auto sort_group = [&](const Group& G, hipStream_t st, bool mark) -> int {
-    const u32 nsuper_g = (u32)G.Wg << HB;
-    const size_t nthist_g = (size_t)nsuper_g * ntiles;
-    hipLaunchKernelGGL(msm_part_hist_kernel, dim3(ntiles, G.Wg), dim3(256), (size_t)4 << HB, st, G.keys, (u32)n, HB, LB,
-                       ntiles, ptile, G.thist);
-    scan_exclusive(G.thist, nthist_g, G.sums, G.toff, st);
-    if (mark && timing) ARK_HIP_TRY(hipEventRecord(job.ev[2], st));
-    hipLaunchKernelGGL(msm_part_scatter_kernel, dim3(ntiles, G.Wg), dim3(1024), lds_a, st, G.keys, (u32)n, HB, LB, ntiles,
-                       ptile, G.toff, G.part, compacted ? (const u32*)ws.cidx.p : (const u32*)nullptr);
-    hipLaunchKernelGGL(msm_part_finish_kernel, dim3(nsuper_g), dim3(1024), lds_b, st, G.part, G.toff, ntiles, LB, nsuper_g,
-                       stage_cap, big_on ? PART_BIG : 0u, G.big_count, G.big, G.offsets, G.sorted);
-    if (big_on) {
-      u32* const bigcnt = G.big + nsuper_g;
-      u32* const cursor = bigcnt + G.nslots;
-      hipLaunchKernelGGL(msm_part_big_hist_kernel, dim3(PART_BIG_SLICES, PART_BIG_GRID_Y), dim3(1024), (size_t)4 << LB, st,
-                         G.part, G.toff, ntiles, LB, G.big_count, G.big, bigcnt);
-      hipLaunchKernelGGL(msm_part_big_place_kernel, dim3(PART_BIG_SLICES, PART_BIG_GRID_Y), dim3(1024),
-                         ((size_t)8 << LB) + 4096, st, G.part, G.toff, ntiles, LB, G.big_count, G.big, bigcnt, cursor, G.offsets,
-                         G.sorted);
-    }
+    MsmSortBufs sb{};
+    sb.Wg = G.Wg;
+    sb.keys = G.keys;
+    sb.thist = G.thist;
+    sb.toff = G.toff;
+    sb.sums = G.sums;
+    sb.part = G.part;
+    sb.point_idx = compacted ? (const u32*)ws.cidx.p : (const u32*)nullptr;
+    sb.big_count = G.big_count;
+    sb.big = G.big;
+    sb.offsets = G.offsets;
+    sb.sorted = G.sorted;
+    if (int rc = msm_sort_launch(sg, sb, st, (mark && timing) ? job.ev[2] : (hipEvent_t) nullptr)) return rc;
     int shift = 0;
     while ((mean_load >> shift) >= 64) shift++;
     const u32 noblk_g = (u32)((G.nbk_g + ORDER_TILE - 1) / ORDER_TILE);
diff --git a/algebra_amd/csrc/msm_sort.cuh b/algebra_amd/csrc/msm_sort.cuh
--- a/algebra_amd/csrc/msm_sort.cuh
+++ b/algebra_amd/csrc/msm_sort.cuh
@@ -39,13 +39,25 @@
 static constexpr int PART_TILE = 8192;
 static constexpr int PART_TILE_BIG = 16384;
 static constexpr size_t PART_SCATTER_LDS_MAX = 160 * 1024 - 4096 - 64;
-static inline u32 msm_part_tile(int HB) {
+static constexpr u32 PART_RUNS_MAX = 6144;
+static inline size_t msm_part_scatter_lds(int HB, u32 tile, int entry_bytes) {
+  return (((size_t)2 << HB) + 2) * 4 + (size_t)tile * (size_t)entry_bytes;
+}
+static inline u32 msm_part_tile(int HB, int entry_bytes) {
+  const bool fits = msm_part_scatter_lds(HB, PART_TILE_BIG, entry_bytes) <= PART_SCATTER_LDS_MAX;
   if (const char* e = getenv("ARK_HIP_MSM_TILE")) {
     const int v = atoi(e);
-    if (v == PART_TILE || (v == PART_TILE_BIG && ((size_t)8 << HB) + (size_t)PART_TILE_BIG * 8 <= PART_SCATTER_LDS_MAX)) return (u32)v;
-  }
-  const bool fits = ((size_t)8 << HB) + (size_t)PART_TILE_BIG * 8 <= PART_SCATTER_LDS_MAX;
-  return (HB >= 11 && fits) ? (u32)PART_TILE_BIG : (u32)PART_TILE;
+    if (v == PART_TILE || (v == PART_TILE_BIG && fits)) return (u32)v;
+  }
+  return (HB >= (entry_bytes == 4 ? 9 : 11) && fits) ? (u32)PART_TILE_BIG : (u32)PART_TILE;
+}
+static inline int msm_part_entry_env() {
+  static const int v = [] {
+    const char* e = getenv("ARK_HIP_MSM_SORT_ENTRY");
+    const int x = e ? atoi(e) : 0;
+    return (x == 4 || x == 8) ? x : 0;
+  }();
+  return v;
 }
 static constexpr u32 PART_KEY_NONE = 0xffffffffu;
 static constexpr int PART_MLP = 8;
@@ -66,6 +78,57 @@
   return b < (per << 3) ? (b & 7u) * per + (b >> 3) : b;
 }
 
+struct PartWalk {
+  u32 r;
+  __device__ __forceinline__ void init(const u32* starts, u32 nruns, u32 j0) {
+    u32 lo = 0, hi = nruns;
+    while (hi - lo > 1) {
+      const u32 mid = (lo + hi) >> 1;
+      if (starts[mid] <= j0) lo = mid; else hi = mid;
+    }
+    r = lo;
+  }
+  __device__ __forceinline__ u32 at(const u32* starts, u32 j) {
+    while (starts[r + 1] <= j) r++;
+    return r;
+  }
+};
+struct PartSweep {
+  u32 beg, end, stride, off;
+  __device__ __forceinline__ PartSweep(u32 lo, u32 hi, bool chunked) {
+    if (chunked) {
+      const u32 nw = blockDim.x >> 6, wv = threadIdx.x >> 6;
+      const u32 per = ((hi - lo + nw * 64u - 1u) / (nw * 64u)) * 64u;
+      const u32 a = wv * per < hi - lo ? wv * per : hi - lo;
+      beg = lo + a;
+      end = hi - beg < per ? hi : beg + per;
+      stride = 64u;
+      off = threadIdx.x & 63u;
+    } else {
+      beg = lo;
+      end = hi;
+      stride = blockDim.x;
+      off = threadIdx.x;
+    }
+  }
+};
+__device__ __forceinline__ u32 part_entry_key(u32 e) { return e; }
+__device__ __forceinline__ u32 part_entry_key(uint2 e) { return e.x; }
+__device__ __forceinline__ u32 part_entry_index(u32 e, PartWalk& wk, const u32* runs, u32 tile, int LB, u32 j) {
+  return (wk.at(runs, j) * tile + ((e & 0x7fffffffu) >> LB)) | (e & 0x80000000u);
+}
+__device__ __forceinline__ u32 part_entry_index(uint2 e, PartWalk&, const u32*, u32, int, u32) {
+  return e.y | (e.x & 0x80000000u);
+}
+template <class E> __device__ __forceinline__ E part_entry_none();
+template <> __device__ __forceinline__ u32 part_entry_none<u32>() { return PART_KEY_NONE; }
+template <> __device__ __forceinline__ uint2 part_entry_none<uint2>() { return make_uint2(PART_KEY_NONE, 0u); }
+template <class E>
+__device__ __forceinline__ void part_load_runs(u32* runs, const u32* __restrict__ tile_off, u32 sb, u32 ntiles) {
+  if constexpr (sizeof(E) == 4)
+    for (u32 t = threadIdx.x; t <= ntiles; t += blockDim.x) runs[t] = tile_off[(size_t)sb * ntiles + t];
+}
+
 static __global__ void __launch_bounds__(256) msm_part_hist_kernel(const u32* __restrict__ keys, u32 n, int HB, int LB,
                                                                    u32 ntiles, u32 tile, u32* __restrict__ tile_hist) {
   extern __shared__ u32 part_lds[];
@@ -94,16 +157,18 @@
     tile_hist[((size_t)((w << HB) | b)) * ntiles + tile_id] = part_lds[b];
 }
 
-static __global__ void __launch_bounds__(1024, 8) msm_part_scatter_kernel(const u32* __restrict__ keys, u32 n, int HB,
-                                                                       int LB, u32 ntiles, u32 tile,
-                                                                       const u32* __restrict__ tile_off,
-                                                                       uint2* __restrict__ part,
-                                                                       const u32* __restrict__ point_idx = nullptr) {
+template <class E>
+__global__ void __launch_bounds__(1024, 8) msm_part_scatter_kernel(const u32* __restrict__ keys, u32 n, int HB,
+                                                                int LB, u32 ntiles, u32 tile,
+                                                                const u32* __restrict__ tile_off,
+                                                                E* __restrict__ part,
+                                                                const u32* __restrict__ point_idx = nullptr) {
+  constexpr bool E4 = sizeof(E) == 4;
   extern __shared__ u32 part_lds[];
   const u32 nbins = 1u << HB;
   u32* cnt = part_lds;
   u32* lstart = part_lds + nbins;
-  uint2* stage = (uint2*)(part_lds + 2 * nbins);
+  E* stage = (E*)(part_lds + 2 * nbins + 2);
   __shared__ u32 wsum[1024];
   const u32 w = blockIdx.y;
   const size_t base = (size_t)w * n;
@@ -112,12 +177,12 @@
   const u32 hi = lo + tile < n ? lo + tile : n;
   const u32 hmask = nbins - 1u;
   for (u32 b = threadIdx.x; b < nbins; b += blockDim.x) cnt[b] = 0;
-  u32 key[PART_SCATTER_KEYS], pidx[PART_SCATTER_KEYS];
+  u32 key[PART_SCATTER_KEYS], pidx[E4 ? 1 : PART_SCATTER_KEYS];
 #pragma unroll
   for (int b = 0; b < PART_SCATTER_KEYS; b++) {
     const u32 i = lo + (u32)b * blockDim.x + threadIdx.x;
     key[b] = i < hi ? keys[base + i] : PART_KEY_NONE;
-    pidx[b] = (point_idx && i < hi) ? point_idx[i] : i;
+    if constexpr (!E4) pidx[b] = (point_idx && i < hi) ? point_idx[i] : i;
   }
   __syncthreads();
 #pragma unroll
@@ -148,34 +213,50 @@
       run += v;
     }
   }
-  __syncthreads();
   const u32 total = wsum[blockDim.x - 1];
+  if (threadIdx.x == 0) lstart[nbins] = total;
+  __syncthreads();
 #pragma unroll
   for (int b = 0; b < PART_SCATTER_KEYS; b++) {
     if (key[b] != PART_KEY_NONE) {
       const u32 pos = atomicAdd(&cnt[key[b] & hmask], 1u);
-      stage[pos] = make_uint2(key[b], pidx[b]);
-    }
-  }
-  __syncthreads();
-  for (u32 j0 = 0; j0 < total; j0 += blockDim.x * PART_OUT_MLP) {
-    uint2 e[PART_OUT_MLP];
-    u32 dst[PART_OUT_MLP];
-#pragma unroll
-    for (int b = 0; b < PART_OUT_MLP; b++) {
-      const u32 j = j0 + (u32)b * blockDim.x + threadIdx.x;
-      if (j < total) {
+      if constexpr (E4) {
+        const u32 local = (u32)b * blockDim.x + threadIdx.x;
+        stage[pos] = ((key[b] & 0x7fffffffu) >> HB) | (local << LB) | (key[b] & 0x80000000u);
+      } else {
+        stage[pos] = make_uint2(key[b], pidx[b]);
+      }
+    }
+  }
+  __syncthreads();
+  constexpr int MLP = E4 ? 2 * PART_OUT_MLP : PART_OUT_MLP;
+  const PartSweep sw(0u, total, E4);
+  PartWalk wk;
+  if constexpr (E4) wk.init(lstart, nbins, sw.beg);
+  for (u32 c0 = sw.beg; c0 < sw.end; c0 += sw.stride * MLP) {
+    E e[MLP];
+    u32 dst[MLP];
+#pragma unroll
+    for (int b = 0; b < MLP; b++) {
+      const u32 j = c0 + (u32)b * sw.stride + sw.off;
+      if (j < sw.end) {
         e[b] = stage[j];
-        const u32 bin = e[b].x & hmask;
+        u32 bin;
+        if constexpr (E4) bin = wk.at(lstart, j);
+        else bin = e[b].x & hmask;
         dst[b] = tile_off[((size_t)((w << HB) | bin)) * ntiles + tile_id] + (j - lstart[bin]);
       }
     }
 #pragma unroll
-    for (int b = 0; b < PART_OUT_MLP; b++) {
-      const u32 j = j0 + (u32)b * blockDim.x + threadIdx.x;
-      if (j < total) {
-        const u32 bkt = e[b].x & 0x7fffffffu;
-        part[dst[b]] = make_uint2((bkt >> HB) | (e[b].x & 0x80000000u), e[b].y);
+    for (int b = 0; b < MLP; b++) {
+      const u32 j = c0 + (u32)b * sw.stride + sw.off;
+      if (j < sw.end) {
+        if constexpr (E4) {
+          part[dst[b]] = e[b];
+        } else {
+          const u32 bkt = e[b].x & 0x7fffffffu;
+          part[dst[b]] = make_uint2((bkt >> HB) | (e[b].x & 0x80000000u), e[b].y);
+        }
       }
     }
   }
@@ -196,8 +277,9 @@
   return pos;
 }
 
-static __global__ void __launch_bounds__(1024) msm_part_finish_kernel(const uint2* __restrict__ part,
-                                                                      const u32* __restrict__ tile_off, u32 ntiles,
+template <class E>
+__global__ void __launch_bounds__(1024) msm_part_finish_kernel(const E* __restrict__ part,
+                                                                      const u32* __restrict__ tile_off, u32 ntiles, u32 tile,
                                                                       int LB, u32 nsuper, u32 stage_cap, u32 big_thresh,
                                                                       u32* __restrict__ big_count, u32* __restrict__ big,
                                                                       u32* __restrict__ offsets,
@@ -206,7 +288,8 @@
   const u32 nlow = 1u << LB;
   u32* cnt = part_lds;
   u32* wsum = part_lds + nlow;
-  u32* stage = wsum + 1024;
+  u32* runs = wsum + 1024;
+  u32* stage = runs + (sizeof(E) == 4 ? ntiles + 1 : 0u);
   const u32 sb = blockIdx.x;
   const u32 start = tile_off[(size_t)sb * ntiles];
   const u32 end = tile_off[(size_t)(sb + 1) * ntiles];
@@ -222,6 +305,7 @@
     return;
   }
   for (u32 b = threadIdx.x; b < nlow; b += blockDim.x) cnt[b] = 0;
+  part_load_runs<E>(runs, tile_off, sb, ntiles);
   __syncthreads();
   const u32 lmask = nlow - 1u;
   for (u32 c0 = start; c0 < end; c0 += blockDim.x * PART_MLP) {
@@ -229,7 +313,7 @@
 #pragma unroll
     for (int b = 0; b < PART_MLP; b++) {
       const u32 j = c0 + (u32)b * blockDim.x + threadIdx.x;
-      kx[b] = j < end ? part[j].x : PART_KEY_NONE;
+      kx[b] = j < end ? part_entry_key(part[j]) : PART_KEY_NONE;
     }
 #pragma unroll
     for (int b = 0; b < PART_MLP; b++)
@@ -260,29 +344,33 @@
   }
   __syncthreads();
   const u32 total = end - start;
+  const PartSweep sw(start, end, sizeof(E) == 4);
+  PartWalk wk;
+  if constexpr (sizeof(E) == 4) wk.init(runs, ntiles, sw.beg);
   if (total <= stage_cap) {
-    for (u32 c0 = start; c0 < end; c0 += blockDim.x * PART_MLP) {
-      uint2 e[PART_MLP];
+    for (u32 c0 = sw.beg; c0 < sw.end; c0 += sw.stride * PART_MLP) {
+      E e[PART_MLP];
 #pragma unroll
       for (int b = 0; b < PART_MLP; b++) {
-        const u32 j = c0 + (u32)b * blockDim.x + threadIdx.x;
-        e[b] = j < end ? part[j] : make_uint2(PART_KEY_NONE, 0u);
+        const u32 j = c0 + (u32)b * sw.stride + sw.off;
+        e[b] = j < sw.end ? part[j] : part_entry_none<E>();
       }
 #pragma unroll
       for (int b = 0; b < PART_MLP; b++) {
-        if (e[b].x != PART_KEY_NONE) {
-          const u32 pos = lds_inc_leading(cnt, e[b].x & lmask);
-          stage[pos] = e[b].y | (e[b].x & 0x80000000u);
+        if (part_entry_key(e[b]) != PART_KEY_NONE) {
+          const u32 j = c0 + (u32)b * sw.stride + sw.off;
+          const u32 pos = lds_inc_leading(cnt, part_entry_key(e[b]) & lmask);
+          stage[pos] = part_entry_index(e[b], wk, runs, tile, LB, j);
         }
       }
     }
     __syncthreads();
     for (u32 j = threadIdx.x; j < total; j += blockDim.x) sorted[start + j] = stage[j];
   } else {
-    for (u32 j = start + threadIdx.x; j < end; j += blockDim.x) {
-      uint2 e = part[j];
-      u32 pos = lds_inc_leading(cnt, e.x & lmask);
-      sorted[start + pos] = e.y | (e.x & 0x80000000u);
+    for (u32 j = sw.beg + sw.off; j < sw.end; j += sw.stride) {
+      const E e = part[j];
+      const u32 pos = lds_inc_leading(cnt, part_entry_key(e) & lmask);
+      sorted[start + pos] = part_entry_index(e, wk, runs, tile, LB, j);
     }
   }
 }
@@ -299,7 +387,8 @@
   *hi = start + (b < total ? b : total);
 }
 
-static __global__ void __launch_bounds__(1024) msm_part_big_hist_kernel(const uint2* __restrict__ part,
+template <class E>
+__global__ void __launch_bounds__(1024) msm_part_big_hist_kernel(const E* __restrict__ part,
                                                                         const u32* __restrict__ tile_off, u32 ntiles, int LB,
                                                                         const u32* __restrict__ big_count,
                                                                         const u32* __restrict__ big,
@@ -318,7 +407,7 @@
 #pragma unroll
       for (int b = 0; b < PART_MLP; b++) {
         const u32 j = c0 + (u32)b * blockDim.x + threadIdx.x;
-        kx[b] = j < hi ? part[j].x : PART_KEY_NONE;
+        kx[b] = j < hi ? part_entry_key(part[j]) : PART_KEY_NONE;
       }
 #pragma unroll
       for (int b = 0; b < PART_MLP; b++)
@@ -331,8 +420,9 @@
   }
 }
 
-static __global__ void __launch_bounds__(1024) msm_part_big_place_kernel(const uint2* __restrict__ part,
-                                                                         const u32* __restrict__ tile_off, u32 ntiles, int LB,
+template <class E>
+__global__ void __launch_bounds__(1024) msm_part_big_place_kernel(const E* __restrict__ part,
+                                                                         const u32* __restrict__ tile_off, u32 ntiles, u32 tile, int LB,
                                                                          const u32* __restrict__ big_count,
                                                                          const u32* __restrict__ big,
                                                                          const u32* __restrict__ bigcnt,
@@ -344,6 +434,7 @@
   u32* cnt = part_lds;
   u32* wsum = part_lds + nlow;
   u32* mine = wsum + 1024;
+  u32* runs = mine + nlow;
   for (u32 k = blockIdx.y; k < nbig; k += gridDim.y) {
     const u32 sb = big[k];
     const u32 start = tile_off[(size_t)sb * ntiles];
@@ -353,6 +444,7 @@
       cnt[b] = bigcnt[((size_t)sb << LB) + b];
       mine[b] = 0;
     }
+    part_load_runs<E>(runs, tile_off, sb, ntiles);
     __syncthreads();
     const u32 per = nlow > blockDim.x ? nlow / blockDim.x : 1u;
     const u32 b0 = threadIdx.x * per;
@@ -382,7 +474,7 @@
 #pragma unroll
       for (int b = 0; b < PART_MLP; b++) {
         const u32 j = c0 + (u32)b * blockDim.x + threadIdx.x;
-        kx[b] = j < hi ? part[j].x : PART_KEY_NONE;
+        kx[b] = j < hi ? part_entry_key(part[j]) : PART_KEY_NONE;
       }
 #pragma unroll
       for (int b = 0; b < PART_MLP; b++)
@@ -394,18 +486,22 @@
       if (m) mine[b] = cnt[b] + atomicAdd(&cursor[((size_t)sb << LB) + b], m);
     }
     __syncthreads();
-    for (u32 c0 = lo; c0 < hi; c0 += blockDim.x * PART_MLP) {
-      uint2 e[PART_MLP];
+    const PartSweep sw(lo, hi, sizeof(E) == 4);
+    PartWalk wk;
+    if constexpr (sizeof(E) == 4) wk.init(runs, ntiles, sw.beg);
+    for (u32 c0 = sw.beg; c0 < sw.end; c0 += sw.stride * PART_MLP) {
+      E e[PART_MLP];
 #pragma unroll
       for (int b = 0; b < PART_MLP; b++) {
-        const u32 j = c0 + (u32)b * blockDim.x + threadIdx.x;
-        e[b] = j < hi ? part[j] : make_uint2(PART_KEY_NONE, 0u);
+        const u32 j = c0 + (u32)b * sw.stride + sw.off;
+        e[b] = j < sw.end ? part[j] : part_entry_none<E>();
       }
 #pragma unroll
       for (int b = 0; b < PART_MLP; b++) {
-        if (e[b].x != PART_KEY_NONE) {
-          const u32 pos = lds_inc_leading(mine, e[b].x & lmask);
-          sorted[start + pos] = e[b].y | (e[b].x & 0x80000000u);
+        if (part_entry_key(e[b]) != PART_KEY_NONE) {
+          const u32 j = c0 + (u32)b * sw.stride + sw.off;
+          const u32 pos = lds_inc_leading(mine, part_entry_key(e[b]) & lmask);
+          sorted[start + pos] = part_entry_index(e[b], wk, runs, tile, LB, j);
         }
       }
     }
diff --git a/algebra_amd/csrc/testops_field.hip b/algebra_amd/csrc/testops_field.hip
--- a/algebra_amd/csrc/testops_field.hip
+++ b/algebra_amd/csrc/testops_field.hip
@@ -1,5 +1,6 @@
 #define ARK_LAZYTEST_FFT 1
 #include "lazytest.cuh"
+#include "msm.cuh"
 #ifndef ARK_TEST_FIELD
 #error "compile with -DARK_TEST_FIELD=BLS12_381_FR (or another scalar field of params.hpp)"
 #endif
@@ -9,4 +10,8 @@
 int ARK_CAT(test_lazy_raw_op_, ARK_TEST_FIELD)(int op, int k, int h, const void* in, void* out, size_t n, hipStream_t s) {
   return lazytest::lazy_raw_op_launch<ARK_TEST_FIELD, true, void>(op, k, h, in, out, n, s);
 }
+int ARK_CAT(test_msm_sort_, ARK_TEST_FIELD)(const void* d_scalars, size_t n, int mont, int c, int entry, uint32_t* h_offsets,
+                                            uint32_t* h_sorted, int info[8]) {
+  return msm_test_sort<ARK_TEST_FIELD>(d_scalars, n, mont, c, entry, h_offsets, h_sorted, info);
 }
+}
diff --git a/include/ark_hip.h b/include/ark_hip.h
--- a/include/ark_hip.h
+++ b/include/ark_hip.h
@@ -180,6 +180,8 @@
                                uint64_t* out_xyz);
 int ark_hip_test_msm_host_fold_l0(int curve, const uint64_t* parts, int windows, int nbits, int l0, const int* widths,
                                   uint64_t* out_xyz);
+int ark_hip_test_msm_sort(int curve, const void* d_scalars, size_t n, int scalars_are_montgomery, int window_bits, int entry_bytes,
+                          uint32_t* offsets, uint32_t* sorted, int info[8]);
 int ark_hip_test_lazy_raw_op(int field, int op, int k, int h, const uint32_t* in, uint32_t* out, size_t n);
 int ark_hip_test_lazy_acc_op(int curve, int kind, const void* acc, const void* other, void* out, size_t n);
 
```

Result: no change. 472.2 million, median of 2 (+0.1%).
